# EnnaDelfen/SUHMO

Hardware: AMD Instinct MI355X
Metric: multigrid V-cycles/s (FAS head solve) + GSRB cell-updates/s; achieved HBM GB/s vs peak (higher is better)
Workload: dtype f64; 1 GPU; SHMIP-A head solve, 4096x4096 cells per GPU (square cells of 24.4 m), single AMR level, 64x64 boxes, 6 MG depths, 4+4 GSRB sweeps per depth, 16 bottom (BASELINE north_star: 4096^2 single-level); partition=none

## Files before the change

### suhmo_amd/csrc/suhmo_common.h

```cpp
#pragma once
#include <hip/hip_runtime.h>
#include <cstdio>
#include <cstdlib>
#include <cstring>
#include <utility>
#include <string>
#include <vector>
#include "../../include/suhmo_hip.h"

#define SUHMO_XOFF 16
#define SUHMO_MAXDEPTH 16

struct DV {
    int nx, ny;
    int P;
    int gy;
    int rows;
    int j0, nyg;
    double dx, dy;
    double rdx, rdy;
    double fdx, fdy;
    double alpha, beta;
    int bct[2][2];
    double two_v[2][2];
    double neu[2][2];
    int per[2];
    int ext[2];
    int i0, nxg;
    int cfx[2];
    int rk[2];
};

struct FP { double *f[SUHMO_F_COUNT]; };

__host__ __device__ __forceinline__ int cidx(const DV &v, int i, int j)
{
    return (j + v.gy) * v.P + SUHMO_XOFF + i;
}

__device__ __forceinline__ double phiW(const DV &v, const double *__restrict__ p, int idx, int i, double c, bool homog)
{
    if (i > 0 || v.cfx[0]) return p[idx - 1];
    if (v.per[0]) return p[idx + v.nx - 1];
    if (v.bct[0][0] == 0) return (homog ? 0.0 : v.two_v[0][0]) - c;
    return homog ? c : c + v.neu[0][0];
}
__device__ __forceinline__ double phiE(const DV &v, const double *__restrict__ p, int idx, int i, double c, bool homog)
{
    if (i < v.nx - 1 || v.cfx[1]) return p[idx + 1];
    if (v.per[0]) return p[idx - (v.nx - 1)];
    if (v.bct[0][1] == 0) return (homog ? 0.0 : v.two_v[0][1]) - c;
    return homog ? c : c + v.neu[0][1];
}
__device__ __forceinline__ double phiS(const DV &v, const double *__restrict__ p, int idx, int j, double c, bool homog)
{
    if (j > 0 || v.ext[0]) return p[idx - v.P];
    if (v.per[1]) return p[idx + (v.ny - 1) * v.P];
    if (v.bct[1][0] == 0) return (homog ? 0.0 : v.two_v[1][0]) - c;
    return homog ? c : c + v.neu[1][0];
}
__device__ __forceinline__ double phiN(const DV &v, const double *__restrict__ p, int idx, int j, double c, bool homog)
{
    if (j < v.ny - 1 || v.ext[1]) return p[idx + v.P];
    if (v.per[1]) return p[idx - (v.ny - 1) * v.P];
    if (v.bct[1][1] == 0) return (homog ? 0.0 : v.two_v[1][1]) - c;
    return homog ? c : c + v.neu[1][1];
}

__device__ __forceinline__ void nl_terms(const suhmo_phys_t &ph, double phi, double B, double Pi,
                                         double zb, double mask, double &nl, double &dnl)
{
    if (!ph.use_NL || mask < 0.0) { nl = 0.0; dnl = 0.0; return; }
    double N = Pi - ph.rho_w_g * (phi - zb);
    nl = -ph.A * B * N * N * N;
    dnl = 3.0 * ph.A * B * 1000.0 * ph.grav * N * N;
    if (ph.cutOffbr > B) {
        nl = nl * (1.0 - (ph.cutOffbr - B) / ph.cutOffbr);
        dnl = dnl * B / ph.cutOffbr;
    }
    if (ph.maxOffbr < B) {
        nl = nl * (1.0 - (ph.maxOffbr - B) / ph.maxOffbr);
        dnl = dnl * B / ph.maxOffbr;
    }
}

__device__ __forceinline__ double lofphi_cell(const DV &v, double aterm, double c, double e, double w,
                                              double n, double s, double bxE, double bxW, double byN,
                                              double byS, double nl)
{
    return aterm * c
           - v.beta * (bxE * (e - c) * v.rdx - bxW * (c - w) * v.rdx
                       + byN * (n - c) * v.rdy - byS * (c - s) * v.rdy)
           + nl;
}

__device__ __forceinline__ double lambda_cell(const DV &v, double aterm, double bxE, double bxW,
                                              double byN, double byS)
{
    double lam = aterm;
    lam = lam + v.rdx * v.beta * (bxE + bxW);
    lam = lam + v.rdy * v.beta * (byN + byS);
    return lam;
}

__device__ __forceinline__ void gradcc_from(const DV &v, double c, double w, double e, double s, double n, bool zW, bool zE, bool zS,
                                            bool zN, double &gx, double &gy)
{
    double gW = v.fdx * (c - w), gE = v.fdx * (e - c), gS = v.fdy * (c - s), gN = v.fdy * (n - c);
    if (zW) gW = 0.0;
    if (zE) gE = 0.0;
    if (zS) gS = 0.0;
    if (zN) gN = 0.0;
    gx = 0.5 * (gW + gE);
    gy = 0.5 * (gS + gN);
}
__device__ __forceinline__ double grad_norm(double gx, double gy) { return sqrt(gx * gx + gy * gy); }
__device__ __forceinline__ double re_from(const suhmo_phys_t &ph, double sg, double B)
{
    double discr = 1.0 + 4.0 * ph.omega * (B * B * B * ph.grav * sg) / (12.0 * ph.nu * ph.nu);
    return (-1.0 + sqrt(discr)) / (2.0 * ph.omega);
}
__device__ __forceinline__ double bcoef_face(const suhmo_phys_t &ph, double Rc, double Rm, double Bc, double Bm,
                                             double mc, double mm, bool dom_edge)
{
    double Ref = 0.5 * (Rc + Rm), Bf = 0.5 * (Bc + Bm);
    double mec;
    if (fabs(mc - mm) < 1e-10) mec = (mc > 0.0) ? 1.0 : -1.0; else mec = 0.0;
    if (dom_edge) mec = 0.0;
    double num_q = -(Bf * Bf * Bf * ph.grav);
    double denom_q = 12.0 * ph.nu * (1.0 + ph.omega * Ref);
    if (mec < 0.0 && ph.cutOffB > 0) return 0.0;
    return num_q / denom_q;
}

struct Depth {
    DV v;
    FP fp;
    size_t elems;
    int nbox;
    int prolong_pending;
    int rhs_pending;
    int bcoef_pending;
    double *phi_alt;
    int phi_fresh;
    int zb_state;
    double zb_value;
};

struct VGraph {
    int key[4]; hipGraphExec_t exec;
    double *p0[SUHMO_MAXDEPTH], *a0[SUHMO_MAXDEPTH];
    double *p1[SUHMO_MAXDEPTH], *a1[SUHMO_MAXDEPTH];
    double *rhs;
    int rout_req, rout_done, rout_np; const double *rout_rhs;
    int bcoef_in_relax; long n_bcoef_in_relax;
    int mask_clean; long n_bcoef_unmasked, n_relax_unmasked;
    unsigned zb_uniform, zb_version; long n_relax_zb[SUHMO_MAXDEPTH];
    int has_scan;
};
struct ProfEv { hipEvent_t a, b; long cells; int restricts; };

struct suhmo_level {
    int ndepth;
    int batch_owned;
    int stub;
    Depth d[SUHMO_MAXDEPTH];
    suhmo_level_desc_t desc;
    std::vector<int> boxes;
    suhmo_phys_t ph;
    int device;
    double *scratch;
    double *hscratch;
    double *hscratch_dev;
    unsigned long long hseq;
    int poll_readback;
    size_t scratch_elems;
    suhmo_exchange_fn ex;
    suhmo_allreduce_max_fn ar;
    suhmo_allreduce_fn ar2;
    int (*ard)(void *user, double *dev_values, int n, int op, suhmo_stream_t s);
    void *user;
    int (*ex_begin)(void *user);
    int (*ex_end)(void *user, suhmo_level *L, suhmo_stream_t s);
    long graph_max_cells;
    std::vector<VGraph> vgraphs; int vgraph_seen[4]; hipStream_t gstream;
    long vgraph_replays;
    suhmo_level *gap; double gap_dt;
    void *rccl;
    int faces_deferred;
    void *ipc; int ipc_owner;
    long agg_min_cells;
    int agg_depth, agg_world, agg_rank;
    suhmo_level *agg;
    int agg_static_stale;
    suhmo_allgather_fn ag; void *ag_user;
    double *agg_send, *agg_recv; size_t agg_cap; long agg_gathers;
    int resout_req, resout_armed, resout_done; const double *resout_rhs; long resout_count;
    int resout_np;
    int bcoef_in_relax, bcoef_nd; long bcoef_in_relax_count;
    int avg_overlap, avg_fork, avg_flying; long avg_overlap_count;
    hipStream_t astream; hipEvent_t aev[2];
    long frhs_stream, frhs_tile;
    long strip_tile, strip_tile_rst, strip_tile_shallow, strip_colour, strip_stream, strip_stream_rst, strip_prolong_unfused;
    int prof_on;
    std::vector<ProfEv> prof;
    int gsrb_variant;
    long fused_min_cells;
    int bcoef_fused;
    int bcoef_tile_x;
    int fused_nt;
    int fused_restrict;
    int fused_hc;
    int fas_rhs_fused;
    int strips_rhs_local;
    int skip_mask;
    int mask_reported;
    int coarse_mask_ok;
    unsigned mask_epoch, maskflag_epoch;
    int mask_known, mask_state;
    unsigned mask_version, mask_scan_version;
    int mask_scan_pending, mask_capturing;
    int mask_scan_captured;
    int mask_view;
    int mask_scan_errors;
    unsigned *mask_host; hipEvent_t mask_ev;
    long mask_scans, bcoef_unmasked, relax_unmasked;
    int zb_known, zb_off;
    unsigned zb_version, zb_scan_version;
    int zb_scan_pending, zb_scan_errors;
    unsigned long long *zb_dev, *zb_host;
    hipEvent_t zb_ev;
    long zb_scans, relax_zb_uniform[SUHMO_MAXDEPTH];
    int overlap_halo;
    hipStream_t xstream; hipEvent_t xev[2]; long overlapped;
    int tile_strips;
    int tile_chunks;
    int resid_in_relax;
    int fas_rhs_in_relax;
    long tile_max_cells;
    int tile_restrict;
    int tile_order;
    int bottom_solver; long bottom_one_launch_max_cells;
    unsigned long long *bottom_ctr; long bottom_host_iters, bottom_host_solves;
    int gsrb_tile, tile_t, tile_s;
    struct suhmo_tagmap *tags;
    int faces_made;
    double *bal_buf;
    int track_old_volume, vol_np;
    double *vol_buf, *wb_buf;
};
static inline void suhmo_faces_made(suhmo_level *L) { L->faces_made = 1; }

enum { SUHMO_MASK_UNKNOWN = 0, SUHMO_MASK_CLEAN = 1, SUHMO_MASK_DIRTY = 2 };
static inline void suhmo_mask_written(suhmo_level *L)
{
    L->coarse_mask_ok = 0; L->maskflag_epoch = 0;
    L->mask_version++; L->mask_state = SUHMO_MASK_UNKNOWN;
}
static inline void suhmo_mask_halo_written(suhmo_level *L) { L->mask_version++; L->mask_state = SUHMO_MASK_UNKNOWN; }
enum { SUHMO_ZB_UNKNOWN = 0, SUHMO_ZB_UNIFORM = 1, SUHMO_ZB_VARYING = 2 };
static inline void suhmo_zb_written(suhmo_level *L)
{
    L->zb_version++;
    for (int d = 0; d < SUHMO_MAXDEPTH; d++) L->d[d].zb_state = SUHMO_ZB_UNKNOWN;
}
static inline bool suhmo_zb_uniform(const suhmo_level *L, int depth)
{
    return L->zb_known && !L->zb_off && L->d[depth].zb_state == SUHMO_ZB_UNIFORM && !L->ex && L->desc.nx_global == 0;
}
void suhmo_zb_poll(suhmo_level *L);
int suhmo_zb_scan_if_due(suhmo_level *L, hipStream_t st);
bool suhmo_gsrb_streams(const suhmo_level *L, int depth);
bool suhmo_mask_would_scan(const suhmo_level *L);
#define SUHMO_HSCRATCH_DOUBLES 64
#define SUHMO_HSCRATCH_MASK 60
#define SUHMO_HSCRATCH_ZB 16
static inline unsigned *suhmo_mask_report_word(const suhmo_level *L) { return (unsigned *)(L->scratch + L->scratch_elems - 1); }
static inline unsigned *suhmo_mask_scan_word(const suhmo_level *L) { return suhmo_mask_report_word(L) + 1; }
int suhmo_mask_scan_begin(suhmo_level *L, hipStream_t st);
int suhmo_mask_scan_end(suhmo_level *L, hipStream_t st);
void suhmo_mask_poll(suhmo_level *L);
static inline bool suhmo_mask_clean(const suhmo_level *L, int depth)
{
    return L->mask_known && !L->mask_view && L->mask_state == SUHMO_MASK_CLEAN && (depth == 0 || L->coarse_mask_ok) && L->desc.nx_global == 0;
}
void suhmo_set_error(const char *fmt, ...);
void suhmo_tagmap_release(struct suhmo_tagmap *m);
struct SuhmoTimer { const char *name; double t0; int mode; explicit SuhmoTimer(const char *n); ~SuhmoTimer(); };
#define SUHMO_TIME(label) SuhmoTimer suhmo_tm_(label)
#define HIPCHK(x) do { hipError_t e_ = (x); if (e_ != hipSuccess) { \
    suhmo_set_error("%s:%d %s -> %s", __FILE__, __LINE__, #x, hipGetErrorString(e_)); return -2; } } while (0)
#define ARG(cond) do { if (!(cond)) { suhmo_set_error("%s:%d bad argument: %s", __FILE__, __LINE__, #cond); return -1; } } while (0)

double *suhmo_field(suhmo_level *L, int depth, int field);
int suhmo_level_create_(suhmo_level_t **out, const suhmo_level_desc_t *desc, bool stub);
void suhmo_level_share_transport(suhmo_level *dst, const suhmo_level *src);
int suhmo_level_materialize_(suhmo_level *L);
void suhmo_fp_changed();
unsigned long suhmo_fp_epoch();
struct SwapGuard {
    double **a, **b; bool armed;
    SwapGuard() : a(nullptr), b(nullptr), armed(false) {}
    void arm(double **a_, double **b_) { a = a_; b = b_; std::swap(*a, *b); armed = true; suhmo_fp_changed(); }
    void back() { if (armed) { std::swap(*a, *b); armed = false; suhmo_fp_changed(); } }
    ~SwapGuard() { back(); }
};
int suhmo_average_operator_all(suhmo_level *L, int nd, hipStream_t st);
int suhmo_restrict_both(suhmo_level *L, int depth, hipStream_t st);
bool suhmo_gsrb_can_fuse_prolong(suhmo_level *L, int depth, int sweeps);
int suhmo_level_residual_and_norm(suhmo_level *L, double *out, hipStream_t st);
int suhmo_level_norm_from_partials(suhmo_level *L, int np, double *out, hipStream_t st);
bool suhmo_gsrb_can_fuse_rhs(suhmo_level *L, int depth, int sweeps, bool rhs_local = false);
bool suhmo_gsrb_can_fuse_bcoef(suhmo_level *L, int sweeps);
bool suhmo_gsrb_can_overlap_avg(const suhmo_level *L);
int suhmo_avg_join(suhmo_level *L, hipStream_t st);
void suhmo_avg_release(suhmo_level *L);
int suhmo_launch_gsrb(suhmo_level *L, int depth, int sweeps, int tail, hipStream_t st, int *restricted = nullptr);
void suhmo_level_drop_graphs(suhmo_level *L);
int suhmo_ensure_phi_halo(suhmo_level *L, int depth, int need, hipStream_t st);
int suhmo_fas_coarse_rhs(suhmo_level *L, int depth, hipStream_t st, int hcomp = 0);
struct HostSlot { double *val; unsigned long long *flag; unsigned long long seq; };
HostSlot suhmo_host_slot(suhmo_level *L);
int suhmo_readback(suhmo_level *L, hipStream_t st, double *out, double *out2 = nullptr);
HostSlot suhmo_reduce_slot(suhmo_level *L);
int suhmo_reduce_finish(suhmo_level *L, hipStream_t st, int n, int op, double *out, double *out2 = nullptr);
__device__ __forceinline__ void suhmo_publish(const HostSlot &h, double v)
{
    if (!h.val) return;
    h.val[0] = v;
    __hip_atomic_store(h.flag, h.seq, __ATOMIC_RELEASE, __HIP_MEMORY_SCOPE_SYSTEM);
}
int suhmo_build_mg_coefficients(suhmo_level *L, bool with_faces, hipStream_t st);
void suhmo_ipc_release(suhmo_level *L);
int suhmo_ipc_batch(suhmo_level *L, int open, hipStream_t st);
int suhmo_agg_setup(suhmo_level *L);
void suhmo_agg_release(suhmo_level *L);
int suhmo_agg_gather_static(suhmo_level *L, bool with_faces, hipStream_t st);
int suhmo_agg_gather_faces(suhmo_level *L, int nd, hipStream_t st);
int suhmo_agg_gather_state(suhmo_level *L, hipStream_t st);
int suhmo_agg_scatter(suhmo_level *L, hipStream_t st);
int suhmo_exchange_list(suhmo_level *L, int depth, const int *fields, int n, hipStream_t st);
bool suhmo_bottom_one_launch(const suhmo_level *L, int dep);
int suhmo_bottom_configure(suhmo_level *L, int solver, long one_launch_max_cells);
long suhmo_bottom_counter(const suhmo_level *L, int which);
int suhmo_bottom_solve(suhmo_level *L, int dep, int tail, hipStream_t st);
static inline int suhmo_halo_rows(const DV &v) { return v.gy < v.ny ? v.gy : v.ny; }
struct SolveNoInit {
    double rnorm, initial_rnorm, norm_last;
    int iter;
    void start(double r) { rnorm = r; initial_rnorm = r; norm_last = 2.0 * r; iter = 0; }
    bool go(const suhmo_solver_params_t *sp) const
    {
        const bool goNorm = rnorm > sp->norm_thresh, goRedu = rnorm > sp->eps * initial_rnorm, goIter = iter < sp->max_iter;
        const bool goHang = iter < sp->imin || rnorm < (1.0 - sp->hang) * norm_last, goMin = iter < sp->iter_min;
        return goMin || (goIter && goRedu && goHang && goNorm);
    }
    void cycled(double r) { norm_last = rnorm; rnorm = r; iter++; }
};
template <class Residual, class Cycle>
int suhmo_solve_no_init(const suhmo_solver_params_t *sp, int *iters, double *hist, Residual residual, Cycle cycle)
{
    int rc;
    double rnorm = 0.0;
    if ((rc = residual(&rnorm))) return rc;
    SolveNoInit s;
    s.start(rnorm);
    if (hist) hist[0] = rnorm;
    while (s.go(sp)) {
        if ((rc = cycle()) || (rc = residual(&rnorm))) return rc;
        s.cycled(rnorm);
        if (hist) hist[s.iter] = rnorm;
    }
    if (iters) *iters = s.iter;
    return 0;
}
```

### suhmo_amd/csrc/suhmo_fas.hip

```cpp
#include "suhmo_common.h"
#include <cstdlib>

static int eff_depths(const suhmo_level *L, const suhmo_solver_params_t *sp)
{
    int nd = L->ndepth;
    if (sp->max_depth >= 0 && sp->max_depth + 1 < nd) nd = sp->max_depth + 1;
    return nd;
}

static int relax(suhmo_level *L, int dep, int sweeps, int tail, suhmo_stream_t s, bool observable = false, int *restricted = nullptr)
{
    L->resout_armed = observable && dep == 0 && L->resout_req && L->resid_in_relax;
    int rc = suhmo_launch_gsrb(L, dep, sweeps, tail, (hipStream_t)s, restricted);
    L->resout_armed = 0;
    if (rc) return rc;
    if (sweeps > 0 && observable) return suhmo_level_fill_ghosts(L, dep, SUHMO_F_PHI, 1, s);
    return 0;
}

static int rows_after_prolong(int dep, int num_smooth)
{
    int tail_post = 2;
    for (int d = 1; d <= dep; d++) tail_post = (2 * num_smooth + tail_post + 1) / 2;
    return 2 * num_smooth + tail_post;
}
int suhmo_prolong_with_halo(suhmo_level *L, int depth, hipStream_t st);

static int fas_cycle(suhmo_level *L, int dep, const suhmo_solver_params_t *sp, int nd, suhmo_stream_t s)
{
    int rc;
    const int S = sp->num_smooth;
    const int tail_post = dep == 0 ? 2 : (rows_after_prolong(dep - 1, S) + 1) / 2;
    if (dep == nd - 1) {
        if (!L->bottom_solver) return relax(L, dep, sp->num_bottom, tail_post, s, dep == 0);
        if ((rc = relax(L, dep, sp->num_bottom, tail_post, s))) return rc;
        if ((rc = suhmo_bottom_solve(L, dep, tail_post, (hipStream_t)s))) return rc;
        return dep == 0 ? suhmo_level_fill_ghosts(L, dep, SUHMO_F_PHI, 0, s) : 0;
    }
    Depth &C = L->d[dep + 1];
    int restricted = 0;
    if ((rc = relax(L, dep, S, rows_after_prolong(dep, S), s, false, &restricted))) return rc;
    if (!restricted && (rc = suhmo_restrict_both(L, dep, (hipStream_t)s))) return rc;
    if ((rc = suhmo_avg_join(L, (hipStream_t)s))) return rc;
    if (L->agg && dep + 1 == L->agg_depth) {
        suhmo_level *A = L->agg;
        const int ndA = nd - L->agg_depth;
        if (L->agg_static_stale && (rc = suhmo_agg_gather_static(L, true, (hipStream_t)s))) return rc;
        if ((rc = suhmo_agg_gather_state(L, (hipStream_t)s))) return rc;
        const int next_sweeps = ndA == 1 ? sp->num_bottom : S;
        if (suhmo_gsrb_can_fuse_rhs(A, 0, next_sweeps)) A->d[0].rhs_pending = 1;
        else if ((rc = suhmo_fas_coarse_rhs(A, 0, (hipStream_t)s))) return rc;
        if ((rc = fas_cycle(A, 0, sp, ndA, s))) return rc;
        if ((rc = suhmo_agg_scatter(L, (hipStream_t)s))) return rc;
        if (suhmo_gsrb_can_fuse_prolong(L, dep, S)) L->d[dep].prolong_pending = 1;
        else if ((rc = suhmo_prolong_with_halo(L, dep, (hipStream_t)s))) return rc;
        return relax(L, dep, S, tail_post, s, dep == 0);
    }
    const bool one_pass_rhs = L->fas_rhs_fused != 0;
    const bool rhs_local = L->ex && (C.v.rk[0] || C.v.rk[1]) && one_pass_rhs && L->desc.nx_global == 0 && L->strips_rhs_local
                           && suhmo_halo_rows(C.v) >= 2;
    if (rhs_local) {
        static const int both[2] = {SUHMO_F_PHI, SUHMO_F_RES};
        if ((rc = suhmo_exchange_list(L, dep + 1, both, 2, (hipStream_t)s))) return rc;
    } else if ((rc = suhmo_ensure_phi_halo(L, dep + 1, suhmo_halo_rows(C.v), (hipStream_t)s))) return rc;
    if (one_pass_rhs && (L->desc.nx_global == 0)) {
        const int next_sweeps = (dep + 1 == nd - 1) ? sp->num_bottom : S;
        if (suhmo_gsrb_can_fuse_rhs(L, dep + 1, next_sweeps, rhs_local)) C.rhs_pending = 1;
        else if ((rc = suhmo_fas_coarse_rhs(L, dep + 1, (hipStream_t)s, rhs_local ? suhmo_halo_rows(C.v) - 1 : 0))) return rc;
    } else {
        HIPCHK(hipMemcpyAsync(C.fp.f[SUHMO_F_PHIOLD], C.fp.f[SUHMO_F_PHI], C.elems * sizeof(double), hipMemcpyDeviceToDevice, (hipStream_t)s));
        if ((rc = suhmo_level_apply_op(L, dep + 1, 0, s))) return rc;
        if ((rc = suhmo_level_axby(L, dep + 1, SUHMO_F_RHS, SUHMO_F_RES, SUHMO_F_LPHI, 1.0, 1.0, s))) return rc;
    }
    if (!rhs_local && (rc = suhmo_level_exchange(L, dep + 1, SUHMO_F_RHS, s))) return rc;
    if ((rc = fas_cycle(L, dep + 1, sp, nd, s))) return rc;
    if (suhmo_gsrb_can_fuse_prolong(L, dep, S)) {
        L->d[dep].prolong_pending = 1;
    } else {
        if ((rc = suhmo_prolong_with_halo(L, dep, (hipStream_t)s))) return rc;
    }
    return relax(L, dep, S, tail_post, s, dep == 0);
}

static int vcycle_body(suhmo_level *L, const suhmo_solver_params_t *sp, int nd, suhmo_stream_t s, bool eager)
{
    int rc;
    L->avg_fork = 0;
    if (sp->bcoeff_otf && nd > 1 && suhmo_gsrb_can_fuse_bcoef(L, sp->num_smooth)) {
        L->d[0].bcoef_pending = 1; L->bcoef_nd = nd;
        L->maskflag_epoch = 0; L->mask_reported = 0;
        L->avg_fork = eager && suhmo_gsrb_can_overlap_avg(L);
    } else if (sp->bcoeff_otf) {
        if ((rc = suhmo_avg_join(L, (hipStream_t)s))) return rc;
        L->faces_deferred = 1;
        rc = suhmo_level_update_operator(L, 0, s);
        if (rc) { L->faces_deferred = 0; return rc; }
        if (L->mask_reported) L->maskflag_epoch = L->mask_epoch;
        if ((rc = suhmo_average_operator_all(L, nd, (hipStream_t)s))) return rc;
    } else L->maskflag_epoch = 0;
    rc = fas_cycle(L, 0, sp, nd, s);
    L->avg_fork = 0;
    { int rj = suhmo_avg_join(L, (hipStream_t)s); if (!rc) rc = rj; }
    if (L->d[0].bcoef_pending) {
        L->d[0].bcoef_pending = 0;
        if (!rc) { suhmo_set_error("internal: no relaxation launch formed the face coefficients"); rc = -4; }
    }
    L->maskflag_epoch = 0;
    return rc;
}

void suhmo_level_drop_graphs(suhmo_level *L)
{
    if (getenv("SUHMO_GRAPH_DEBUG")) { int ok = 0; for (VGraph &g : L->vgraphs) ok += g.exec != nullptr; fprintf(stderr,
        "[suhmo] level %dx%d: %zu V-cycle graphs, %d executable\n", L->d[0].v.nx, L->d[0].v.ny, L->vgraphs.size(), ok); }
    for (VGraph &g : L->vgraphs) if (g.exec) (void)hipGraphExecDestroy(g.exec);
    L->vgraphs.clear();
    if (L->gstream) { (void)hipStreamDestroy(L->gstream); L->gstream = nullptr; }
    suhmo_avg_release(L);
}
static int vcycle_graph(suhmo_level *L, const suhmo_solver_params_t *sp, int nd, suhmo_stream_t s, bool &done)
{
    done = false;
    const int key[4] = {sp->num_smooth, sp->num_bottom, sp->bcoeff_otf, nd};
    const int mask_clean = (suhmo_mask_clean(L, 0) ? 1 : 0) | (L->ndepth > 1 && suhmo_mask_clean(L, 1) ? 2 : 0);
    const bool scanning = sp->bcoeff_otf && suhmo_mask_would_scan(L);
    const int bcoef_in_relax = L->bcoef_in_relax != 0;
    unsigned zb_uniform = 0;
    for (int d = 0; d < L->ndepth; d++) if (suhmo_zb_uniform(L, d)) zb_uniform |= 1u << d;
    for (size_t k = L->vgraphs.size(); k-- > 0;) {
        VGraph &g = L->vgraphs[k];
        if (!g.zb_uniform || g.zb_version == L->zb_version) continue;
        if (g.exec) (void)hipGraphExecDestroy(g.exec);
        L->vgraphs.erase(L->vgraphs.begin() + k);
    }
    auto launch = [&](const VGraph &g) {
        int rc = 0;
        if (scanning && (rc = suhmo_mask_scan_begin(L, (hipStream_t)s))) return rc;
        HIPCHK(hipGraphLaunch(g.exec, (hipStream_t)s)); L->vgraph_replays++;
        if (scanning && (rc = suhmo_mask_scan_end(L, (hipStream_t)s))) return rc;
        return 0;
    };
    auto replayed = [&](const VGraph &g) {
        L->bcoef_unmasked += g.n_bcoef_unmasked; L->relax_unmasked += g.n_relax_unmasked; L->bcoef_in_relax_count += g.n_bcoef_in_relax;
        for (int d = 0; d < L->ndepth; d++) L->relax_zb_uniform[d] += g.n_relax_zb[d];
        if (g.rout_done) { L->resout_done = 1; L->resout_count++; L->resout_np = g.rout_np; }
    };
    auto at_start = [&](const VGraph &g) {
        if (memcmp(g.key, key, sizeof(key)) || g.mask_clean != mask_clean || g.bcoef_in_relax != bcoef_in_relax || g.zb_uniform != zb_uniform) return false;
        for (int d = 0; d < L->ndepth; d++) if (L->d[d].fp.f[SUHMO_F_PHI] != g.p0[d] || L->d[d].phi_alt != g.a0[d]) return false;
        if (g.rout_req != (L->resid_in_relax ? L->resout_req : 0) || g.rout_rhs != L->resout_rhs) return false;
        return L->d[0].fp.f[SUHMO_F_RHS] == g.rhs;
    };
    for (const VGraph &g : L->vgraphs)
        if (at_start(g)) {
            if (!g.exec || (scanning && !g.has_scan)) return 0;
            { int rc = launch(g); if (rc) return rc; }
            for (int d = 0; d < L->ndepth; d++) { L->d[d].fp.f[SUHMO_F_PHI] = g.p1[d]; L->d[d].phi_alt = g.a1[d]; } suhmo_fp_changed();
            replayed(g);
            done = true;
            return 0;
        }
    for (int k = 0; k < 4; k++) if (L->vgraph_seen[k] != key[k]) { memcpy(L->vgraph_seen, key, sizeof(key)); return 0; }
    if (L->vgraphs.size() >= 16) return 0;
    if (!L->gstream) HIPCHK(hipStreamCreateWithFlags(&L->gstream, hipStreamNonBlocking));
    VGraph g; memcpy(g.key, key, sizeof(key)); g.exec = nullptr; g.mask_clean = mask_clean; g.has_scan = 0; g.bcoef_in_relax = bcoef_in_relax;
    g.zb_uniform = zb_uniform; g.zb_version = L->zb_version;
    long relax_zb[SUHMO_MAXDEPTH]; memcpy(relax_zb, L->relax_zb_uniform, sizeof(relax_zb));
    for (int d = 0; d < SUHMO_MAXDEPTH; d++) { g.p0[d] = g.a0[d] = g.p1[d] = g.a1[d] = nullptr; }
    for (int d = 0; d < L->ndepth; d++) { g.p0[d] = L->d[d].fp.f[SUHMO_F_PHI]; g.a0[d] = L->d[d].phi_alt; }
    g.rhs = L->d[0].fp.f[SUHMO_F_RHS];
    g.rout_req = L->resid_in_relax ? L->resout_req : 0; g.rout_rhs = L->resout_rhs; g.rout_done = 0;
    const int rout_before = L->resout_done; const long rout_count = L->resout_count;
    const long bcoef_unmasked = L->bcoef_unmasked, relax_unmasked = L->relax_unmasked, bcoef_in_relax_count = L->bcoef_in_relax_count;
    HIPCHK(hipStreamSynchronize((hipStream_t)s));
    hipGraph_t graph = nullptr;
    hipError_t e = hipStreamBeginCapture(L->gstream, hipStreamCaptureModeThreadLocal);
    int rc = 0;
    if (e == hipSuccess) {
        L->mask_capturing = 1; L->mask_scan_captured = 0;
        rc = vcycle_body(L, sp, nd, (suhmo_stream_t)L->gstream, false);
        L->mask_capturing = 0; g.has_scan = L->mask_scan_captured;
        e = hipStreamEndCapture(L->gstream, &graph);
    }
    g.n_bcoef_unmasked = L->bcoef_unmasked - bcoef_unmasked; g.n_relax_unmasked = L->relax_unmasked - relax_unmasked;
    g.n_bcoef_in_relax = L->bcoef_in_relax_count - bcoef_in_relax_count; L->bcoef_in_relax_count = bcoef_in_relax_count;
    L->bcoef_unmasked = bcoef_unmasked; L->relax_unmasked = relax_unmasked;
    for (int d = 0; d < SUHMO_MAXDEPTH; d++) { g.n_relax_zb[d] = L->relax_zb_uniform[d] - relax_zb[d]; L->relax_zb_uniform[d] = relax_zb[d]; }
    g.rout_done = L->resout_count != rout_count;
    g.rout_np = L->resout_np;
    L->resout_done = rout_before; L->resout_count = rout_count;
    bool clean = true;
    for (int d = 0; d < L->ndepth; d++) {
        clean = clean && !L->d[d].prolong_pending && !L->d[d].rhs_pending && !L->d[d].bcoef_pending;
        g.p1[d] = L->d[d].fp.f[SUHMO_F_PHI]; g.a1[d] = L->d[d].phi_alt;
        L->d[d].prolong_pending = 0; L->d[d].rhs_pending = 0; L->d[d].bcoef_pending = 0;
        L->d[d].fp.f[SUHMO_F_PHI] = g.p0[d]; L->d[d].phi_alt = g.a0[d];
    }
    if (e == hipSuccess && rc == 0 && clean && graph && hipGraphInstantiate(&g.exec, graph, nullptr, nullptr, 0) != hipSuccess) g.exec = nullptr;
    if (!(e == hipSuccess && rc == 0 && clean)) g.exec = nullptr;
    if (graph) (void)hipGraphDestroy(graph);
    (void)hipGetLastError();
    L->vgraphs.push_back(g);
    if (!g.exec || (scanning && !g.has_scan)) return 0;
    if ((rc = launch(g))) return rc;
    for (int d = 0; d < L->ndepth; d++) { L->d[d].fp.f[SUHMO_F_PHI] = g.p1[d]; L->d[d].phi_alt = g.a1[d]; } suhmo_fp_changed();
    replayed(g);
    done = true;
    return 0;
}

extern "C" int suhmo_level_vcycle(suhmo_level_t *L, const suhmo_solver_params_t *sp, suhmo_stream_t s)
{
    SUHMO_TIME("AMRFASMultiGrid::VCycle");
    ARG(L && sp);
    HIPCHK(hipSetDevice(L->device));
    int nd = eff_depths(L, sp);
    const Depth &D = L->d[0];
    const bool ext = D.v.ext[0] || D.v.ext[1];
    const bool host_bottom = L->bottom_solver && !suhmo_bottom_one_launch(L, nd - 1);
    suhmo_mask_poll(L);
    suhmo_zb_poll(L);
    { int rc = suhmo_zb_scan_if_due(L, (hipStream_t)s); if (rc) return rc; }
    const bool graphs = L->graph_max_cells > 0 && !L->ex && !ext && !L->prof_on && !host_bottom && (long)D.v.nx * D.v.ny <= L->graph_max_cells;
    if (graphs) {
        bool done = false;
        int rc = vcycle_graph(L, sp, nd, s, done);
        if (rc || done) return rc;
    }
    return vcycle_body(L, sp, nd, s, !graphs);
}

extern "C" int suhmo_level_solve(suhmo_level_t *L, const suhmo_solver_params_t *sp, int *iters, double *hist, suhmo_stream_t s)
{
    SUHMO_TIME("AMRFASMultiGrid::solve");
    ARG(L && sp);
    HIPCHK(hipSetDevice(L->device));
    bool have_res = false;
    int np = 0;
    auto residual = [&](double *rnorm) {
        if (!have_res) return suhmo_level_residual_and_norm(L, rnorm, (hipStream_t)s);
        if (np > 0) return suhmo_level_norm_from_partials(L, np, rnorm, (hipStream_t)s);
        return suhmo_level_norm(L, 0, SUHMO_F_RES, 0, rnorm, s);
    };
    auto cycle = [&] {
        L->resout_req = 1 | 4; L->resout_rhs = nullptr; L->resout_done = 0; L->resout_np = 0;
        int rc = suhmo_level_vcycle(L, sp, s);
        have_res = L->resout_done != 0;
        np = have_res ? L->resout_np : 0;
        L->resout_req = 0; L->resout_done = 0; L->resout_np = 0;
        return rc;
    };
    int rc = suhmo_solve_no_init(sp, iters, hist, residual, cycle);
    if (rc) return rc;
    return suhmo_level_fill_ghosts(L, 0, SUHMO_F_PHI, 0, s);
}
```

### suhmo_amd/csrc/suhmo_gsrb.hip

```cpp
#include "suhmo_hier.h"
#include "suhmo_batch.h"
#include "suhmo_relax_plan.h"
#include <type_traits>

template <bool HAS_ALPHA>
__device__ __forceinline__ void d_gsrb_pass_simple(const DV &v, const FP &fp, suhmo_phys_t ph, int pass, int jlo, int jhi,
                                                   const FP *__restrict__ ft = nullptr, const int2 *__restrict__ push = nullptr)
{
    int j = jlo + (int)(blockIdx.y * blockDim.y + threadIdx.y);
    int t = blockIdx.x * blockDim.x + threadIdx.x;
    if (j > jhi) return;
    int i = 2 * t + ((j + v.j0 + pass) & 1);
    if (i >= v.nx) return;
    double *__restrict__ phi = fp.f[SUHMO_F_PHI];
    int idx = cidx(v, i, j);
    double c = phi[idx];
    double e = phiE(v, phi, idx, i, c, false), w = phiW(v, phi, idx, i, c, false);
    double n = phiN(v, phi, idx, j, c, false), s = phiS(v, phi, idx, j, c, false);
    double bxW = fp.f[SUHMO_F_BX][idx], bxE = fp.f[SUHMO_F_BX][idx + 1];
    double byS = fp.f[SUHMO_F_BY][idx], byN = fp.f[SUHMO_F_BY][idx + v.P];
    double nl, dnl;
    nl_terms(ph, c, fp.f[SUHMO_F_B][idx], fp.f[SUHMO_F_PI][idx], fp.f[SUHMO_F_ZB][idx],
             fp.f[SUHMO_F_MASK][idx], nl, dnl);
    double aterm = HAS_ALPHA ? v.alpha * fp.f[SUHMO_F_ACOEF][idx] : v.alpha;
    double lofphi = lofphi_cell(v, aterm, c, e, w, n, s, bxE, bxW, byN, byS, nl);
    double lam = lambda_cell(v, aterm, bxE, bxW, byN, byS);
    double denom = 1.0e-16 + lam + dnl;
    const double pnew = c + (fp.f[SUHMO_F_RHS][idx] - lofphi) / denom;
    phi[idx] = pnew;
    if (push) {
        if (i == 0) { int2 q = push[j]; if (q.x >= 0) ft[q.x].f[SUHMO_F_PHI][q.y] = pnew; }
        if (i == v.nx - 1) { int2 q = push[v.ny + j]; if (q.x >= 0) ft[q.x].f[SUHMO_F_PHI][q.y] = pnew; }
        if (j == 0) { int2 q = push[2 * v.ny + i]; if (q.x >= 0) ft[q.x].f[SUHMO_F_PHI][q.y] = pnew; }
        if (j == v.ny - 1) { int2 q = push[2 * v.ny + v.nx + i]; if (q.x >= 0) ft[q.x].f[SUHMO_F_PHI][q.y] = pnew; }
    }
}
template <class T, bool HAS_ALPHA>
__global__ __launch_bounds__(256) void k_gsrb_pass_simple(T t, int pass, int lo, int hi, const int2 *__restrict__ push, const int *__restrict__ pbase)
{
    const DV &v = t.view();
    const FP *ft = t.table();
    d_gsrb_pass_simple<HAS_ALPHA>(v, t.fields(), t.phys(), pass, -lo, v.ny - 1 + hi, ft, ft && push ? push + pbase[blockIdx.z] : nullptr);
}
template <class T> int launch_colour_pass(const T &t, bool has_alpha, int pass, int lo, int hi, const void *push, const int *pbase, hipStream_t st)
{
    const dim3 grd = grid2d((t.nx() + 1) / 2, t.ny() + lo + hi);
    if (has_alpha) return launch_grid(k_gsrb_pass_simple<T, true>, t, grd, BLK2D, st, pass, lo, hi, (const int2 *)push, pbase);
    return launch_grid(k_gsrb_pass_simple<T, false>, t, grd, BLK2D, st, pass, lo, hi, (const int2 *)push, pbase);
}
template int launch_colour_pass(const OnBoxes &, bool, int, int, int, const void *, const int *, hipStream_t);
template int launch_colour_pass(const OnMembers &, bool, int, int, int, const void *, const int *, hipStream_t);

static int launch_simple(suhmo_level *L, int depth, int pass, int ext_rows, hipStream_t st)
{
    const DV &v = L->d[depth].v;
    return launch_colour_pass(on_level(L, depth), v.alpha != 0.0, pass, v.rk[0] ? ext_rows : 0, v.rk[1] ? ext_rows : 0, nullptr, nullptr, st);
}

int suhmo_gsrb_colour_pass(suhmo_level *L, int depth, int pass, hipStream_t st)
{
    int rc = launch_simple(L, depth, pass, 0, st); if (rc) return rc;
    L->d[depth].phi_fresh = 0;
    return 0;
}

template <int G, int T, int S> struct BoxGeom { static constexpr int LW = T + 2 * G, NT = (((LW * LW / 2 + S - 1) / S + 63) / 64) * 64; };
template <bool HAS_ALPHA, int G, int T, int S>
__global__ __launch_bounds__((BoxGeom<G, T, S>::NT)) __attribute__((amdgpu_waves_per_eu(1, 3))) void k_gsrb_box_m(const DV *__restrict__ vt,
    const FP *__restrict__ ft, const int2 *__restrict__ halo, const int *__restrict__ hbase,
                                                                     suhmo_phys_t ph, int fsrc, int fdst, int npass, int bcg)
{
    constexpr int BOXG = G, BOXNT = BoxGeom<G, T, S>::NT, HG = SUHMO_BOX_HALO;
    constexpr int LWmax = T + 2 * BOXG;
    __shared__ double pl[LWmax * LWmax];
    __shared__ int own[LWmax * LWmax];
    const int k = blockIdx.y, tid = threadIdx.x;
    const DV &v = vt[k];
    const int tiles_x = (v.nx + T - 1) / T, tiles_y = (v.ny + T - 1) / T;
    if ((int)blockIdx.x >= tiles_x * tiles_y) return;
    const int tj = blockIdx.x / tiles_x, ti = blockIdx.x - tj * tiles_x;
    const int twb = (v.nx + tiles_x - 1) / tiles_x, thb = (v.ny + tiles_y - 1) / tiles_y;
    const int x0 = ti * twb, y0 = tj * thb;
    const int tw = min(twb, v.nx - x0), th = min(thb, v.ny - y0);
    if (tw <= 0 || th <= 0) return;
    const int LW = tw + 2 * BOXG, LH = th + 2 * BOXG, EW = v.nx + 2 * HG, HW = (LW + 1) / 2;
    const int2 *__restrict__ hk = halo + hbase[k];
    const FP &fk = ft[k];
    const int par0 = (v.i0 + x0 - BOXG + v.j0 + y0 - BOXG) & 1;
    int cq[S][2], cb[S][2], co[S][2], cd[S][2];
    double c_rhs[S][2], c_bxW[S][2], c_bxE[S][2], c_byS[S][2], c_byN[S][2], c_B[S][2], c_Pi[S][2], c_zb[S][2], c_mk[S][2], c_at[S][2];
    int2 hq[S][2];
#pragma unroll
    for (int s = 0; s < S; s++)
#pragma unroll
        for (int c = 0; c < 2; c++) {
            cq[s][c] = -1; hq[s][c] = int2{-1, 0};
            const int p = tid + s * BOXNT;
            if (p < LH * HW) {
                const int lj = p / HW, li = 2 * (p - lj * HW) + ((lj + par0 + c) & 1);
                if (li < LW) { cq[s][c] = lj * LW + li; hq[s][c] = hk[(y0 + lj + HG - BOXG) * EW + x0 + li + HG - BOXG]; }
            }
        }
#pragma unroll
    for (int s = 0; s < S; s++)
#pragma unroll
        for (int c = 0; c < 2; c++) {
            const int q = cq[s][c];
            cb[s][c] = -1; co[s][c] = 0; cd[s][c] = 0;
            c_rhs[s][c] = c_bxW[s][c] = c_bxE[s][c] = c_byS[s][c] = c_byN[s][c] = c_B[s][c] = c_Pi[s][c] = c_zb[s][c] = c_mk[s][c] = c_at[s][c] = 0.0;
            if (q < 0) continue;
            const int b = hq[s][c].x, off = hq[s][c].y;
            own[q] = b;
            if (b < 0) { pl[q] = 0.0; continue; }
            const int lj = q / LW, li = q - lj * LW;
            const int dx = li < BOXG ? BOXG - li : (li >= BOXG + tw ? li - (BOXG + tw - 1) : 0), dy = lj < BOXG ? BOXG - lj : (lj >= BOXG + th ? lj - (BOXG + th - 1) : 0);
            const int d = max(dx, dy);
            const FP &fb = b == k ? fk : ft[b];
            if (d >= BOXG) { pl[q] = fb.f[fsrc][off]; continue; }
            const int Pb = b == k ? v.P : vt[b].P;
            cb[s][c] = b; co[s][c] = off; cd[s][c] = d;
            pl[q] = fb.f[fsrc][off];
            c_rhs[s][c] = fb.f[SUHMO_F_RHS][off];
            c_bxW[s][c] = fb.f[SUHMO_F_BX][off]; c_bxE[s][c] = fb.f[SUHMO_F_BX][off + 1];
            c_byS[s][c] = fb.f[SUHMO_F_BY][off]; c_byN[s][c] = fb.f[SUHMO_F_BY][off + Pb];
            c_B[s][c] = fb.f[SUHMO_F_B][off]; c_Pi[s][c] = fb.f[SUHMO_F_PI][off]; c_zb[s][c] = fb.f[SUHMO_F_ZB][off]; c_mk[s][c] = fb.f[SUHMO_F_MASK][off];
            c_at[s][c] = HAS_ALPHA ? v.alpha * fb.f[SUHMO_F_ACOEF][off] : v.alpha;
        }
    __syncthreads();
    int nk[S][2];
    double hW[S][2], hE[S][2], hS[S][2], hN[S][2];
#pragma unroll
    for (int s = 0; s < S; s++)
#pragma unroll
        for (int c = 0; c < 2; c++) {
            nk[s][c] = 0; hW[s][c] = hE[s][c] = hS[s][c] = hN[s][c] = 0.0;
            const int q = cq[s][c], b = cb[s][c];
            if (b < 0) continue;
            const bool oW = own[q - 1] < 0, oE = own[q + 1] < 0, oS = own[q - LW] < 0, oN = own[q + LW] < 0;
            if (!(oW || oE || oS || oN)) continue;
            const DV &vb = b == k ? v : vt[b];
            const double *__restrict__ psrc = (b == k ? fk : ft[b]).f[fsrc];
            const int off = co[s][c];
            if (oW) { if (vb.cfx[0]) { nk[s][c] |= 1; hW[s][c] = psrc[off - 1]; } else if (vb.bct[0][0] == 0) { nk[s][c] |= 2; hW[s][c] = vb.two_v[0][0];
                } else { nk[s][c] |= 3; hW[s][c] = vb.neu[0][0]; } }
            if (oE) { if (vb.cfx[1]) { nk[s][c] |= 1 << 2; hE[s][c] = psrc[off + 1]; } else if (vb.bct[0][1] == 0) { nk[s][c] |= 2 << 2; hE[s][c] = vb.two_v[0][1];
                } else { nk[s][c] |= 3 << 2; hE[s][c] = vb.neu[0][1]; } }
            if (oS) { if (vb.ext[0]) { nk[s][c] |= 1 << 4; hS[s][c] = psrc[off - vb.P]; } else if (vb.bct[1][0] == 0) { nk[s][c] |= 2 << 4;
                hS[s][c] = vb.two_v[1][0]; } else { nk[s][c] |= 3 << 4; hS[s][c] = vb.neu[1][0]; } }
            if (oN) { if (vb.ext[1]) { nk[s][c] |= 1 << 6; hN[s][c] = psrc[off + vb.P]; } else if (vb.bct[1][1] == 0) { nk[s][c] |= 2 << 6;
                hN[s][c] = vb.two_v[1][1]; } else { nk[s][c] |= 3 << 6; hN[s][c] = vb.neu[1][1]; } }
        }
    auto outside = [](int kind, double g, double c) { return kind == 1 ? g : (kind == 2 ? g - c : c + g); };
    auto update = [&](int q, int kinds, double g_w, double g_e, double g_s, double g_n, double rhs, double bxW, double bxE, double byS, double byN, double B,
        double Pi, double zb, double mk, double at) {
        const double c = pl[q];
        double w, e, sv, n;
        if (kinds == 0) { w = pl[q - 1]; e = pl[q + 1]; sv = pl[q - LW]; n = pl[q + LW]; }
        else {
            w = (kinds & 3) ? outside(kinds & 3, g_w, c) : pl[q - 1];
            e = ((kinds >> 2) & 3) ? outside((kinds >> 2) & 3, g_e, c) : pl[q + 1];
            sv = ((kinds >> 4) & 3) ? outside((kinds >> 4) & 3, g_s, c) : pl[q - LW];
            n = ((kinds >> 6) & 3) ? outside((kinds >> 6) & 3, g_n, c) : pl[q + LW];
        }
        double nl, dnl;
        nl_terms(ph, c, B, Pi, zb, mk, nl, dnl);
        const double lofphi = lofphi_cell(v, at, c, e, w, n, sv, bxE, bxW, byN, byS, nl);
        const double lam = lambda_cell(v, at, bxE, bxW, byN, byS);
        const double denom = 1.0e-16 + lam + dnl;
        pl[q] = c + (rhs - lofphi) / denom;
    };
    for (int m = 0; m < npass; m++) {
        const int reach = npass - 1 - m;
        if ((m & 1) == 0) {
#pragma unroll
            for (int s = 0; s < S; s++)
                if (cb[s][0] >= 0 && cd[s][0] <= reach)
                    update(cq[s][0], nk[s][0], hW[s][0], hE[s][0], hS[s][0], hN[s][0], c_rhs[s][0], c_bxW[s][0], c_bxE[s][0], c_byS[s][0], c_byN[s][0], c_B[s][0],
                        c_Pi[s][0], c_zb[s][0], c_mk[s][0], c_at[s][0]);
        } else {
#pragma unroll
            for (int s = 0; s < S; s++)
                if (cb[s][1] >= 0 && cd[s][1] <= reach)
                    update(cq[s][1], nk[s][1], hW[s][1], hE[s][1], hS[s][1], hN[s][1], c_rhs[s][1], c_bxW[s][1], c_bxE[s][1], c_byS[s][1], c_byN[s][1], c_B[s][1],
                        c_Pi[s][1], c_zb[s][1], c_mk[s][1], c_at[s][1]);
        }
        __syncthreads();
    }
    const double *__restrict__ psrc = fk.f[fsrc];
    double *__restrict__ pdst = fk.f[fdst];
    const bool gW = bcg && !v.cfx[0] && !v.per[0], gE = bcg && !v.cfx[1] && !v.per[0], gS = bcg && !v.ext[0] && !v.per[1], gN = bcg && !v.ext[1] && !v.per[1];
    for (int q = tid; q < tw * th; q += BOXNT) {
        const int jj = q / tw, ii = q - jj * tw, gi = x0 + ii, gj = y0 + jj, idx = cidx(v, gi, gj);
        const double c = pl[(BOXG + jj) * LW + BOXG + ii];
        pdst[idx] = c;
        if (gW && gi == 0) pdst[idx - 1] = phiW(v, pdst, idx, gi, c, true);
        if (gE && gi == v.nx - 1) pdst[idx + 1] = phiE(v, pdst, idx, gi, c, true);
        if (gS && gj == 0) pdst[idx - v.P] = phiS(v, pdst, idx, gj, c, true);
        if (gN && gj == v.ny - 1) pdst[idx + v.P] = phiN(v, pdst, idx, gj, c, true);
    }
    if (blockIdx.x == 0)
        for (int q = tid; q < 2 * (v.nx + 2) + 2 * v.ny; q += BOXNT) {
            int ii, jj;
            bool filled;
            if (q < v.nx + 2) { ii = q - 1; jj = -1; filled = gS && ii >= 0 && ii < v.nx; }
            else if (q < 2 * (v.nx + 2)) { ii = q - (v.nx + 2) - 1; jj = v.ny; filled = gN && ii >= 0 && ii < v.nx; }
            else if (q < 2 * (v.nx + 2) + v.ny) { ii = -1; jj = q - 2 * (v.nx + 2); filled = gW; }
            else { ii = v.nx; jj = q - 2 * (v.nx + 2) - v.ny; filled = gE; }
            if (filled) continue;
            const int idx = cidx(v, ii, jj);
            pdst[idx] = psrc[idx];
        }
}
template <int G, int T, int S>
static void launch_box(const suhmo_multi &m, const suhmo_phys_t &ph, bool has_alpha, const void *halo, const int *hbase, int fsrc, int fdst, int npass, int bc_ghosts, hipStream_t st)
{
    const dim3 grd(((m.maxnx + T - 1) / T) * ((m.maxny + T - 1) / T), m.nbox);
    if (has_alpha) hipLaunchKernelGGL((k_gsrb_box_m<true, G, T, S>), grd, dim3(BoxGeom<G, T, S>::NT), 0, st, m.dv, m.fp, (const int2 *)halo, hbase, ph, fsrc, fdst, npass, bc_ghosts);
    else hipLaunchKernelGGL((k_gsrb_box_m<false, G, T, S>), grd, dim3(BoxGeom<G, T, S>::NT), 0, st, m.dv, m.fp, (const int2 *)halo, hbase, ph, fsrc, fdst, npass, bc_ghosts);
}
int suhmo_multi_gsrb_box(const suhmo_multi &m, const suhmo_phys_t &ph, bool has_alpha, const void *halo, const int *hbase, int fsrc, int fdst, int npass, int bc_ghosts, hipStream_t st)
{
    if (m.nbox <= 0) return 0;
    if (npass < 1 || npass > 2 * SUHMO_BOX_HALO) { suhmo_set_error("internal: %d colour passes in one box launch", npass); return -4; }
    if (npass > 4) launch_box<8, 16, 1>(m, ph, has_alpha, halo, hbase, fsrc, fdst, npass, bc_ghosts, st);
    else launch_box<4, 16, 1>(m, ph, has_alpha, halo, hbase, fsrc, fdst, npass, bc_ghosts, st);
    HIPCHK(hipGetLastError());
    return 0;
}

struct FusedGeom {
    int W;
    int Hc;
    int nstrips, nchunks, ntiles;
    int ylo, yhi;
    int jbeg, jend;
    int wrap_y;
    const unsigned *negflag; unsigned mask_epoch;
    int nchl, chunk0, chunk1, edges;
    const double *pc, *pco; int Pc, gyc;
    double *rres, *rphi; int rP, rgy;
    const double *fres; double *frhs, *flphi, *fphiold;
    const double *ortrue; double *ores, *olphi;
    double *onorm;
    double zb_uniform;
};

struct FusedArgs { DV v; FP fp; const double *pin; double *pout; suhmo_phys_t ph; FusedGeom g; };
typedef const __attribute__((address_space(4))) FusedArgs *ColdArgs;
__device__ __forceinline__ ColdArgs cold_args()
{
    ColdArgs k = (ColdArgs)__builtin_amdgcn_kernarg_segment_ptr();
    asm volatile("" : "+s"(k));
    return k;
}
struct SideBC { int t; double two_v, neu; };
template <bool COLD> __device__ __forceinline__ SideBC side_bc(const DV &v, const int d, const int s)
{
    SideBC b;
    if constexpr (COLD) { const ColdArgs k = cold_args(); b.t = k->v.bct[d][s]; b.two_v = k->v.two_v[d][s]; b.neu = k->v.neu[d][s]; }
    else { b.t = v.bct[d][s]; b.two_v = v.two_v[d][s]; b.neu = v.neu[d][s]; }
    return b;
}
__device__ __forceinline__ double bc_ghost(const SideBC &b, double c) { return (b.t == 0) ? b.two_v - c : c + b.neu; }

template <bool MASKED> struct RowMask { double mask[2]; };
template <> struct RowMask<false> {};
template <bool ZBU> struct RowZb { double zb[2]; };
template <> struct RowZb<true> {};
template <bool MASKED, bool ZBU = false>
struct RowCoef : RowMask<MASKED>, RowZb<ZBU> {
    double rhs[2], B[2], Pi[2], a[2], byS[2], byN[2];
    double bx0, bx1, bx2;
};
template <bool MASKED, bool ZBU> __device__ __forceinline__ double row_mask(const RowCoef<MASKED, ZBU> &q, int a)
{
    if constexpr (MASKED) return q.mask[a]; else return 1.0;
}
template <bool MASKED, bool ZBU> __device__ __forceinline__ double row_zb(const RowCoef<MASKED, ZBU> &q, int a, const FusedGeom &g)
{
    if constexpr (ZBU) return g.zb_uniform; else return q.zb[a];
}
#define CP2(d, s, f) d.f[0] = s.f[0]; d.f[1] = s.f[1]
template <bool HAS_ALPHA, bool MASKED, bool ZBU>
__device__ __forceinline__ void copy_coef(RowCoef<MASKED, ZBU> &d, const RowCoef<MASKED, ZBU> &s)
{
    CP2(d, s, rhs); CP2(d, s, B); CP2(d, s, Pi);
    if constexpr (!ZBU) { CP2(d, s, zb); }
    if constexpr (MASKED) { CP2(d, s, mask); }
    if (HAS_ALPHA) { CP2(d, s, a); }
    CP2(d, s, byS); CP2(d, s, byN);
    d.bx0 = s.bx0; d.bx1 = s.bx1; d.bx2 = s.bx2;
}

template <int K, bool HAS_ALPHA, int NT, int RM = 0, bool FRHS = false, bool MASKED = true, bool BCF = false, bool ZBU = false>
__global__ __launch_bounds__(NT) void k_gsrb_fused(DV v, FP fp, const double *__restrict__ pin,
                                                   double *__restrict__ pout, suhmo_phys_t ph, FusedGeom g)
{
    constexpr bool ROUT = RM == 2, RR = RM != 0;
    static_assert(!(FRHS && (RR || HAS_ALPHA)), "the right-hand side is formed in the plain launch of an alpha = 0 operator");
    static_assert(!BCF || (K == 2 && NT == 64 && RM == 0 && !FRHS && !HAS_ALPHA && !MASKED), "the faces are formed in the plain two-sweep launch of a clean-mask alpha = 0 operator");
    static_assert(!ZBU || (K == 2 && NT == 64 && !HAS_ALPHA && !MASKED), "the bed as a scalar: the two-sweep launches of a clean-mask alpha = 0 operator");
    constexpr bool WIDE = RR || BCF;
    constexpr int DL = BCF ? 1 : 0;
    constexpr int LW = 2 * NT, R = 2 * K + 3 + (WIDE ? 1 : 0);
    constexpr int HX = 2 * K + (WIDE ? 2 : 0), EY = RR ? 1 : 0;
    __shared__ double lds[R * LW];
    __shared__ double rre[BCF ? LW : 1], rsg[BCF ? LW : 1];
    __shared__ double2 gpv[BCF ? 2 * NT : 1];

    int b = blockIdx.x, q = g.ntiles / 8, rem = g.ntiles % 8, xcd = b % 8;
    int tile = xcd * q + (xcd < rem ? xcd : rem) + b / 8;
    int strip = tile / g.nchl, chunk = tile % g.nchl;
    chunk = g.edges ? (chunk < g.chunk0 ? chunk : g.chunk1 + (chunk - g.chunk0)) : g.chunk0 + chunk;

    const int t = threadIdx.x;
    const int c0 = strip * g.W;
    const int xl = 2 * t;
    const int i0 = c0 - HX + xl;
    const bool in_row = xl < g.W + 2 * HX;
    int im = i0;
    if (v.per[0]) { if (im < 0) im += v.nx; else if (im >= v.nx) im -= v.nx; }
    const bool cval = in_row && im >= 0 && im < v.nx;
    const int cend = (c0 + g.W < v.nx) ? c0 + g.W : v.nx;
    const bool own = cval && i0 >= c0 && i0 < cend;

    const int jA = g.jbeg + chunk * g.Hc;
    const int jB = (jA + g.Hc < g.jend) ? jA + g.Hc : g.jend;
    const int jmin = (jA - EY - 2 * K > g.ylo) ? jA - EY - 2 * K : g.ylo;
    const int jmax = (jB - 1 + EY + 2 * K < g.yhi) ? jB - 1 + EY + 2 * K : g.yhi;

    const double *__restrict__ f_rhs = fp.f[SUHMO_F_RHS], *__restrict__ f_B = fp.f[SUHMO_F_B];
    const double *__restrict__ f_Pi = fp.f[SUHMO_F_PI], *__restrict__ f_zb = fp.f[SUHMO_F_ZB];
    const double *__restrict__ f_mask = fp.f[SUHMO_F_MASK], *__restrict__ f_a = fp.f[SUHMO_F_ACOEF];
    const double *__restrict__ f_bx = fp.f[SUHMO_F_BX], *__restrict__ f_by = fp.f[SUHMO_F_BY];
    const int jminP = BCF ? ((g.wrap_y || jmin > 0) ? jmin - 1 : jmin) : jmin;
    const int jmaxP = BCF ? ((g.wrap_y || jmax < v.ny - 1) ? jmax + 1 : jmax) : jmax;

    auto wrapj = [&](int j) { if (g.wrap_y) { if (j < 0) j += v.ny; else if (j >= v.ny) j -= v.ny; } return j; };
    auto ld2 = [&](const double *__restrict__ p, int idx) { return *reinterpret_cast<const double2 *>(p + idx); };

    RowCoef<MASKED, ZBU> cf0, cf1, cf2, cf3, cf4, cf5;
    double racc = 0.0, raccp = 0.0;
    double nmax = 0.0;
    const bool xbc = !v.per[0] && (c0 - HX <= 0 || c0 + g.W + HX >= v.nx);
    const bool ybc = !v.per[1] && (jmin <= 0 || jmax >= v.ny - 1);
    double2 pnext = make_double2(0.0, 0.0);
    double2 pprev = make_double2(0.0, 0.0);
    double bw0 = 0.0, be0 = 0.0, bw1 = 0.0, be1 = 0.0, rn0 = 0.0, rn1 = 0.0, rep0 = 0.0, rep1 = 0.0, sgG = 0.0;
    const bool xedge = c0 - HX <= 0 || c0 + g.W + HX >= v.nx;
    bool usemask = false;
    if constexpr (MASKED) usemask = !g.negflag || *g.negflag == g.mask_epoch;

    int sr = 0;
    auto ring = [](int x) { return x < 0 ? x + R : x; };
    for (int r = jminP - 1; r <= jB - 1 + 2 * K + EY + DL; r++) {
        bool lphi = cval && (r + 1 >= jminP) && (r + 1 <= jmaxP);
        if (lphi) {
            const int jr = wrapj(r + 1);
            pnext = ld2(pin, cidx(v, im, jr));
            if (!BCF && g.pc) {
                const int ic = ((jr >> 1) + g.gyc) * g.Pc + SUHMO_XOFF + (im >> 1);
                const double corr = 1.0 * g.pc[ic] + (-1.0) * g.pco[ic];
                pnext.x = pnext.x + corr; pnext.y = pnext.y + corr;
            }
        }
        bool lcf = cval && (r >= jmin) && (r <= jmax);
        if (lcf) {
            int idx = cidx(v, im, wrapj(r));
#define LD2(dst, p, ix) { double2 t_ = ld2(p, ix); dst[0] = t_.x; dst[1] = t_.y; }
            if constexpr (!BCF) { LD2(cf0.rhs, (FRHS ? g.fres : f_rhs), idx); LD2(cf0.Pi, f_Pi, idx); if constexpr (!ZBU) { LD2(cf0.zb, f_zb, idx); } }
            LD2(cf0.B, f_B, idx);
            if constexpr (MASKED) { if (usemask) { LD2(cf0.mask, f_mask, idx); } else { cf0.mask[0] = 1.0; cf0.mask[1] = 1.0; } }
            if (HAS_ALPHA) LD2(cf0.a, f_a, idx);
            if constexpr (BCF) { bw0 = f_B[idx - 1]; be0 = f_B[idx + 2]; }
            else {
                LD2(cf0.byS, f_by, idx); LD2(cf0.byN, f_by, idx + v.P);
                double2 bxp = ld2(f_bx, idx);
                cf0.bx0 = bxp.x; cf0.bx1 = bxp.y; cf0.bx2 = f_bx[idx + 2];
            }
        }
        if constexpr (BCF) {
            if (cval && (r - 1 >= jmin) && (r - 1 <= jmax)) {
                const int idx = cidx(v, im, wrapj(r - 1));
                LD2(cf1.rhs, f_rhs, idx); LD2(cf1.Pi, f_Pi, idx); if constexpr (!ZBU) { LD2(cf1.zb, f_zb, idx); }
            }
        }
        __syncthreads();

        if constexpr (FRHS) {
            const int jf = r - 1;
            if (cval && jf >= jmin && jf <= jmax) {
                const int s0 = ring(sr - 1), sN = sr;
                const double *row = lds + s0 * LW;
                double lo[2], cc[2];
#pragma unroll
                for (int a = 0; a < 2; a++) {
                    const int x = xl + a, i = im + a;
                    double c = row[x];
                    double w = row[(a == 0 && xl == 0) ? 0 : x - 1], e = row[(a == 1 && xl == LW - 2) ? LW - 1 : x + 1];
                    double n = lds[sN * LW + x], s = a ? pprev.y : pprev.x;
                    if (xbc) {
                        if (i == 0) w = (v.bct[0][0] == 0) ? v.two_v[0][0] - c : c + v.neu[0][0];
                        if (i == v.nx - 1) e = (v.bct[0][1] == 0) ? v.two_v[0][1] - c : c + v.neu[0][1];
                    }
                    if (ybc) {
                        if (jf == 0 && !v.ext[0]) s = (v.bct[1][0] == 0) ? v.two_v[1][0] - c : c + v.neu[1][0];
                        if (jf == v.ny - 1 && !v.ext[1]) n = (v.bct[1][1] == 0) ? v.two_v[1][1] - c : c + v.neu[1][1];
                    }
                    double nl, dnl;
                    nl_terms(ph, c, cf1.B[a], cf1.Pi[a], row_zb(cf1, a, g), row_mask(cf1, a), nl, dnl);
                    const double bxW = a ? cf1.bx1 : cf1.bx0, bxE = a ? cf1.bx2 : cf1.bx1;
                    lo[a] = lofphi_cell(v, v.alpha, c, e, w, n, s, bxE, bxW, cf1.byN[a], cf1.byS[a], nl);
                    cc[a] = c;
                }
                cf1.rhs[0] = 1.0 * cf1.rhs[0] + 1.0 * lo[0]; cf1.rhs[1] = 1.0 * cf1.rhs[1] + 1.0 * lo[1];
                const bool lo_end = v.ext[0] && chunk == 0, hi_end = v.ext[1] && chunk == g.nchunks - 1;
                const int jP0 = lo_end ? jmin : jA, jP1 = hi_end ? jmax + 1 : jB;
                const int jR0 = lo_end ? jmin + 1 : jA, jR1 = hi_end ? jmax : jB;
                if (own && jf >= jP0 && jf < jP1) {
                    const int idx = cidx(v, i0, jf);
                    if (jf >= jR0 && jf < jR1) {
                        *reinterpret_cast<double2 *>(g.flphi + idx) = make_double2(lo[0], lo[1]);
                        *reinterpret_cast<double2 *>(g.frhs + idx) = make_double2(cf1.rhs[0], cf1.rhs[1]);
                    }
                    *reinterpret_cast<double2 *>(g.fphiold + idx) = make_double2(cc[0], cc[1]);
                }
                pprev = make_double2(cc[0], cc[1]);
            }
            __syncthreads();
        }

        auto advance_a = [&](const int m, const RowCoef<MASKED, ZBU> &q, auto a_tag) {
            constexpr int a = decltype(a_tag)::value;
            const int j = r - m - DL;
            const int x = xl + a, i = im + a;
            const int s0 = ring(sr - m - DL), sN = ring(sr - m - DL + 1), sS = ring(sr - m - DL - 1);
            const double *row = lds + s0 * LW;
            double c = row[x];
            double w = row[(a == 0 && xl == 0) ? 0 : x - 1], e = row[(a == 1 && xl == LW - 2) ? LW - 1 : x + 1];
            double n = lds[sN * LW + x], s = lds[sS * LW + x];
            if (xbc) {
                const SideBC bW = side_bc<BCF>(v, 0, 0), bE = side_bc<BCF>(v, 0, 1);
                if (i == 0) w = bc_ghost(bW, c);
                if (i == v.nx - 1) e = bc_ghost(bE, c);
            }
            if (ybc) {
                if (j == 0 && (BCF || !v.ext[0])) s = bc_ghost(side_bc<BCF>(v, 1, 0), c);
                if (j == v.ny - 1 && (BCF || !v.ext[1])) n = bc_ghost(side_bc<BCF>(v, 1, 1), c);
            }
            double nl, dnl;
            nl_terms(ph, c, q.B[a], q.Pi[a], row_zb(q, a, g), row_mask(q, a), nl, dnl);
            const double bxW = a ? q.bx1 : q.bx0, bxE = a ? q.bx2 : q.bx1;
            double aterm = HAS_ALPHA ? v.alpha * q.a[a] : v.alpha;
            double lofphi = lofphi_cell(v, aterm, c, e, w, n, s, bxE, bxW, q.byN[a], q.byS[a], nl);
            double lam = lambda_cell(v, aterm, bxE, bxW, q.byN[a], q.byS[a]);
            double denom = 1.0e-16 + lam + dnl;
            lds[s0 * LW + x] = c + (q.rhs[a] - lofphi) / denom;
        };
        auto advance = [&](const int m, const RowCoef<MASKED, ZBU> &q) {
            const int j = r - m - DL;
            if (j >= jmin && j <= jmax) {
                const int a = (j + v.j0 + ((m - 1) & 1)) & 1;
                if (a) { if (cval) advance_a(m, q, std::integral_constant<int, 1>()); }
                else   { if (cval) advance_a(m, q, std::integral_constant<int, 0>()); }
            }
        };
        if constexpr (BCF) {
            const int j1 = r - 1;
            const bool faces = j1 >= jmin && j1 <= jmax;
            double *__restrict__ o_bx = fp.f[SUHMO_F_BX], *__restrict__ o_by = fp.f[SUHMO_F_BY];
            if (faces && cval) {
                const double *row = lds + ring(sr - 1) * LW, *rowN = lds + sr * LW, *rowS = lds + ring(sr - 2) * LW;
                const double ca = row[xl], cb = row[xl + 1];
                double w = row[xl == 0 ? 0 : xl - 1], e = row[xl == LW - 2 ? LW - 1 : xl + 2];
                double na = rowN[xl], nb = rowN[xl + 1], sa = rowS[xl], sb = rowS[xl + 1];
                if (xbc) {
                    const SideBC bW = side_bc<true>(v, 0, 0), bE = side_bc<true>(v, 0, 1);
                    if (im == 0) w = bc_ghost(bW, ca);
                    if (im + 1 == v.nx - 1) e = bc_ghost(bE, cb);
                }
                if (ybc) {
                    if (j1 == 0) { const SideBC bS = side_bc<true>(v, 1, 0); sa = bc_ghost(bS, ca); sb = bc_ghost(bS, cb); }
                    if (j1 == v.ny - 1) { const SideBC bN = side_bc<true>(v, 1, 1); na = bc_ghost(bN, ca); nb = bc_ghost(bN, cb); }
                }
                double gx0, gy0, gx1, gy1;
                gradcc_from(v, ca, w, cb, sa, na, false, false, false, false, gx0, gy0);
                gradcc_from(v, cb, ca, e, sb, nb, false, false, false, false, gx1, gy1);
                const double sg0 = grad_norm(gx0, gy0), sg1 = grad_norm(gx1, gy1);
                rn0 = re_from(ph, sg0, cf1.B[0]); rn1 = re_from(ph, sg1, cf1.B[1]);
                *reinterpret_cast<double2 *>(rre + xl) = make_double2(rn0, rn1);
                if (xedge) {
                    if (v.per[0]) *reinterpret_cast<double2 *>(rsg + xl) = make_double2(sg0, sg1);
                    else if (im == 0) sgG = grad_norm(2.0 * gx0 - gx1, 2.0 * gy0 - gy1);
                    else if (im == v.nx - 2) sgG = grad_norm(2.0 * gx1 - gx0, 2.0 * gy1 - gy0);
                }
                cf1.byN[0] = 0.0; cf1.byN[1] = 0.0;
                if (j1 > jmin) {
                    cf1.byS[0] = bcoef_face(ph, rn0, rep0, cf1.B[0], cf2.B[0], 1.0, 1.0, false);
                    cf1.byS[1] = bcoef_face(ph, rn1, rep1, cf1.B[1], cf2.B[1], 1.0, 1.0, false);
                    cf2.byN[0] = cf1.byS[0]; cf2.byN[1] = cf1.byS[1];
                    double gxp0 = 0.0, gxp1 = 0.0, gyp0 = 0.0, gyp1 = 0.0;
                    if ((g.wrap_y && (j1 == 0 || j1 == v.ny)) || (ybc && (j1 == 1 || j1 == v.ny - 1))) {
                        const double2 px = gpv[t], py = gpv[NT + t];
                        gxp0 = px.x; gxp1 = px.y; gyp0 = py.x; gyp1 = py.y;
                    }
                    if (g.wrap_y && (j1 == 0 || j1 == v.ny)) {
                        const double2 bS = ld2(f_B, cidx(v, im, -1)), bN = ld2(f_B, cidx(v, im, v.ny));
                        const double sp0 = grad_norm(gxp0, gyp0), sp1 = grad_norm(gxp1, gyp1);
                        cf1.byS[0] = bcoef_face(ph, rn0, re_from(ph, sp0, bS.x), cf1.B[0], bS.x, 1.0, 1.0, false);
                        cf1.byS[1] = bcoef_face(ph, rn1, re_from(ph, sp1, bS.y), cf1.B[1], bS.y, 1.0, 1.0, false);
                        cf2.byN[0] = bcoef_face(ph, re_from(ph, sg0, bN.x), rep0, bN.x, cf2.B[0], 1.0, 1.0, false);
                        cf2.byN[1] = bcoef_face(ph, re_from(ph, sg1, bN.y), rep1, bN.y, cf2.B[1], 1.0, 1.0, false);
                        if (own && j1 == v.ny && jB == cold_args()->g.jend) *reinterpret_cast<double2 *>(o_by + cidx(v, i0, v.ny)) = make_double2(cf2.byN[0], cf2.byN[1]);
                    }
                    if (ybc && j1 == 1) {
                        const double2 bS = ld2(f_B, cidx(v, im, -1));
                        const double rg0 = re_from(ph, grad_norm(2.0 * gxp0 - gx0, 2.0 * gyp0 - gy0), bS.x);
                        const double rg1 = re_from(ph, grad_norm(2.0 * gxp1 - gx1, 2.0 * gyp1 - gy1), bS.y);
                        cf2.byS[0] = bcoef_face(ph, rep0, rg0, cf2.B[0], bS.x, 1.0, 1.0, false);
                        cf2.byS[1] = bcoef_face(ph, rep1, rg1, cf2.B[1], bS.y, 1.0, 1.0, false);
                        if (own && jA <= 0) *reinterpret_cast<double2 *>(o_by + cidx(v, i0, 0)) = make_double2(cf2.byS[0], cf2.byS[1]);
                    }
                    if (ybc && j1 == v.ny - 1) {
                        const double2 bN = ld2(f_B, cidx(v, im, v.ny));
                        const double rg0 = re_from(ph, grad_norm(2.0 * gx0 - gxp0, 2.0 * gy0 - gyp0), bN.x);
                        const double rg1 = re_from(ph, grad_norm(2.0 * gx1 - gxp1, 2.0 * gy1 - gyp1), bN.y);
                        cf1.byN[0] = bcoef_face(ph, rg0, rn0, bN.x, cf1.B[0], 1.0, 1.0, false);
                        cf1.byN[1] = bcoef_face(ph, rg1, rn1, bN.y, cf1.B[1], 1.0, 1.0, false);
                        if (own && jB == cold_args()->g.jend) *reinterpret_cast<double2 *>(o_by + cidx(v, i0, v.ny)) = make_double2(cf1.byN[0], cf1.byN[1]);
                    }
                    if (own && j1 >= jA && j1 < jB) *reinterpret_cast<double2 *>(o_by + cidx(v, i0, j1)) = make_double2(cf1.byS[0], cf1.byS[1]);
                } else { cf1.byS[0] = 0.0; cf1.byS[1] = 0.0; }
                gpv[t] = make_double2(gx0, gx1); gpv[NT + t] = make_double2(gy0, gy1);
            }
            advance(1, cf2);
            __syncthreads();
            if (faces && cval) {
                double reW = rre[xl == 0 ? 0 : xl - 1], reE = rre[xl == LW - 2 ? LW - 1 : xl + 2];
                if (xedge) {
                    if (im == 0) reW = re_from(ph, v.per[0] ? rsg[xl == 0 ? 0 : xl - 1] : sgG, bw1);
                    if (im == v.nx - 2) reE = re_from(ph, v.per[0] ? rsg[xl == LW - 2 ? LW - 1 : xl + 2] : sgG, be1);
                }
                cf1.bx0 = bcoef_face(ph, rn0, reW, cf1.B[0], bw1, 1.0, 1.0, false);
                cf1.bx1 = bcoef_face(ph, rn1, rn0, cf1.B[1], cf1.B[0], 1.0, 1.0, false);
                cf1.bx2 = bcoef_face(ph, reE, rn1, be1, cf1.B[1], 1.0, 1.0, false);
                if (own && j1 >= jA && j1 < jB) {
                    const int idx = cidx(v, i0, j1);
                    *reinterpret_cast<double2 *>(o_bx + idx) = make_double2(cf1.bx0, cf1.bx1);
                    if (i0 == v.nx - 2) o_bx[idx + 2] = cf1.bx2;
                }
                rep0 = rn0; rep1 = rn1;
            }
            advance(2, cf3);
            __syncthreads();
            advance(3, cf4);
            __syncthreads();
            advance(4, cf5);
        } else {
        advance(1, cf1);
        __syncthreads();
        advance(2, cf2);
        if constexpr (K >= 2) {
            __syncthreads();
            advance(3, cf3);
            __syncthreads();
            advance(4, cf4);
        }
        }

        if constexpr (RR) {
            const int jr = r - 2 * K - 1;
            if (own && jr >= jA && jr < jB && jr >= 0 && jr < v.ny) {
                const RowCoef<MASKED, ZBU> &q = (K >= 2) ? cf5 : cf3;
                const int s0 = ring(sr - (2 * K + 1)), sN = ring(sr - 2 * K), sS = ring(sr - (2 * K + 2));
                const double *row = lds + s0 * LW;
                double acc = (jr & 1) ? racc : 0.0, accp = (jr & 1) ? raccp : 0.0;
                double lo2[2] = {0.0, 0.0};
#pragma unroll
                for (int a = 0; a < 2; a++) {
                    const int x = xl + a, i = im + a;
                    double c = row[x], w = row[x - 1], e = row[x + 1];
                    double n = lds[sN * LW + x], s = lds[sS * LW + x];
                    if (xbc) {
                        if (i == 0) w = (v.bct[0][0] == 0) ? v.two_v[0][0] - c : c + v.neu[0][0];
                        if (i == v.nx - 1) e = (v.bct[0][1] == 0) ? v.two_v[0][1] - c : c + v.neu[0][1];
                    }
                    if (ybc) {
                        if (jr == 0 && !v.ext[0]) s = (v.bct[1][0] == 0) ? v.two_v[1][0] - c : c + v.neu[1][0];
                        if (jr == v.ny - 1 && !v.ext[1]) n = (v.bct[1][1] == 0) ? v.two_v[1][1] - c : c + v.neu[1][1];
                    }
                    double nl, dnl;
                    nl_terms(ph, c, q.B[a], q.Pi[a], row_zb(q, a, g), row_mask(q, a), nl, dnl);
                    const double bxW = a ? q.bx1 : q.bx0, bxE = a ? q.bx2 : q.bx1;
                    double aterm = HAS_ALPHA ? v.alpha * q.a[a] : v.alpha;
                    double lofphi = lofphi_cell(v, aterm, c, e, w, n, s, bxE, bxW, q.byN[a], q.byS[a], nl);
                    if constexpr (ROUT) lo2[a] = lofphi;
                    else {
                        acc = acc + (q.rhs[a] - lofphi) / 4.0;
                        accp = accp + c / 4.0;
                    }
                }
                if constexpr (ROUT) {
                    const int idx = cidx(v, i0, jr);
                    const double2 rt = *reinterpret_cast<const double2 *>(g.ortrue + idx);
                    const double r0 = -1.0 * lo2[0] + 1.0 * rt.x, r1 = -1.0 * lo2[1] + 1.0 * rt.y;
                    *reinterpret_cast<double2 *>(g.ores + idx) = make_double2(r0, r1);
                    if (g.olphi) *reinterpret_cast<double2 *>(g.olphi + idx) = make_double2(lo2[0], lo2[1]);
                    nmax = fmax(nmax, fmax(fabs(r0), fabs(r1)));
                } else if (jr & 1) {
                    const int ic = ((jr >> 1) + g.rgy) * g.rP + SUHMO_XOFF + (i0 >> 1);
                    g.rres[ic] = acc; g.rphi[ic] = accp;
                } else { racc = acc; raccp = accp; }
            }
        }
        {
            const int jo = r - 2 * K - DL;
            if (own && jo >= jA && jo < jB) {
                const int so = ring(sr - 2 * K - DL);
                double2 o = make_double2(lds[so * LW + xl], lds[so * LW + xl + 1]);
                *reinterpret_cast<double2 *>(pout + cidx(v, i0, jo)) = o;
            }
        }
        sr = sr + 1 == R ? 0 : sr + 1;
        if (in_row) { lds[sr * LW + xl] = pnext.x; lds[sr * LW + xl + 1] = pnext.y; }
        if constexpr (WIDE && K >= 2) copy_coef<HAS_ALPHA, MASKED, ZBU>(cf5, cf4);
        if constexpr (K >= 2) { copy_coef<HAS_ALPHA, MASKED, ZBU>(cf4, cf3); copy_coef<HAS_ALPHA, MASKED, ZBU>(cf3, cf2); }
        else if constexpr (RR) copy_coef<HAS_ALPHA, MASKED, ZBU>(cf3, cf2);
        copy_coef<HAS_ALPHA, MASKED, ZBU>(cf2, cf1);
        if constexpr (BCF) { CP2(cf1, cf0, B); bw1 = bw0; be1 = be0; }
        else copy_coef<HAS_ALPHA, MASKED, ZBU>(cf1, cf0);
    }
    if constexpr (ROUT) {
        if (g.onorm) {
            static_assert(!ROUT || NT == 64, "one wave per workgroup");
#pragma unroll
            for (int o = 32; o > 0; o >>= 1) nmax = fmax(nmax, __shfl_xor(nmax, o));
            if (t == 0) g.onorm[strip * g.nchunks + chunk] = nmax;
        }
    }
}

static bool fused_ok(const suhmo_level *L, const Depth &D, int K)
{
    const DV &v = D.v;
    if (v.nx % 2 || v.nx < 64 || v.ny < 4 * K + 4) return false;
    if (v.cfx[0] || v.cfx[1] || L->desc.nx_global > 0) return false;
    if ((v.ext[0] || v.ext[1]) && (v.gy < 2 * K || v.ny < 2 * K)) return false;
    if (v.per[1] && !(v.ext[0] || v.ext[1]) && v.ny < 4 * K) return false;
    return true;
}

enum { STEP_COLOUR = 0, STEP_TILE, STEP_STREAM };
enum { ABSORB_PROLONG = 1, ABSORB_RHS = 2, ABSORB_BCOEF = 4 };
struct RelaxStep {
    int path;
    int done;
    int S, T, chunks;
    int K, NT;
    bool masked;
    bool zbu;
    bool rst, rout, frhs, bcf, prolong;
    int need, adv;
    bool shallow;
    int absorbs() const { return (prolong ? ABSORB_PROLONG : 0) | (frhs ? ABSORB_RHS : 0) | (bcf ? ABSORB_BCOEF : 0); }
    int RM() const { return rout ? 2 : rst ? 1 : 0; }
};

typedef void (*FusedFn)(DV, FP, const double *, double *, suhmo_phys_t, FusedGeom);
struct FusedKernel { int key; FusedFn fn; int slots; };
constexpr int fused_key(int K, bool alpha, int NT, int RM, bool frhs, bool masked, bool bcf, bool zbu = false)
{
    return K | RM << 4 | alpha << 8 | frhs << 9 | masked << 10 | bcf << 11 | NT << 12 | zbu << 24;
}
#define FK(K, A, NT, RM, F, M, B) {fused_key(K, A, NT, RM, F, M, B), k_gsrb_fused<K, A, NT, RM, F, M, B>, 0}
#define FK_ZBU(RM, F, B) {fused_key(2, false, 64, RM, F, false, B, true), k_gsrb_fused<2, false, 64, RM, F, false, B, true>, 0}
#define FK_PLAIN(K, NT, RM) FK(K, false, NT, RM, false, true, false), FK(K, false, NT, RM, false, false, false)
static FusedKernel fused_kernels[] = {
    FK_PLAIN(2, 64, 0), FK_PLAIN(2, 64, 1), FK_PLAIN(2, 64, 2), FK_PLAIN(1, 64, 0), FK_PLAIN(2, 256, 0), FK_PLAIN(1, 256, 0),
    FK(1, true, 64, 0, false, true, false), FK(2, true, 64, 0, false, true, false), FK(1, true, 256, 0, false, true, false), FK(2, true, 256, 0, false, true, false),
    FK(2, false, 64, 0, true, true, false), FK(2, false, 64, 0, true, false, false), FK(2, false, 64, 0, false, false, true),
    FK_ZBU(0, false, false), FK_ZBU(1, false, false), FK_ZBU(2, false, false), FK_ZBU(0, true, false), FK_ZBU(0, false, true),
};
#undef FK_ZBU
#undef FK_PLAIN
#undef FK
static FusedKernel *fused_kernel(int K, bool alpha, int NT, int RM, bool frhs, bool masked, bool bcf, bool zbu)
{
    const int key = fused_key(K, alpha, NT, RM, frhs, masked, bcf, zbu);
    for (FusedKernel &k : fused_kernels) if (k.key == key) return &k;
    return nullptr;
}

static int launch_fused(suhmo_level *L, int depth, const RelaxStep &s, hipStream_t st, int part = 0)
{
    const int K = s.K, NT = s.NT, RM = s.RM(), ext_rows = s.adv;
    const bool RST = RM == 1, RR = RM != 0, unmasked = !s.masked;
    Depth &D = L->d[depth];
    const DV &v = D.v;
    FusedKernel *k = fused_kernel(K, v.alpha != 0.0, NT, RM, s.frhs, s.masked, s.bcf, s.zbu);
    FusedKernel *plain = (v.alpha != 0.0 || s.frhs || s.bcf) ? fused_kernel(K, false, NT, RM, false, s.masked, false, s.zbu) : k;
    if (!k || !plain || (part && (s.frhs || s.bcf)) || (s.bcf && s.prolong)) { suhmo_set_error("internal: a streaming relaxation step without a kernel"); return -4; }
    if (!D.phi_alt) {
        HIPCHK(hipMalloc(&D.phi_alt, D.elems * sizeof(double)));
        HIPCHK(hipMemsetAsync(D.phi_alt, 0, D.elems * sizeof(double), st));
    }
    FusedGeom g;
    const int HX = 2 * K + ((RR || s.bcf) ? 2 : 0);
    const int EY = RR ? 1 : 0;
    const int maxW = 2 * NT - 2 * HX;
    g.nstrips = (v.nx + maxW - 1) / maxW;
    g.W = 2 * ((v.nx + 2 * g.nstrips - 1) / (2 * g.nstrips));
    g.nstrips = (v.nx + g.W - 1) / g.W;
    {
        if (!plain->slots) {
            int nb = 0, ncu = 0, dev = 0;
            HIPCHK(hipGetDevice(&dev));
            HIPCHK(hipDeviceGetAttribute(&ncu, hipDeviceAttributeMultiprocessorCount, dev));
            HIPCHK(hipOccupancyMaxActiveBlocksPerMultiprocessor(&nb, plain->fn, NT, 0));
            plain->slots = (nb > 0 ? nb : 1) * (ncu > 0 ? ncu : 256);
        }
        g.jbeg = v.ext[0] ? -ext_rows : 0;
        g.jend = v.ny + (v.ext[1] ? ext_rows : 0);
        const int nrows = g.jend - g.jbeg;
        int nch = plain->slots / g.nstrips;
        if (nch < 1) nch = 1;
        g.Hc = (nrows + nch - 1) / nch;
        if (g.Hc < 8 * K) g.Hc = 8 * K;
        if ((long)v.nx * v.ny < 2000000L) g.Hc = 6;
        if (L->fused_hc > 0) g.Hc = L->fused_hc;
        if (RST) g.Hc += g.Hc & 1;
        if (g.Hc > nrows) g.Hc = nrows;
        g.nchunks = (nrows + g.Hc - 1) / g.Hc;
    }
    g.nchl = g.nchunks; g.chunk0 = 0; g.chunk1 = g.nchunks; g.edges = 0;
    if (part) {
        int c0 = 0, c1 = g.nchunks;
        if (v.ext[0]) while (c0 < g.nchunks && g.jbeg + c0 * g.Hc - 2 * K - EY < 0) c0++;
        if (v.ext[1]) while (c1 > c0 && std::min(g.jbeg + c1 * g.Hc, g.jend) - 1 + 2 * K + EY > v.ny - 1) c1--;
        const bool ok = c1 > c0 && c1 - c0 < g.nchunks;
        if (!ok) { if (part == 1) return 1; }
        else if (part == 1) { g.chunk0 = c0; g.chunk1 = c1; g.nchl = c1 - c0; }
        else { g.edges = 1; g.chunk0 = c0; g.chunk1 = c1; g.nchl = g.nchunks - (c1 - c0); }
    }
    g.ntiles = g.nstrips * g.nchl;
    bool selfper = v.per[1] && !(v.ext[0] || v.ext[1]);
    g.wrap_y = selfper;
    g.ylo = v.ext[0] ? g.jbeg - 2 * K - EY : (selfper ? -2 * K - EY : 0);
    g.yhi = v.ext[1] ? g.jend - 1 + 2 * K + EY : (selfper ? v.ny - 1 + 2 * K + EY : v.ny - 1);
    const double *pin = D.fp.f[SUHMO_F_PHI];
    g.pc = g.pco = nullptr; g.Pc = g.gyc = 0;
    if (s.prolong) {
        Depth &C = L->d[depth + 1];
        g.pc = C.fp.f[SUHMO_F_PHI]; g.pco = C.fp.f[SUHMO_F_PHIOLD]; g.Pc = C.v.P; g.gyc = C.v.gy;
        if (part != 1) D.prolong_pending = 0;
    }
    g.negflag = nullptr; g.mask_epoch = 0;
    if (!unmasked && L->skip_mask && L->maskflag_epoch && L->maskflag_epoch == L->mask_epoch && (depth == 0 || L->coarse_mask_ok)
        && (L->desc.nx_global == 0)) {
        g.negflag = suhmo_mask_report_word(L); g.mask_epoch = L->mask_epoch;
    }
    g.rres = g.rphi = nullptr; g.rP = g.rgy = 0;
    if (RST) {
        Depth &C = L->d[depth + 1];
        g.rres = C.fp.f[SUHMO_F_RES]; g.rphi = C.fp.f[SUHMO_F_PHI]; g.rP = C.v.P; g.rgy = C.v.gy;
        C.phi_fresh = 0;
    }
    g.zb_uniform = s.zbu ? D.zb_value : 0.0;
    g.fres = nullptr; g.frhs = g.flphi = g.fphiold = nullptr;
    g.ortrue = nullptr; g.ores = g.olphi = nullptr; g.onorm = nullptr;
    if (RM == 2) {
        g.ortrue = L->resout_rhs ? L->resout_rhs : D.fp.f[SUHMO_F_RHS];
        g.ores = D.fp.f[SUHMO_F_RES];
        if (L->resout_req & 2) { g.olphi = suhmo_field(L, depth, SUHMO_F_LPHI); if (!g.olphi) return -2; }
        if ((L->resout_req & 4) && (size_t)g.nstrips * g.nchunks + 4 < L->scratch_elems) { g.onorm = L->scratch + 2; L->resout_np = g.nstrips * g.nchunks; }
        else L->resout_np = 0;
    }
    if (s.frhs) {
        g.fres = D.fp.f[SUHMO_F_RES]; g.frhs = D.fp.f[SUHMO_F_RHS]; g.flphi = suhmo_field(L, depth, SUHMO_F_LPHI); g.fphiold = suhmo_field(L, depth, SUHMO_F_PHIOLD);
        if (!g.flphi || !g.fphiold) return -2;
        D.rhs_pending = 0; L->frhs_stream++;
    }
    if (s.bcf) { D.bcoef_pending = 0; L->bcoef_in_relax_count++; suhmo_faces_made(L); L->bcoef_unmasked++; }
    hipLaunchKernelGGL(k->fn, dim3(g.ntiles), dim3(NT), 0, st, v, D.fp, pin, D.phi_alt, L->ph, g);
    if (unmasked) L->relax_unmasked++;
    if (s.zbu) L->relax_zb_uniform[depth]++;
    if (part != 1) { std::swap(D.fp.f[SUHMO_F_PHI], D.phi_alt); suhmo_fp_changed(); }
    return 0;
}

struct TileGeom {
    int ntx, nty;
    const double *pc, *pco; int Pc, gyc;
    double *rres, *rphi; int rP, rgy;
    int frhs;
    int jbeg, jend;
    int chunks;
    int order;
};
struct PairCoef { double rhs0, rhs1, B0, B1, Pi0, Pi1, zb0, zb1, a0, a1, byS0, byS1, byN0, byN1, bx0, bx1, bx2; int mneg; };

template <int T, bool RST> struct TileShape { static constexpr int TX = T, TY = (RST && T == 32) ? 28 : T; };
template <int S, int T, bool RST> struct TileThreads { static constexpr int NT = 256; };
template <int S, int T, bool HAS_ALPHA, bool RST = false, bool CHUNKED = false>
__device__ __forceinline__ void d_gsrb_tile(const DV &v, const FP &fp, const double *__restrict__ pin, double *__restrict__ pout,
                                            const suhmo_phys_t &ph, const TileGeom &g)
{
    constexpr int TX = TileShape<T, RST>::TX, TY = TileShape<T, RST>::TY;
    constexpr int HX = 2 * S + (RST ? 2 : 0), HY = 2 * S + (RST ? 1 : 0);
    constexpr int LX = TX + 2 * HX, LY = TY + 2 * HY, NP = LX / 2, NPAIR = NP * LY;
    constexpr int NT = TileThreads<S, T, RST>::NT, NK = (NPAIR + NT - 1) / NT;
    constexpr int PAD = LX + 2;
    __shared__ double lds_raw[LY * LX + 2 * PAD];
    double *const lds = lds_raw + PAD;
    __shared__ double lq[RST ? TY * TX : 1];
    int tl = blockIdx.x;
    if (g.order) {
        const int nt = g.ntx * g.nty, q8 = nt / 8, rem = nt % 8, xcd = tl % 8;
        tl = xcd * q8 + (xcd < rem ? xcd : rem) + tl / 8;
    }
    int tx = tl % g.ntx, ty = tl / g.ntx;
    if (g.order == 2) {
        const int pan = tl / (8 * g.ntx), r = tl - pan * 8 * g.ntx, hp = (g.nty - 8 * pan < 8) ? g.nty - 8 * pan : 8;
        tx = r / hp; ty = 8 * pan + r % hp;
    }
    const int tj0 = g.jbeg + ty * TY;
    const int gx0 = tx * TX - HX, gy0 = tj0 - HY;
    const int t = threadIdx.x;
    const int par = __builtin_amdgcn_readfirstlane((int)(threadIdx.x >> 6)) & 1;
    const int u0 = ((t >> 7) << 6) | (t & 63);
    auto pair_pos = [&](const int k, int &ly, int &lx) -> bool {
        const int u = u0 + (NT / 2) * k, r = u / NP;
        ly = 2 * r + par; lx = 2 * (u - r * NP);
        return ly < LY;
    };
    static_assert(LY % 2 == 0, "rows of the region come in pairs of parities");
    const bool perx = v.per[0] && !v.cfx[0] && !v.cfx[1], pery = v.per[1] && !v.ext[0] && !v.ext[1];
    const bool openW = !perx && gx0 <= (v.cfx[0] ? -1 : 0), openE = !perx && gx0 + LX - 1 >= v.nx - 1 + (v.cfx[1] ? 1 : 0);
    const bool openS = !pery && !v.rk[0] && gy0 <= (v.ext[0] ? -1 : 0), openN = !pery && !v.rk[1] && gy0 + LY - 1 >= v.ny - 1 + (v.ext[1] ? 1 : 0);
    auto wrap = [](int i, int n) { i %= n; return i < 0 ? i + n : i; };
    auto ld2 = [&](const double *__restrict__ p, int idx) { return *reinterpret_cast<const double2 *>(p + idx); };

    PairCoef cf0, cf1, cf2, cf3, cf4;
    bool lv0, lv1, lv2, lv3, lv4;
    static_assert(NK <= 5 && TX * TY / 4 <= NT, "tile too large for the workgroup");
#define TILE_EACH(F) { F(0, cf0, lv0); if constexpr (NK > 1) F(1, cf1, lv1); if constexpr (NK > 2) F(2, cf2, lv2); \
                       if constexpr (NK > 3) F(3, cf3, lv3); if constexpr (NK > 4) F(4, cf4, lv4); }
    bool special = false;
    const bool inner = gx0 >= 0 && gx0 + LX <= v.nx && gy0 >= 0 && gy0 + LY <= v.ny;
    auto ldcoef = [&](PairCoef &c, double2 &p2, const int idx, const int i, const int j) {
        if (g.pc) {
            const int ic = ((j >> 1) + g.gyc) * g.Pc + SUHMO_XOFF + (i >> 1);
            const double corr = 1.0 * g.pc[ic] + (-1.0) * g.pco[ic];
            p2.x = p2.x + corr; p2.y = p2.y + corr;
        }
        double2 d;
        d = ld2(g.frhs ? fp.f[SUHMO_F_RES] : fp.f[SUHMO_F_RHS], idx); c.rhs0 = d.x; c.rhs1 = d.y;
        d = ld2(fp.f[SUHMO_F_B], idx); c.B0 = d.x; c.B1 = d.y;
        d = ld2(fp.f[SUHMO_F_PI], idx); c.Pi0 = d.x; c.Pi1 = d.y;
        d = ld2(fp.f[SUHMO_F_ZB], idx); c.zb0 = d.x; c.zb1 = d.y;
        d = ld2(fp.f[SUHMO_F_MASK], idx); c.mneg = (d.x < 0.0 ? 1 : 0) | (d.y < 0.0 ? 2 : 0);
        if (HAS_ALPHA) { d = ld2(fp.f[SUHMO_F_ACOEF], idx); c.a0 = d.x; c.a1 = d.y; }
        d = ld2(fp.f[SUHMO_F_BY], idx); c.byS0 = d.x; c.byS1 = d.y;
        d = ld2(fp.f[SUHMO_F_BY], idx + v.P); c.byN0 = d.x; c.byN1 = d.y;
        d = ld2(fp.f[SUHMO_F_BX], idx); c.bx0 = d.x; c.bx1 = d.y; c.bx2 = fp.f[SUHMO_F_BX][idx + 2];
        special = special || c.mneg != 0 || ph.cutOffbr > c.B0 || ph.cutOffbr > c.B1 || ph.maxOffbr < c.B0 || ph.maxOffbr < c.B1;
    };
    auto load = [&](const int k, PairCoef &c, bool &live) {
        live = false;
        int ly, lx;
        if (pair_pos(k, ly, lx)) {
            int i = gx0 + lx, j = gy0 + ly;
            if (inner) {
                live = true;
                const int idx = cidx(v, i, j);
                double2 p2 = ld2(pin, idx);
                ldcoef(c, p2, idx, i, j);
                lds[ly * LX + lx] = p2.x; lds[ly * LX + lx + 1] = p2.y;
                return;
            }
            const bool inx = perx || (i >= 0 && i < v.nx), iny = pery || (j >= 0 && j < v.ny) || (j < 0 && v.rk[0] && j >= g.jbeg - HY) || (j >= v.ny && v.rk[1]
                && j < g.jend + HY);
            const bool exi = inx || (i == -2 && v.cfx[0]) || (i == v.nx && v.cfx[1]);
            const bool exj = iny || (j == -1 && v.ext[0] && !v.rk[0]) || (j == v.ny && v.ext[1] && !v.rk[1]);
            double2 p2 = make_double2(0.0, 0.0);
            if (exi && exj) {
                live = inx && iny;
                if (perx) i = wrap(i, v.nx);
                if (pery) j = wrap(j, v.ny);
                const int idx = cidx(v, i, j);
                p2 = ld2(pin, idx);
            }
            if (live) ldcoef(c, p2, cidx(v, i, j), i, j);
            lds[ly * LX + lx] = p2.x; lds[ly * LX + lx + 1] = p2.y;
        }
    };
    TILE_EACH(load);
    constexpr bool PLAIN_OK = !HAS_ALPHA && !RST && !CHUNKED;
    const bool plain = PLAIN_OK && !__syncthreads_or(special ? 1 : 0) && ph.use_NL && !openW && !openE && !openS && !openN
                       && !v.cfx[0] && !v.cfx[1] && !(v.ext[0] && !v.rk[0]) && !(v.ext[1] && !v.rk[1]);
    if constexpr (!PLAIN_OK) __syncthreads();

    if (g.frhs) {
        const int ylo = openS ? 0 : 1, yhi = openN ? LY - 1 : LY - 2;
        auto mkrhs = [&](const int k, PairCoef &q_, const bool live) {
            int ly, lx;
            if (pair_pos(k, ly, lx) && live) {
                const int i = gx0 + lx, j = gy0 + ly;
                if (ly >= ylo && ly <= yhi) {
                    const double *row = lds + ly * LX;
                    double lo[2], cc[2];
#pragma unroll
                    for (int a = 0; a < 2; a++) {
                        const int x = lx + a, ii = i + a;
                        double c = row[x];
                        double w = row[x > 0 ? x - 1 : 0], e = row[x < LX - 1 ? x + 1 : LX - 1];
                        double s_ = lds[(ly > 0 ? ly - 1 : 0) * LX + x], n = lds[(ly < LY - 1 ? ly + 1 : LY - 1) * LX + x];
                        if (!perx) {
                            if (ii == 0 && !v.cfx[0]) w = (v.bct[0][0] == 0) ? v.two_v[0][0] - c : c + v.neu[0][0];
                            if (ii == v.nx - 1 && !v.cfx[1]) e = (v.bct[0][1] == 0) ? v.two_v[0][1] - c : c + v.neu[0][1];
                        }
                        if (!pery) {
                            if (j == 0 && !v.ext[0]) s_ = (v.bct[1][0] == 0) ? v.two_v[1][0] - c : c + v.neu[1][0];
                            if (j == v.ny - 1 && !v.ext[1]) n = (v.bct[1][1] == 0) ? v.two_v[1][1] - c : c + v.neu[1][1];
                        }
                        double nl, dnl;
                        nl_terms(ph, c, a ? q_.B1 : q_.B0, a ? q_.Pi1 : q_.Pi0, a ? q_.zb1 : q_.zb0, (q_.mneg >> a) & 1 ? -1.0 : 1.0, nl, dnl);
                        const double bxW = a ? q_.bx1 : q_.bx0, bxE = a ? q_.bx2 : q_.bx1;
                        double aterm = HAS_ALPHA ? v.alpha * (a ? q_.a1 : q_.a0) : v.alpha;
                        lo[a] = lofphi_cell(v, aterm, c, e, w, n, s_, bxE, bxW, a ? q_.byN1 : q_.byN0, a ? q_.byS1 : q_.byS0, nl);
                        cc[a] = c;
                    }
                    q_.rhs0 = 1.0 * q_.rhs0 + 1.0 * lo[0]; q_.rhs1 = 1.0 * q_.rhs1 + 1.0 * lo[1];
                    if (lx >= HX && lx < HX + TX && ly >= HY && ly < HY + TY && i < v.nx && j < g.jend) {
                        const int idx = cidx(v, i, j);
                        *reinterpret_cast<double2 *>(fp.f[SUHMO_F_LPHI] + idx) = make_double2(lo[0], lo[1]);
                        *reinterpret_cast<double2 *>(fp.f[SUHMO_F_RHS] + idx) = make_double2(q_.rhs0, q_.rhs1);
                        *reinterpret_cast<double2 *>(fp.f[SUHMO_F_PHIOLD] + idx) = make_double2(cc[0], cc[1]);
                    }
                }
            }
        };
        TILE_EACH(mkrhs);
        __syncthreads();
    }

#pragma unroll 1
    for (int chunk = 0; chunk < (CHUNKED ? g.chunks : 1); chunk++) {
    if (CHUNKED && chunk > 0 && (perx || pery)) {
        auto refresh = [&](const int k, const PairCoef &, const bool live) {
            int ly, lx;
            if (pair_pos(k, ly, lx) && live) {
                const int i = gx0 + lx, j = gy0 + ly;
                if (i < 0 || i >= v.nx || j < 0 || j >= v.ny) {
                    const int src = ((pery ? wrap(j, v.ny) : j) - gy0) * LX + ((perx ? wrap(i, v.nx) : i) - gx0);
                    const double a0 = lds[src], a1 = lds[src + 1];
                    lds[ly * LX + lx] = a0; lds[ly * LX + lx + 1] = a1;
                }
            }
        };
        TILE_EACH(refresh);
        __syncthreads();
    }
    if constexpr (PLAIN_OK) { if (plain) {
#pragma unroll 1
        for (int p = 0; p < 2 * S; p++) {
            const int lo = p + 1, xhi = LX - 2 - p, yhi = LY - 2 - p;
            const int a_pass = (gy0 + par + v.j0 + p) & 1;
#define TOUCH(c) asm volatile("" : "+v"(c.rhs0), "+v"(c.rhs1), "+v"(c.B0), "+v"(c.B1), "+v"(c.Pi0), "+v"(c.Pi1), "+v"(c.zb0), "+v"(c.zb1), \
                              "+v"(c.byS0), "+v"(c.byS1), "+v"(c.byN0), "+v"(c.byN1), "+v"(c.bx0), "+v"(c.bx1), "+v"(c.bx2))
            TOUCH(cf0); if constexpr (NK > 1) TOUCH(cf1); if constexpr (NK > 2) TOUCH(cf2); if constexpr (NK > 3) TOUCH(cf3); if constexpr (NK > 4) TOUCH(cf4);
#undef TOUCH
            double nv0 = 0.0, nv1 = 0.0, nv2 = 0.0, nv3 = 0.0, nv4 = 0.0;
            int ad0 = -1, ad1 = -1, ad2 = -1, ad3 = -1, ad4 = -1;
            auto upd = [&](const int k, const PairCoef &q_, auto a_tag, double &nv, int &ad) {
                constexpr int A = decltype(a_tag)::value;
                int ly, lx;
                const bool ok = pair_pos(k, ly, lx);
                if (!ok) { ly = par; lx = 0; }
                const int x = lx + A;
                const double *row = lds + ly * LX;
                double2 pr; double wl, er, s, n;
                pr = *reinterpret_cast<const double2 *>(row + lx); wl = row[lx - 1]; er = row[lx + 2]; s = row[x - LX]; n = row[x + LX];
                const double c = A ? pr.y : pr.x;
                const double w = A ? pr.x : wl, e = A ? er : pr.y;
                const double B = A ? q_.B1 : q_.B0;
                const double N = (A ? q_.Pi1 : q_.Pi0) - ph.rho_w_g * (c - (A ? q_.zb1 : q_.zb0));
                const double nl = -ph.A * B * N * N * N;
                const double dnl = 3.0 * ph.A * B * 1000.0 * ph.grav * N * N;
                const double bxW = A ? q_.bx1 : q_.bx0, bxE = A ? q_.bx2 : q_.bx1;
                const double byN = A ? q_.byN1 : q_.byN0, byS = A ? q_.byS1 : q_.byS0;
                const double aterm = HAS_ALPHA ? v.alpha * (A ? q_.a1 : q_.a0) : v.alpha;
                const double lofphi = lofphi_cell(v, aterm, c, e, w, n, s, bxE, bxW, byN, byS, nl);
                const double lam = lambda_cell(v, aterm, bxE, bxW, byN, byS);
                const double denom = 1.0e-16 + lam + dnl;
                const double cnew = c + ((A ? q_.rhs1 : q_.rhs0) - lofphi) / denom;
                const bool in = ok && x >= lo && x <= xhi && ly >= lo && ly <= yhi;
                nv = cnew;
                ad = in ? ly * LX + x : -1;
            };
            if (a_pass) {
                using A1 = std::integral_constant<int, 1>;
                upd(0, cf0, A1(), nv0, ad0); if constexpr (NK > 1) upd(1, cf1, A1(), nv1, ad1); if constexpr (NK > 2) upd(2, cf2, A1(), nv2, ad2);
                if constexpr (NK > 3) upd(3, cf3, A1(), nv3, ad3); if constexpr (NK > 4) upd(4, cf4, A1(), nv4, ad4);
            } else {
                using A0 = std::integral_constant<int, 0>;
                upd(0, cf0, A0(), nv0, ad0); if constexpr (NK > 1) upd(1, cf1, A0(), nv1, ad1); if constexpr (NK > 2) upd(2, cf2, A0(), nv2, ad2);
                if constexpr (NK > 3) upd(3, cf3, A0(), nv3, ad3); if constexpr (NK > 4) upd(4, cf4, A0(), nv4, ad4);
            }
            lds[ad0] = nv0; if constexpr (NK > 1) lds[ad1] = nv1; if constexpr (NK > 2) lds[ad2] = nv2;
            if constexpr (NK > 3) lds[ad3] = nv3; if constexpr (NK > 4) lds[ad4] = nv4;
            __syncthreads();
        }
    } }
    if (!(PLAIN_OK && plain))
#pragma unroll 1
    for (int p = 0; p < 2 * S; p++) {
        const int xlo = openW ? 0 : p + 1, xhi = openE ? LX - 1 : LX - 2 - p;
        const int ylo = openS ? 0 : p + 1, yhi = openN ? LY - 1 : LY - 2 - p;
        auto relax = [&](const int k, const PairCoef &q_, const bool live) {
            int ly, lx;
            if (pair_pos(k, ly, lx) && live) {
                const int j = gy0 + ly;
                const int a = (j + v.j0 + p) & 1;
                const int x = lx + a, i = gx0 + x;
                if (x >= xlo && x <= xhi && ly >= ylo && ly <= yhi) {
                    const double *row = lds + ly * LX;
                    double c = row[x];
                    double w = row[x > 0 ? x - 1 : 0], e = row[x < LX - 1 ? x + 1 : LX - 1];
                    double s = lds[(ly > 0 ? ly - 1 : 0) * LX + x], n = lds[(ly < LY - 1 ? ly + 1 : LY - 1) * LX + x];
                    if (!perx) {
                        if (i == 0 && !v.cfx[0]) w = (v.bct[0][0] == 0) ? v.two_v[0][0] - c : c + v.neu[0][0];
                        if (i == v.nx - 1 && !v.cfx[1]) e = (v.bct[0][1] == 0) ? v.two_v[0][1] - c : c + v.neu[0][1];
                    }
                    if (!pery) {
                        if (j == 0 && !v.ext[0]) s = (v.bct[1][0] == 0) ? v.two_v[1][0] - c : c + v.neu[1][0];
                        if (j == v.ny - 1 && !v.ext[1]) n = (v.bct[1][1] == 0) ? v.two_v[1][1] - c : c + v.neu[1][1];
                    }
                    double nl, dnl;
                    nl_terms(ph, c, a ? q_.B1 : q_.B0, a ? q_.Pi1 : q_.Pi0, a ? q_.zb1 : q_.zb0, (q_.mneg >> a) & 1 ? -1.0 : 1.0, nl, dnl);
                    const double bxW = a ? q_.bx1 : q_.bx0, bxE = a ? q_.bx2 : q_.bx1;
                    const double byN = a ? q_.byN1 : q_.byN0, byS = a ? q_.byS1 : q_.byS0;
                    double aterm = HAS_ALPHA ? v.alpha * (a ? q_.a1 : q_.a0) : v.alpha;
                    double lofphi = lofphi_cell(v, aterm, c, e, w, n, s, bxE, bxW, byN, byS, nl);
                    double lam = lambda_cell(v, aterm, bxE, bxW, byN, byS);
                    double denom = 1.0e-16 + lam + dnl;
                    lds[ly * LX + x] = c + ((a ? q_.rhs1 : q_.rhs0) - lofphi) / denom;
                }
            }
        };
        TILE_EACH(relax);
        __syncthreads();
    }
    }

    const int oi1 = (tx * TX + TX < v.nx) ? tx * TX + TX : v.nx, oj1 = (tj0 + TY < g.jend) ? tj0 + TY : g.jend;
    const int wi0 = tx * TX - ((tx == 0 && v.cfx[0]) ? 1 : 0), wi1 = oi1 + ((oi1 == v.nx && v.cfx[1]) ? 1 : 0);
    const int wj0 = tj0 - ((ty == 0 && v.ext[0] && !v.rk[0]) ? 1 : 0), wj1 = oj1 + ((oj1 == v.ny && v.ext[1] && !v.rk[1]) ? 1 : 0);
    auto store = [&](const int k, const PairCoef &q_, const bool) {
        int ly, lx;
        if (pair_pos(k, ly, lx)) {
            const int i = gx0 + lx, j = gy0 + ly;
            if (inner && !RST) {
                if (lx >= HX && lx < HX + TX && ly >= HY && ly < HY + TY)
                    *reinterpret_cast<double2 *>(pout + cidx(v, i, j)) = make_double2(lds[ly * LX + lx], lds[ly * LX + lx + 1]);
                return;
            }
            if (j >= wj0 && j < wj1) {
                const bool m0 = i >= wi0 && i < wi1, m1 = i + 1 >= wi0 && i + 1 < wi1;
                if (m0 && m1) *reinterpret_cast<double2 *>(pout + cidx(v, i, j)) = make_double2(lds[ly * LX + lx], lds[ly * LX + lx + 1]);
                else if (m0) pout[cidx(v, i, j)] = lds[ly * LX + lx];
                else if (m1) pout[cidx(v, i + 1, j)] = lds[ly * LX + lx + 1];
            }
            if (lx >= HX && lx < HX + TX && ly >= HY && ly < HY + TY && i < v.nx && j >= 0 && j < v.ny) {
                if constexpr (RST) {
                    const double *row = lds + ly * LX;
#pragma unroll
                    for (int a = 0; a < 2; a++) {
                        const int x = lx + a, ii = i + a;
                        double c = row[x], w = row[x - 1], e = row[x + 1];
                        double s_ = lds[(ly - 1) * LX + x], n = lds[(ly + 1) * LX + x];
                        if (!perx) {
                            if (ii == 0 && !v.cfx[0]) w = (v.bct[0][0] == 0) ? v.two_v[0][0] - c : c + v.neu[0][0];
                            if (ii == v.nx - 1 && !v.cfx[1]) e = (v.bct[0][1] == 0) ? v.two_v[0][1] - c : c + v.neu[0][1];
                        }
                        if (!pery) {
                            if (j == 0 && !v.ext[0]) s_ = (v.bct[1][0] == 0) ? v.two_v[1][0] - c : c + v.neu[1][0];
                            if (j == v.ny - 1 && !v.ext[1]) n = (v.bct[1][1] == 0) ? v.two_v[1][1] - c : c + v.neu[1][1];
                        }
                        double nl, dnl;
                        nl_terms(ph, c, a ? q_.B1 : q_.B0, a ? q_.Pi1 : q_.Pi0, a ? q_.zb1 : q_.zb0, (q_.mneg >> a) & 1 ? -1.0 : 1.0, nl, dnl);
                        const double bxW = a ? q_.bx1 : q_.bx0, bxE = a ? q_.bx2 : q_.bx1;
                        double aterm = HAS_ALPHA ? v.alpha * (a ? q_.a1 : q_.a0) : v.alpha;
                        double lofphi = lofphi_cell(v, aterm, c, e, w, n, s_, bxE, bxW, a ? q_.byN1 : q_.byN0, a ? q_.byS1 : q_.byS0, nl);
                        lq[(ly - HY) * TX + (lx - HX) + a] = ((a ? q_.rhs1 : q_.rhs0) - lofphi) / 4.0;
                    }
                }
            }
        }
    };
    TILE_EACH(store);
#undef TILE_EACH
    if constexpr (RST) {
        __syncthreads();
        if (t < TX * TY / 4) {
            const int cx = t % (TX / 2), cy = t / (TX / 2);
            const int i = tx * TX + 2 * cx, j = tj0 + 2 * cy;
            if (i < v.nx && j >= 0 && j < v.ny) {
                const double *q0 = lq + (2 * cy) * TX + 2 * cx, *p0 = lds + (HY + 2 * cy) * LX + HX + 2 * cx;
                double acc = 0.0, accp = 0.0;
                acc = acc + q0[0]; accp = accp + p0[0] / 4.0;
                acc = acc + q0[1]; accp = accp + p0[1] / 4.0;
                acc = acc + q0[TX]; accp = accp + p0[LX] / 4.0;
                acc = acc + q0[TX + 1]; accp = accp + p0[LX + 1] / 4.0;
                const int ic = ((j >> 1) + g.rgy) * g.rP + SUHMO_XOFF + (i >> 1);
                g.rres[ic] = acc; g.rphi[ic] = accp;
            }
        }
    }
}
#define TILE_KERNEL_ATTRS(S, T, RST) __launch_bounds__((TileThreads<S, T, RST>::NT)) __attribute__((amdgpu_waves_per_eu((TileThreads<S, T, RST>::NT == 384 ? 3 : 2))))
template <int S, int T, bool HAS_ALPHA, bool RST = false, bool CHUNKED = false>
__global__ TILE_KERNEL_ATTRS(S, T, RST) void k_gsrb_tile(DV v, FP fp, const double *__restrict__ pin, double *__restrict__ pout, suhmo_phys_t ph, TileGeom g)
{
    d_gsrb_tile<S, T, HAS_ALPHA, RST, CHUNKED>(v, fp, pin, pout, ph, g);
}
template <int S, int T, bool HAS_ALPHA, bool CHUNKED>
__global__ TILE_KERNEL_ATTRS(S, T, false) void k_gsrb_tile_b(BatchTab t, BatchTab c, BatchSel sel, TileGeom g, int prolong)
{
    const int k = batch_member(sel);
    const DV v = t.dv[k];
    const FP fp = batch_fp(t, k);
    const suhmo_phys_t ph = t.ph[k];
    if (prolong) { const FP fc = batch_fp(c, k); g.pc = fc.f[SUHMO_F_PHI]; g.pco = fc.f[SUHMO_F_PHIOLD]; }
    d_gsrb_tile<S, T, HAS_ALPHA, false, CHUNKED>(v, fp, fp.f[SUHMO_F_PHI], fp.f[SUHMO_F_PHI2], ph, g);
}
static bool tile_ok(const suhmo_level *L, const Depth &D)
{
    const DV &v = D.v;
    if (!L->gsrb_tile || !suhmo_batch_tile_ok(v)) return false;
    if ((v.rk[0] || v.rk[1]) && (!L->ex || !L->tile_strips || L->desc.nx_global > 0 || v.gy < 10 || v.ny < 10)) return false;
    return true;
}
bool suhmo_batch_tile_ok(const DV &v)
{
    if (v.nx & 1) return false;
    if (v.per[1] && (v.ny & 1)) return false;
    if ((v.per[0] && v.cfx[0] != v.cfx[1]) || (v.per[1] && v.ext[0] != v.ext[1])) return false;
    return true;
}

typedef void (*TileFn)(DV, FP, const double *, double *, suhmo_phys_t, TileGeom);
struct TileKernel { int key; TileFn fn; int NT, TX, TY; };
constexpr int tile_key(int S, int T, bool alpha, bool rst, bool chunked) { return S | alpha << 4 | rst << 5 | chunked << 6 | T << 8; }
#define TK(S, T, A, R, C) {tile_key(S, T, A, R, C), k_gsrb_tile<S, T, A, R, C>, TileThreads<S, T, R>::NT, TileShape<T, R>::TX, TileShape<T, R>::TY}
#define TK_ST(S, T, C) TK(S, T, false, false, C), TK(S, T, true, false, C), TK(S, T, false, true, C), TK(S, T, true, true, C)
static const TileKernel tile_kernels[] = {
    TK_ST(4, 16, false), TK_ST(4, 32, false), TK_ST(2, 16, false), TK_ST(2, 32, false), TK_ST(1, 16, false), TK_ST(1, 32, false),
    TK_ST(4, 16, true), TK_ST(4, 32, true),
};
#undef TK_ST
#undef TK
static const TileKernel *tile_kernel(int S, int T, bool alpha, bool rst, bool chunked)
{
    const int key = tile_key(S, T, alpha, rst, chunked);
    for (const TileKernel &k : tile_kernels) if (k.key == key) return &k;
    return nullptr;
}
static int launch_tile(suhmo_level *L, int depth, const RelaxStep &s, hipStream_t st)
{
    Depth &D = L->d[depth];
    const DV &v = D.v;
    const TileKernel *k = tile_kernel(s.S, s.T, v.alpha != 0.0, s.rst, s.chunks > 1);
    if (!k) { suhmo_set_error("internal: a tile relaxation step without a kernel"); return -4; }
    if (!D.phi_alt) {
        HIPCHK(hipMalloc(&D.phi_alt, D.elems * sizeof(double)));
        HIPCHK(hipMemsetAsync(D.phi_alt, 0, D.elems * sizeof(double), st));
    }
    TileGeom g;
    g.jbeg = v.rk[0] ? -s.adv : 0; g.jend = v.ny + (v.rk[1] ? s.adv : 0);
    g.ntx = (v.nx + k->TX - 1) / k->TX; g.nty = (g.jend - g.jbeg + k->TY - 1) / k->TY;
    g.pc = g.pco = nullptr; g.Pc = g.gyc = 0;
    g.rres = g.rphi = nullptr; g.rP = g.rgy = 0;
    if (s.rst) {
        Depth &C = L->d[depth + 1];
        g.rres = C.fp.f[SUHMO_F_RES]; g.rphi = C.fp.f[SUHMO_F_PHI]; g.rP = C.v.P; g.rgy = C.v.gy;
        C.phi_fresh = 0;
    }
    if (s.prolong) {
        Depth &C = L->d[depth + 1];
        g.pc = C.fp.f[SUHMO_F_PHI]; g.pco = C.fp.f[SUHMO_F_PHIOLD]; g.Pc = C.v.P; g.gyc = C.v.gy;
        D.prolong_pending = 0;
    }
    g.chunks = s.chunks;
    g.order = L->tile_order;
    g.frhs = 0;
    if (s.frhs) {
        if (!suhmo_field(L, depth, SUHMO_F_LPHI) || !suhmo_field(L, depth, SUHMO_F_PHIOLD)) return -2;
        g.frhs = 1; D.rhs_pending = 0; L->frhs_tile++;
    }
    hipLaunchKernelGGL(k->fn, dim3(g.ntx * g.nty), dim3(k->NT), 0, st, v, D.fp, (const double *)D.fp.f[SUHMO_F_PHI], D.phi_alt, L->ph, g);
    { std::swap(D.fp.f[SUHMO_F_PHI], D.phi_alt); suhmo_fp_changed(); }
    return 0;
}

static int pick_K(const suhmo_level *L, const Depth &D, bool tile, int remaining)
{
    int variant = L->gsrb_variant;
    if (variant < 0) {
        const long cells = (long)D.v.nx * D.v.ny;
        variant = (cells >= (long)L->fused_min_cells) ? 2 : 0;
        if (tile && cells < L->tile_max_cells) variant = 0;
    }
    if (variant >= 2 && remaining >= 2 && fused_ok(L, D, 2)) return 2;
    if (variant >= 1 && fused_ok(L, D, 1)) return 1;
    return 0;
}
static int prolong_halo_rows(const suhmo_level *L, int depth)
{
    const Depth &D = L->d[depth], &C = L->d[depth + 1];
    int R = D.phi_fresh < 2 * C.phi_fresh ? D.phi_fresh : 2 * C.phi_fresh;
    return R & ~1;
}
static int pending(const Depth &D)
{
    return (D.prolong_pending ? ABSORB_PROLONG : 0) | (D.rhs_pending ? ABSORB_RHS : 0) | (D.bcoef_pending ? ABSORB_BCOEF : 0);
}
static bool has_halo(const suhmo_level *L, const DV &v) { return L->ex && (v.ext[0] || v.ext[1]); }

static RelaxStep relax_step(const suhmo_level *L, int depth, int left, int tail, bool restricts, int F, bool settled, int absorb)
{
    const Depth &D = L->d[depth];
    const DV &v = D.v;
    const bool ext = has_halo(L, v), stored = v.ext[0] || v.ext[1];
    const long cells = (long)v.nx * v.ny;
    const bool can_restrict = restricts && L->fused_restrict && depth + 1 < L->ndepth && !(v.ny & 1) && !(v.j0 & 1);
    const bool tile = tile_ok(L, D);
    const int K = pick_K(L, D, tile, left);
    RelaxStep s{};
    if (K == 0 && tile) {
        const TileStep t = plan_tile_step(left, L->tile_s, L->tile_chunks && !ext ? plan_single_tile(L->tile_t, v.nx, v.ny) : 0, plan_tile_edge(L->tile_t, cells));
        s.rst = can_restrict && (L->tile_restrict == 1 || (L->tile_restrict == 2 && ext)) && t.S * t.chunks == left;
        s.need = ext ? 2 * t.S + (s.rst ? 1 : 0) : 0;
        if (!(settled && F < s.need)) {
            s.path = STEP_TILE; s.S = t.S; s.chunks = t.chunks; s.T = t.T; s.done = t.S * t.chunks;
            s.frhs = absorb & ABSORB_RHS; s.prolong = absorb & ABSORB_PROLONG;
            s.adv = ext ? plan_halo_advance(F, s.need, 2 * (left - t.S) + tail, v.gy - s.need, true) : 0;
            return s;
        }
        s = RelaxStep{}; s.shallow = true;
    }
    if (K == 0) { s.path = STEP_COLOUR; s.done = 1; s.need = ext ? 1 : 0; return s; }
    s.path = STEP_STREAM; s.K = s.done = K; s.NT = plan_stream_threads(L->fused_nt, cells);
    s.masked = !(suhmo_mask_clean(L, depth) && v.alpha == 0.0);
    s.prolong = absorb & ABSORB_PROLONG;
    const bool variants = K == 2 && s.NT == 64 && v.alpha == 0.0, last = K == left;
    s.zbu = variants && !s.masked && !stored && suhmo_zb_uniform(L, depth);
    s.rst = can_restrict && variants && last && (!stored || (ext && L->desc.nx_global == 0 && v.gy >= 5));
    s.rout = L->resout_armed && depth == 0 && !restricts && variants && last && (!stored || ext) && L->desc.nx_global == 0 && !(absorb & ABSORB_RHS);
    if (ext && settled && F < 2 * K + 1) s.rst = s.rout = false;
    s.need = ext ? 2 * K + (s.rst || s.rout ? 1 : 0) : 0;
    const bool plain = variants && !s.rst && !s.rout;
    s.frhs = (absorb & ABSORB_RHS) && plain;
    s.bcf = absorb == ABSORB_BCOEF && plain && depth == 0 && !stored && !s.masked;
    s.adv = ext ? plan_halo_advance(F, s.need, (absorb & ABSORB_RHS) ? F : 2 * (left - K) + tail, v.gy - s.need, s.rst) : 0;
    return s;
}

bool suhmo_gsrb_streams(const suhmo_level *L, int depth) { return relax_step(L, depth, 2, 0, false, 0, false, 0).path == STEP_STREAM; }

bool suhmo_gsrb_can_fuse_rhs(suhmo_level *L, int depth, int sweeps, bool rhs_local)
{
    const Depth &D = L->d[depth];
    if (sweeps < 1 || !L->fas_rhs_in_relax) return false;
    const RelaxStep s = relax_step(L, depth, sweeps, 0, false, 0, false, ABSORB_RHS);
    if (!s.frhs) return false;
    const bool strip = D.v.rk[0] || D.v.rk[1];
    if (s.path == STEP_TILE) return !strip && (L->fas_rhs_in_relax & 1);
    if (!(L->fas_rhs_in_relax & 2) || sweeps < 4) return false;
    if (!(D.v.ext[0] || D.v.ext[1])) return true;
    return strip && L->ex && rhs_local && L->desc.nx_global == 0 && D.phi_fresh >= D.v.gy && D.v.gy >= 2 * s.K + 1 && D.v.ny >= D.v.gy;
}
bool suhmo_gsrb_can_fuse_bcoef(suhmo_level *L, int sweeps)
{
    if (!L->bcoef_in_relax || L->ex) return false;
    const RelaxStep s = relax_step(L, 0, sweeps, 0, false, 0, false, ABSORB_BCOEF | pending(L->d[0]));
    return s.bcf && sweeps >= 3;
}
bool suhmo_gsrb_can_overlap_avg(const suhmo_level *L)
{
    return L->avg_overlap && !L->mask_capturing && !L->prof_on && !L->ex && !L->agg && !L->ex_begin && !L->ex_end && !L->ipc;
}
static int avg_fork(suhmo_level *L, hipStream_t st)
{
    if (!L->astream) {
        HIPCHK(hipStreamCreateWithFlags(&L->astream, hipStreamNonBlocking));
        HIPCHK(hipEventCreateWithFlags(&L->aev[0], hipEventDisableTiming)); HIPCHK(hipEventCreateWithFlags(&L->aev[1], hipEventDisableTiming));
    }
    HIPCHK(hipEventRecord(L->aev[0], st));
    HIPCHK(hipStreamWaitEvent(L->astream, L->aev[0], 0));
    int rc = suhmo_average_operator_all(L, L->bcoef_nd, L->astream); if (rc) return rc;
    HIPCHK(hipEventRecord(L->aev[1], L->astream));
    L->avg_flying = 1; L->avg_overlap_count++;
    return 0;
}
int suhmo_avg_join(suhmo_level *L, hipStream_t st)
{
    if (!L->avg_flying) return 0;
    L->avg_flying = 0;
    HIPCHK(hipStreamWaitEvent(st, L->aev[1], 0));
    return 0;
}
void suhmo_avg_release(suhmo_level *L)
{
    if (!L->astream) return;
    (void)hipStreamDestroy(L->astream); (void)hipEventDestroy(L->aev[0]); (void)hipEventDestroy(L->aev[1]);
    L->astream = nullptr; L->aev[0] = L->aev[1] = nullptr; L->avg_flying = 0;
}
bool suhmo_gsrb_can_fuse_prolong(suhmo_level *L, int depth, int sweeps)
{
    const Depth &D = L->d[depth];
    if (sweeps < 1 || depth + 1 >= L->ndepth) return false;
    const RelaxStep s = relax_step(L, depth, sweeps, 0, false, 0, false, ABSORB_PROLONG);
    if (!s.prolong) return false;
    const bool stored = D.v.ext[0] || D.v.ext[1];
    if (s.path == STEP_STREAM && stored && !L->ex) return false;
    const bool halo = s.path == STEP_TILE ? (D.v.rk[0] || D.v.rk[1]) : stored;
    return !halo || prolong_halo_rows(L, depth) >= s.need;
}

int suhmo_launch_gsrb(suhmo_level *L, int depth, int sweeps, int tail, hipStream_t st, int *restricted)
{
    Depth &D = L->d[depth];
    const bool ext = has_halo(L, D.v);
    if (restricted) *restricted = 0;
    int F = !ext ? 0 : D.prolong_pending ? prolong_halo_rows(L, depth) : D.phi_fresh;
    if (depth > 0) { int rc = suhmo_avg_join(L, st); if (rc) return rc; }
    for (int it = 0; it < sweeps;) {
        const int left = sweeps - it, absorb = pending(D);
        const bool settled = !ext || D.prolong_pending;
        RelaxStep s = relax_step(L, depth, left, tail, restricted != nullptr, F, settled, absorb);
        bool flying = false;
        if (!settled && s.path != STEP_COLOUR && F < s.need) {
            flying = s.path == STEP_STREAM && (L->overlap_halo == 2 || (L->overlap_halo && (L->rccl || L->ipc))) && D.v.ny >= 6 * s.need;
            if (flying) {
                if (!L->xstream) {
                    HIPCHK(hipStreamCreateWithFlags(&L->xstream, hipStreamNonBlocking));
                    HIPCHK(hipEventCreateWithFlags(&L->xev[0], hipEventDisableTiming)); HIPCHK(hipEventCreateWithFlags(&L->xev[1], hipEventDisableTiming));
                }
                HIPCHK(hipEventRecord(L->xev[0], st));
                HIPCHK(hipStreamWaitEvent(L->xstream, L->xev[0], 0));
            }
            int rc = suhmo_ensure_phi_halo(L, depth, s.need, flying ? L->xstream : st); if (rc) return rc;
            if (flying) HIPCHK(hipEventRecord(L->xev[1], L->xstream));
            F = D.phi_fresh;
            s = relax_step(L, depth, left, tail, restricted != nullptr, F, true, absorb);
        }
        if (s.absorbs() != absorb || (ext && s.path != STEP_COLOUR && F < s.need)) {
            suhmo_set_error("internal: a relaxation launch that takes %d of what is pending (%d) or reads %d halo rows of %d", s.absorbs(), absorb, s.need, F);
            return -4;
        }
        if (s.shallow) L->strip_tile_shallow++;
        ProfEv pe{};
        const bool prof = L->prof_on && depth == 0;
        if (prof) {
            HIPCHK(hipEventCreate(&pe.a)); HIPCHK(hipEventCreate(&pe.b));
            HIPCHK(hipEventRecord(pe.a, st));
        }
        int rc = 0;
        if (s.path == STEP_TILE) {
            rc = launch_tile(L, depth, s, st);
            if (!rc && ext) { L->strip_tile++; if (s.rst) L->strip_tile_rst++; }
        } else if (s.path == STEP_COLOUR) {
            for (int pass = 0; pass < 2; pass++) {
                if (ext && F < 1) {
                    if ((rc = suhmo_ensure_phi_halo(L, depth, 1, st))) return rc;
                    F = D.phi_fresh;
                }
                const int E = ext ? plan_halo_advance(F, 1, 2 * left - (pass + 1) + tail, L->desc.nx_global > 0 ? 0 : D.v.gy - 1, false) : 0;
                if ((rc = launch_simple(L, depth, pass, E, st))) return rc;
                if (ext) { F = E; D.phi_fresh = F; L->strip_colour++; }
            }
        } else {
            if (flying) {
                rc = launch_fused(L, depth, s, st, 1);
                if (rc < 0) return rc;
                HIPCHK(hipStreamWaitEvent(st, L->xev[1], 0));
                if (rc == 1) rc = launch_fused(L, depth, s, st, 0); else { rc = launch_fused(L, depth, s, st, 2); L->overlapped++; }
            } else rc = launch_fused(L, depth, s, st);
            if (!rc && ext) { L->strip_stream++; if (s.rst) L->strip_stream_rst++; }
        }
        if (rc) return rc;
        if (s.rst) *restricted = 1;
        if (s.rout) { L->resout_done = 1; L->resout_count++; }
        if (ext && s.path != STEP_COLOUR) { F = s.adv; D.phi_fresh = F; }
        if (prof) {
            HIPCHK(hipEventRecord(pe.b, st));
            pe.cells = (long)D.v.nx * D.v.ny * s.done;
            pe.restricts = s.bcf ? 2 : s.rst ? 1 : 0;
            L->prof.push_back(pe);
        }
        if (s.bcf) { rc = L->avg_fork ? avg_fork(L, st) : suhmo_average_operator_all(L, L->bcoef_nd, st); if (rc) return rc; }
        it += s.done;
    }
    HIPCHK(hipGetLastError());
    return 0;
}

typedef void (*TileBFn)(BatchTab, BatchTab, BatchSel, TileGeom, int);
struct TileBKernel { int key; TileBFn fn; int NT; };
#define TB(S, T, A, C) {tile_key(S, T, A, false, C), k_gsrb_tile_b<S, T, A, C>, TileThreads<S, T, false>::NT}
#define TB_ST(S, T, C) TB(S, T, false, C), TB(S, T, true, C)
static const TileBKernel tile_b_kernels[] = {
    TB_ST(4, 16, false), TB_ST(4, 32, false), TB_ST(2, 16, false), TB_ST(2, 32, false), TB_ST(1, 16, false), TB_ST(1, 32, false),
    TB_ST(4, 16, true), TB_ST(4, 32, true),
};
#undef TB_ST
#undef TB
static const TileBKernel *tile_b_kernel(int S, int T, bool alpha, bool chunked)
{
    const int key = tile_key(S, T, alpha, false, chunked);
    for (const TileBKernel &k : tile_b_kernels) if (k.key == key) return &k;
    return nullptr;
}
int suhmo_batch_gsrb_tile(const BatchTab &t, const BatchTab *coarse, const DV *vc, const BatchSel &sel, const DV &v, int S, int T, int chunks, bool frhs, bool prolong,
                          bool has_alpha, int order, hipStream_t st)
{
    if (sel.n <= 0) return 0;
    TileGeom g;
    g.jbeg = 0; g.jend = v.ny;
    g.ntx = (v.nx + T - 1) / T; g.nty = (v.ny + T - 1) / T;
    g.pc = g.pco = nullptr; g.Pc = g.gyc = 0;
    g.rres = g.rphi = nullptr; g.rP = g.rgy = 0;
    const TileBKernel *k = tile_b_kernel(S, T, has_alpha, chunks > 1);
    if (!k || (chunks > 1 && g.ntx * g.nty != 1)) { suhmo_set_error("internal: a tile relaxation step of a batch without a kernel"); return -4; }
    if (prolong) {
        if (!coarse || !vc) { suhmo_set_error("internal: fused prolongation without the coarse tables"); return -4; }
        g.Pc = vc->P; g.gyc = vc->gy;
    }
    g.chunks = chunks; g.order = order; g.frhs = frhs ? 1 : 0;
    hipLaunchKernelGGL(k->fn, dim3(g.ntx * g.nty, 1, sel.n), dim3(k->NT), 0, st, t, coarse ? *coarse : t, sel, g, (int)prolong);
    HIPCHK(hipGetLastError());
    return 0;
}
```

### suhmo_amd/csrc/suhmo_level.hip

```cpp
#include "suhmo_hier.h"
#include "suhmo_level_int.h"
#include "suhmo_reduce.h"
#include <algorithm>
#include <cstdarg>
#include <cmath>
#include <initializer_list>

static thread_local char g_err[512] = "";
void suhmo_set_error(const char *fmt, ...)
{
    va_list ap; va_start(ap, fmt); vsnprintf(g_err, sizeof(g_err), fmt, ap); va_end(ap);
}
extern "C" const char *suhmo_last_error(void) { return g_err; }
#include <atomic>
#include <chrono>
#include <map>
#include <mutex>
namespace {
std::atomic<int> g_timer_mode{-1};
std::mutex g_timer_mu;
struct TimerRec { long count = 0; double total = 0.0; };
std::map<std::string, TimerRec> g_timers;
inline double now_s() { return std::chrono::duration<double>(std::chrono::steady_clock::now().time_since_epoch()).count(); }
inline int timer_mode()
{
    int m = g_timer_mode.load(std::memory_order_relaxed);
    if (m < 0) { const char *e = getenv("SUHMO_TIMERS"); m = e ? atoi(e) : 0; g_timer_mode.store(m); }
    return m;
}
}
SuhmoTimer::SuhmoTimer(const char *n) : name(n), t0(0.0), mode(timer_mode())
{
    if (!mode) return;
    if (mode >= 2) (void)hipDeviceSynchronize();
    t0 = now_s();
}
SuhmoTimer::~SuhmoTimer()
{
    if (!mode) return;
    if (mode >= 2) (void)hipDeviceSynchronize();
    double dt = now_s() - t0;
    std::lock_guard<std::mutex> lk(g_timer_mu);
    TimerRec &r = g_timers[name];
    r.count++; r.total += dt;
}
extern "C" int suhmo_timers_enable(int mode) { g_timer_mode.store(mode < 0 ? 0 : mode); return 0; }
extern "C" int suhmo_timers_reset(void) { std::lock_guard<std::mutex> lk(g_timer_mu); g_timers.clear(); return 0; }
extern "C" long suhmo_timers_report(char *buf, long size)
{
    std::vector<std::pair<std::string, TimerRec>> v;
    { std::lock_guard<std::mutex> lk(g_timer_mu); v.assign(g_timers.begin(), g_timers.end()); }
    std::sort(v.begin(), v.end(), [](const auto &a, const auto &b) { return a.second.total > b.second.total; });
    std::string out;
    char line[256];
    for (auto &e : v) {
        snprintf(line, sizeof(line), "%-56s %10ld %14.6f %12.2f\n", e.first.c_str(), e.second.count, e.second.total, 1e6 * e.second.total / std::max(1L, e.second.count));
        out += line;
    }
    if (buf && size > 0) { long n = std::min<long>(size - 1, (long)out.size()); memcpy(buf, out.data(), n); buf[n] = 0; }
    return (long)out.size() + 1;
}

extern "C" int suhmo_device_count(void)
{
    int n = 0;
    if (hipGetDeviceCount(&n) != hipSuccess) return 0;
    return n;
}

static bool boxes_coarsenable(const std::vector<int> &b, int r)
{
    for (size_t k = 0; k < b.size(); k += 4)
        if (b[k] % r || b[k + 1] % r || (b[k + 2] + 1) % r || (b[k + 3] + 1) % r) return false;
    return true;
}

static void make_dv(DV &v, const suhmo_level_desc_t &d, int depth)
{
    int c = 1 << depth;
    memset(&v, 0, sizeof(v));
    v.nx = d.nx / c; v.ny = d.ny / c;
    v.gy = d.halo_rows < 1 ? 1 : d.halo_rows;
    v.rows = v.ny + 2 * v.gy;
    v.P = ((v.nx + 2 * SUHMO_XOFF + 15) / 16) * 16;
    v.j0 = d.j0 / c; v.nyg = d.ny_global / c;
    v.i0 = d.i0 / c; v.nxg = (d.nx_global > 0 ? d.nx_global : d.nx) / c;
    v.dx = d.dx * c; v.dy = d.dy * c;
    v.rdx = 1.0 / (v.dx * v.dx); v.rdy = 1.0 / (v.dy * v.dy);
    v.fdx = 1.0 / v.dx; v.fdy = 1.0 / v.dy;
    v.alpha = d.alpha; v.beta = d.beta;
    for (int dir = 0; dir < 2; dir++) {
        v.per[dir] = d.bc.periodic[dir];
        for (int s = 0; s < 2; s++) {
            v.bct[dir][s] = d.bc.type[dir][s];
            v.two_v[dir][s] = 2.0 * d.bc.value[dir][s];
            double isign = s == 0 ? -1.0 : 1.0;
            v.neu[dir][s] = isign * (dir == 0 ? v.dx : v.dy) * d.bc.value[dir][s];
        }
    }
    bool whole = (d.j0 == 0 && d.ny == d.ny_global);
    v.ext[0] = (!whole) && (d.j0 > 0 || d.bc.periodic[1]);
    v.ext[1] = (!whole) && (d.j0 + d.ny < d.ny_global || d.bc.periodic[1]);
    v.cfx[0] = v.i0 > 0 || (v.per[0] && v.nx < v.nxg);
    v.cfx[1] = v.i0 + v.nx < v.nxg || (v.per[0] && v.nx < v.nxg);
    if (d.nx_global > 0) {
        const int pj0 = d.patch_ny > 0 ? d.patch_j0 : d.j0, pj1 = d.patch_ny > 0 ? d.patch_j0 + d.patch_ny : d.j0 + d.ny;
        v.rk[0] = d.j0 > pj0; v.rk[1] = d.j0 + d.ny < pj1;
    } else { v.rk[0] = v.ext[0]; v.rk[1] = v.ext[1]; }
}

static std::atomic<unsigned long> g_fp_epoch{1};
void suhmo_fp_changed() { g_fp_epoch.fetch_add(1, std::memory_order_relaxed); }
unsigned long suhmo_fp_epoch() { return g_fp_epoch.load(std::memory_order_relaxed); }

double *suhmo_field(suhmo_level *L, int depth, int field)
{
    Depth &D = L->d[depth];
    if (!D.fp.f[field]) {
        double *p = nullptr;
        if (L->stub) return nullptr;
        if (hipMalloc(&p, D.elems * sizeof(double)) != hipSuccess) return nullptr;
        (void)hipMemset(p, 0, D.elems * sizeof(double));
        D.fp.f[field] = p;
        suhmo_fp_changed();
    }
    return D.fp.f[field];
}

static int level_storage(suhmo_level *L);
int suhmo_level_create_(suhmo_level_t **out, const suhmo_level_desc_t *desc, bool stub);
extern "C" int suhmo_level_create(suhmo_level_t **out, const suhmo_level_desc_t *desc) { return suhmo_level_create_(out, desc, false); }
int suhmo_level_materialize_(suhmo_level *L) { return L->stub ? level_storage(L) : 0; }
int suhmo_level_create_(suhmo_level_t **out, const suhmo_level_desc_t *desc, bool stub)
{
    ARG(out && desc);
    ARG(desc->nx >= 2 && desc->ny >= 2 && desc->dx > 0 && desc->dy > 0);
    ARG(desc->ny_global >= desc->ny && desc->j0 >= 0 && desc->j0 + desc->ny <= desc->ny_global);
    ARG(desc->i0 >= 0 && (desc->nx_global == 0 ? desc->i0 == 0 : desc->i0 + desc->nx <= desc->nx_global));
    ARG(desc->i0 % 2 == 0);
    ARG(desc->patch_ny == 0 || (desc->nx_global > 0 && desc->patch_j0 <= desc->j0 && desc->j0 + desc->ny <= desc->patch_j0 + desc->patch_ny));
    ARG((long)(desc->nx + 64) * (long)(desc->ny + 2 * (desc->halo_rows < 1 ? 1 : desc->halo_rows)) < (1L << 31));
    int ndev = 0;
    HIPCHK(hipGetDeviceCount(&ndev));
    if (ndev <= 0) { suhmo_set_error("no HIP device: the product path has no CPU fallback"); return -3; }
    ARG(desc->device >= 0 && desc->device < ndev);
    HIPCHK(hipSetDevice(desc->device));
    suhmo_level *L = new suhmo_level();
    L->desc = *desc; L->ph = desc->phys; L->device = desc->device; L->batch_owned = 0;
    L->ex = nullptr; L->ar = nullptr; L->ar2 = nullptr; L->ard = nullptr; L->user = nullptr; L->ex_begin = nullptr; L->ex_end = nullptr; L->rccl = nullptr;
        L->ipc = nullptr; L->ipc_owner = 0; L->faces_deferred = 0; L->gap = nullptr; L->gap_dt = 0.0; L->prof_on = 0; L->gsrb_variant = -1; L->fused_hc = 0;
    L->bcoef_fused = 1;
    L->bcoef_tile_x = 62;
    L->fused_nt = 64;
    L->fused_restrict = 1;
    L->gsrb_tile = 1; L->tile_t = 0; L->tile_s = 4;
    L->tile_max_cells = 3000000;
    L->fas_rhs_in_relax = 3;
    L->tile_chunks = 1;
    L->tile_order = 2; L->tile_restrict = 0;
    L->tile_strips = 1;
    L->overlap_halo = 1; L->xstream = nullptr; L->xev[0] = L->xev[1] = nullptr; L->overlapped = 0;
    L->strips_rhs_local = 1;
    L->fas_rhs_fused = 1;
    L->agg_min_cells = 100000; L->agg_depth = 0; L->agg_world = 1; L->agg_rank = 0; L->agg = nullptr; L->ag = nullptr; L->ag_user = nullptr;
    L->agg_send = L->agg_recv = nullptr; L->agg_cap = 0; L->agg_gathers = 0; L->agg_static_stale = 0;
    L->frhs_stream = L->frhs_tile = 0;
    L->strip_tile = L->strip_tile_rst = L->strip_tile_shallow = L->strip_colour = L->strip_stream = L->strip_stream_rst = L->strip_prolong_unfused = 0;
    L->bcoef_in_relax = 1; L->bcoef_nd = 0; L->bcoef_in_relax_count = 0;
    L->avg_overlap = 1; L->avg_fork = L->avg_flying = 0; L->avg_overlap_count = 0; L->astream = nullptr; L->aev[0] = L->aev[1] = nullptr;
    L->resout_np = 0;
    L->resout_req = L->resout_armed = L->resout_done = 0; L->resout_rhs = nullptr; L->resout_count = 0; L->resid_in_relax = 1;
    L->graph_max_cells = 1500000; L->gstream = nullptr; L->vgraph_replays = 0; memset(L->vgraph_seen, 0, sizeof(L->vgraph_seen));
    L->fused_min_cells = 1000000;
    L->skip_mask = 1; L->mask_known = 1; L->poll_readback = 1; L->zb_known = 1;
    L->bottom_solver = 0; L->bottom_one_launch_max_cells = 16384;
    L->bottom_ctr = nullptr; L->bottom_host_iters = L->bottom_host_solves = 0;
    {
        struct IntKnob { const char *env; int suhmo_level::*field; };
        struct LongKnob { const char *env; long suhmo_level::*field; };
        static const IntKnob ints[] = {
            {"SUHMO_GSRB_VARIANT", &suhmo_level::gsrb_variant}, {"SUHMO_FUSED_HC", &suhmo_level::fused_hc}, {"SUHMO_BCOEF_FUSED", &suhmo_level::bcoef_fused},
            {"SUHMO_BCOEF_TILE_X", &suhmo_level::bcoef_tile_x}, {"SUHMO_FUSED_NT", &suhmo_level::fused_nt}, {"SUHMO_OVERLAP_HALO", &suhmo_level::overlap_halo},
            {"SUHMO_STRIPS_RHS_LOCAL", &suhmo_level::strips_rhs_local}, {"SUHMO_FAS_RHS_FUSED", &suhmo_level::fas_rhs_fused},
            {"SUHMO_RESID_IN_RELAX", &suhmo_level::resid_in_relax}, {"SUHMO_BCOEF_IN_RELAX", &suhmo_level::bcoef_in_relax}, {"SUHMO_TILE_STRIPS", &suhmo_level::tile_strips}, {"SUHMO_TILE_CHUNKS", &suhmo_level::tile_chunks},
            {"SUHMO_TILE_RESTRICT", &suhmo_level::tile_restrict}, {"SUHMO_TILE_ORDER", &suhmo_level::tile_order}, {"SUHMO_FAS_RHS_IN_RELAX", &suhmo_level::fas_rhs_in_relax},
            {"SUHMO_TILE_S", &suhmo_level::tile_s}, {"SUHMO_GSRB_TILE", &suhmo_level::gsrb_tile}, {"SUHMO_TILE_T", &suhmo_level::tile_t},
            {"SUHMO_FUSED_RESTRICT", &suhmo_level::fused_restrict}, {"SUHMO_SKIP_MASK", &suhmo_level::skip_mask}, {"SUHMO_MASK_KNOWN", &suhmo_level::mask_known}, {"SUHMO_ZB_KNOWN", &suhmo_level::zb_known},
            {"SUHMO_POLL_READBACK", &suhmo_level::poll_readback}, {"SUHMO_AVG_OVERLAP", &suhmo_level::avg_overlap}};
        static const LongKnob longs[] = {
            {"SUHMO_AGG_MIN_CELLS", &suhmo_level::agg_min_cells}, {"SUHMO_TILE_MAX_CELLS", &suhmo_level::tile_max_cells},
            {"SUHMO_GRAPH_MAX_CELLS", &suhmo_level::graph_max_cells}, {"SUHMO_FUSED_MIN_CELLS", &suhmo_level::fused_min_cells},
            {"SUHMO_BOTTOM_ONE_LAUNCH_MAX_CELLS", &suhmo_level::bottom_one_launch_max_cells}};
        for (const IntKnob &k : ints) if (const char *e = getenv(k.env)) L->*(k.field) = atoi(e);
        for (const LongKnob &k : longs) if (const char *e = getenv(k.env)) L->*(k.field) = atol(e);
        L->fas_rhs_fused = L->fas_rhs_fused != 0;
        if (L->tile_order < 0 || L->tile_order > 2) L->tile_order = 0;
        if (L->tile_t != 16 && L->tile_t != 32) L->tile_t = 0;
    }
    if (desc->boxes && desc->nbox > 0) {
        L->boxes.assign(desc->boxes, desc->boxes + 4 * (size_t)desc->nbox);
    } else {
        int mb = desc->max_box > 0 ? desc->max_box : 64;
        for (int bj = 0; bj * mb < desc->ny; bj++)
            for (int bi = 0; bi * mb < desc->nx; bi++) {
                int lo0 = desc->i0 + bi * mb, lo1 = desc->j0 + bj * mb;
                int hi0 = std::min(lo0 + mb, desc->i0 + desc->nx) - 1, hi1 = std::min(lo1 + mb, desc->j0 + desc->ny) - 1;
                int b[4] = {lo0, lo1, hi0, hi1};
                L->boxes.insert(L->boxes.end(), b, b + 4);
            }
    }
    L->desc.boxes = nullptr;
    L->desc.nbox = (int)(L->boxes.size() / 4);
    {
        long cells = 0;
        for (size_t k = 0; k < L->boxes.size(); k += 4) {
            const int *b = &L->boxes[k];
            if (b[0] < desc->i0 || b[2] >= desc->i0 + desc->nx || b[1] < desc->j0 || b[3] >= desc->j0 + desc->ny || b[0] > b[2] || b[1] > b[3]) {
                suhmo_set_error("box %zu outside the strip", k / 4); delete L; return -1;
            }
            cells += (long)(b[2] - b[0] + 1) * (b[3] - b[1] + 1);
        }
        if (cells != (long)desc->nx * desc->ny) { suhmo_set_error("boxes do not tile the level"); delete L; return -1; }
    }
    L->ndepth = 1;
    for (int dep = 1; dep < SUHMO_MAXDEPTH; dep++) {
        if (!boxes_coarsenable(L->boxes, (1 << dep) * 2)) break;
        if ((desc->j0 % (1 << dep)) || (desc->ny_global % (1 << dep))) break;
        if ((desc->i0 % (2 << dep)) || (desc->nx_global % (1 << dep))) break;
        L->ndepth = dep + 1;
    }
    for (int dep = 0; dep < L->ndepth; dep++) {
        Depth &D = L->d[dep];
        make_dv(D.v, L->desc, dep);
        D.elems = (size_t)D.v.P * (size_t)(D.v.rows + 1);
        D.nbox = L->desc.nbox;
        memset(&D.fp, 0, sizeof(D.fp));
        D.phi_alt = nullptr; D.prolong_pending = 0; D.rhs_pending = 0; D.bcoef_pending = 0; D.phi_fresh = 0;
        D.zb_state = SUHMO_ZB_UNKNOWN; D.zb_value = 0.0;
    }
    L->scratch = nullptr; L->scratch_elems = 0; L->hscratch = nullptr; L->hscratch_dev = nullptr; L->hseq = 0;
    L->mask_epoch = 0; L->maskflag_epoch = 0; L->mask_reported = 0; L->coarse_mask_ok = 0;
    L->mask_state = SUHMO_MASK_UNKNOWN; L->mask_version = 1; L->mask_scan_version = 0; L->mask_scan_pending = 0; L->mask_capturing = 0;
    L->mask_scan_captured = 0; L->mask_view = 0; L->mask_scan_errors = 0;
    L->mask_host = nullptr; L->mask_ev = nullptr; L->mask_scans = L->bcoef_unmasked = L->relax_unmasked = 0;
    L->zb_off = 0; L->zb_version = 1; L->zb_scan_version = 0; L->zb_scan_pending = 0; L->zb_scan_errors = 0;
    L->zb_dev = L->zb_host = nullptr; L->zb_ev = nullptr; L->zb_scans = 0; memset(L->relax_zb_uniform, 0, sizeof(L->relax_zb_uniform));
    L->stub = 1;
    if (!stub) { int rc = level_storage(L); if (rc) { suhmo_level_destroy(L); return rc; } }
    *out = L;
    return 0;
}
static int level_storage(suhmo_level *L)
{
    static const int eager[] = {SUHMO_F_PHI, SUHMO_F_RHS, SUHMO_F_ACOEF, SUHMO_F_B, SUHMO_F_PI, SUHMO_F_ZB,
                                SUHMO_F_MASK, SUHMO_F_BX, SUHMO_F_BY, SUHMO_F_RES, SUHMO_F_LPHI};
    HIPCHK(hipSetDevice(L->device));
    L->stub = 0;
    for (int dep = 0; dep < L->ndepth; dep++) {
        for (int f : eager) {
            if (dep == 0 && f == SUHMO_F_LPHI) continue;
            if (!suhmo_field(L, dep, f)) { suhmo_set_error("hipMalloc failed (depth %d field %d)", dep, f); return -2; }
        }
        if (dep > 0) { suhmo_field(L, dep, SUHMO_F_PHIOLD); suhmo_field(L, dep, SUHMO_F_CORR); }
    }
    L->scratch_elems = 16384;
    HIPCHK(hipMalloc(&L->scratch, L->scratch_elems * sizeof(double)));
    HIPCHK(hipMemset(L->scratch, 0, L->scratch_elems * sizeof(double)));
    HIPCHK(hipHostMalloc(&L->hscratch, SUHMO_HSCRATCH_DOUBLES * sizeof(double), hipHostMallocMapped | hipHostMallocCoherent));
    memset(L->hscratch, 0, SUHMO_HSCRATCH_DOUBLES * sizeof(double));
    L->mask_host = (unsigned *)(L->hscratch + SUHMO_HSCRATCH_MASK);
    L->zb_host = (unsigned long long *)(L->hscratch + SUHMO_HSCRATCH_ZB);
    HIPCHK(hipMalloc(&L->zb_dev, 2 * SUHMO_MAXDEPTH * sizeof(unsigned long long)));
    if (L->poll_readback && hipHostGetDevicePointer((void **)&L->hscratch_dev, L->hscratch, 0) != hipSuccess) { L->hscratch_dev = nullptr; L->poll_readback = 0; (void)hipGetLastError(); }
    return 0;
}

extern "C" int suhmo_level_destroy(suhmo_level_t *L)
{
    if (!L) return 0;
    if (L->batch_owned) { suhmo_set_error("this level is a member of a batch: suhmo_batch_destroy frees it"); return -1; }
    (void)hipSetDevice(L->device);
    (void)hipDeviceSynchronize();
    if (L->rccl) (void)suhmo_level_detach_rccl(L);
    if (L->gap) { (void)suhmo_level_destroy(L->gap); L->gap = nullptr; }
    suhmo_ipc_release(L);
    suhmo_agg_release(L);
    suhmo_level_drop_graphs(L);
    for (int dep = 0; dep < L->ndepth; dep++)
        for (int f = 0; f < SUHMO_F_COUNT; f++)
            if (L->d[dep].fp.f[f]) (void)hipFree(L->d[dep].fp.f[f]);
    for (int dep = 0; dep < L->ndepth; dep++)
        if (L->d[dep].phi_alt) (void)hipFree(L->d[dep].phi_alt);
    for (auto &pe : L->prof) { (void)hipEventDestroy(pe.a); (void)hipEventDestroy(pe.b); }
    if (L->xstream) { (void)hipStreamDestroy(L->xstream); (void)hipEventDestroy(L->xev[0]); (void)hipEventDestroy(L->xev[1]); }
    if (L->scratch) (void)hipFree(L->scratch);
    if (L->bal_buf) (void)hipFree(L->bal_buf);
    if (L->vol_buf) (void)hipFree(L->vol_buf);
    if (L->wb_buf) (void)hipFree(L->wb_buf);
    if (L->bottom_ctr) (void)hipFree(L->bottom_ctr);
    suhmo_tagmap_release(L->tags);
    if (L->mask_ev) (void)hipEventDestroy(L->mask_ev);
    if (L->zb_ev) (void)hipEventDestroy(L->zb_ev);
    if (L->zb_dev) (void)hipFree(L->zb_dev);
    if (L->hscratch) (void)hipHostFree(L->hscratch);
    delete L;
    return 0;
}

__global__ __launch_bounds__(256) void k_zb_scan(DV v, const double *__restrict__ zb, unsigned long long *__restrict__ out)
{
    const long long first = __double_as_longlong(zb[cidx(v, 0, 0)]);
    bool differs = false;
    for_valid_cells(v, [&](int i, int j) { differs = differs || __double_as_longlong(zb[cidx(v, i, j)]) != first; });
    if (differs) out[0] = 1ull;
    if (blockIdx.x == 0 && blockIdx.y == 0 && threadIdx.x == 0 && threadIdx.y == 0) out[1] = (unsigned long long)first;
}
void suhmo_zb_poll(suhmo_level *L)
{
    if (!L->zb_scan_pending) return;
    const hipError_t e = hipEventQuery(L->zb_ev);
    if (e == hipErrorNotReady) { (void)hipGetLastError(); return; }
    L->zb_scan_pending = 0;
    if (e != hipSuccess) { (void)hipGetLastError(); L->zb_scan_errors++; return; }
    if (L->zb_scan_version != L->zb_version) return;
    const volatile unsigned long long *h = L->zb_host;
    for (int d = 0; d < L->ndepth; d++) {
        const unsigned long long bits = h[2 * d + 1];
        L->d[d].zb_state = h[2 * d] ? SUHMO_ZB_VARYING : SUHMO_ZB_UNIFORM;
        memcpy(&L->d[d].zb_value, &bits, sizeof(double));
    }
}
int suhmo_zb_scan_if_due(suhmo_level *L, hipStream_t st)
{
    const DV &v0 = L->d[0].v;
    if (!L->zb_known || L->zb_off || L->zb_scan_pending || L->zb_scan_errors >= 3 || !L->zb_host || !L->zb_dev || L->d[0].zb_state != SUHMO_ZB_UNKNOWN) return 0;
    if (L->ex || L->desc.nx_global != 0 || v0.ext[0] || v0.ext[1] || L->batch_owned) return 0;
    bool streams = false;
    for (int d = 0; d < L->ndepth && !streams; d++) streams = suhmo_gsrb_streams(L, d);
    if (!streams) return 0;
    if (!L->zb_ev) HIPCHK(hipEventCreateWithFlags(&L->zb_ev, hipEventDisableTiming));
    const size_t bytes = 2 * (size_t)L->ndepth * sizeof(unsigned long long);
    HIPCHK(hipMemsetAsync(L->zb_dev, 0, bytes, st));
    for (int d = 0; d < L->ndepth; d++) {
        const DV &v = L->d[d].v;
        hipLaunchKernelGGL(k_zb_scan, reduce_grid(v.nx, v.ny, CAP_LEVEL), BLK2D, 0, st, v, (const double *)L->d[d].fp.f[SUHMO_F_ZB], L->zb_dev + 2 * d);
    }
    HIPCHK(hipGetLastError());
    HIPCHK(hipMemcpyAsync(L->zb_host, L->zb_dev, bytes, hipMemcpyDeviceToHost, st));
    HIPCHK(hipEventRecord(L->zb_ev, st));
    L->zb_scan_pending = 1; L->zb_scan_version = L->zb_version; L->zb_scans++;
    return 0;
}

static int remake_views(suhmo_level *L)
{
    for (int dep = 0; dep < L->ndepth; dep++) make_dv(L->d[dep].v, L->desc, dep);
    suhmo_level_drop_graphs(L);
    return 0;
}
extern "C" int suhmo_level_set_alpha_beta(suhmo_level_t *L, double alpha, double beta)
{
    ARG(L);
    L->desc.alpha = alpha; L->desc.beta = beta;
    if (L->agg) { int rc = suhmo_level_set_alpha_beta(L->agg, alpha, beta); if (rc) return rc; }
    return remake_views(L);
}
extern "C" int suhmo_level_set_bc(suhmo_level_t *L, const suhmo_bc_t *bc)
{
    ARG(L && bc);
    for (int d = 0; d < 2; d++)
        if ((bc->periodic[d] != 0) != (L->desc.bc.periodic[d] != 0)) { suhmo_set_error("setBC cannot change the periodicity of the domain"); return -1; }
    for (int d = 0; d < 2; d++) for (int s = 0; s < 2; s++) ARG(bc->type[d][s] == 0 || bc->type[d][s] == 1);
    L->desc.bc = *bc;
    if (L->agg) { int rc = suhmo_level_set_bc(L->agg, bc); if (rc) return rc; }
    return remake_views(L);
}

static long *option_slot_long(suhmo_level *L, const char *key)
{
    if (!strcmp(key, "fused_min_cells")) return &L->fused_min_cells;
    if (!strcmp(key, "tile_max_cells")) return &L->tile_max_cells;
    if (!strcmp(key, "graph_max_cells")) return &L->graph_max_cells;
    if (!strcmp(key, "agg_min_cells")) return &L->agg_min_cells;
    return nullptr;
}
static int *option_slot_int(suhmo_level *L, const char *key)
{
    static const struct { const char *k; int suhmo_level::*m; } tab[] = {
        {"gsrb_variant", &suhmo_level::gsrb_variant}, {"fused_hc", &suhmo_level::fused_hc}, {"bcoef_fused", &suhmo_level::bcoef_fused}, {"bcoef_tile_x", &suhmo_level::bcoef_tile_x},
        {"fused_nt", &suhmo_level::fused_nt}, {"fused_restrict", &suhmo_level::fused_restrict}, {"strips_rhs_local", &suhmo_level::strips_rhs_local},
        {"tile_strips", &suhmo_level::tile_strips}, {"overlap_halo", &suhmo_level::overlap_halo}, {"skip_mask", &suhmo_level::skip_mask}, {"mask_known", &suhmo_level::mask_known}, {"zb_known", &suhmo_level::zb_known}, {"tile_chunks",
            &suhmo_level::tile_chunks}, {"tile_order", &suhmo_level::tile_order}, {"tile_restrict", &suhmo_level::tile_restrict}, {"fas_rhs_in_relax",
            &suhmo_level::fas_rhs_in_relax}, {"resid_in_relax", &suhmo_level::resid_in_relax}, {"bcoef_in_relax", &suhmo_level::bcoef_in_relax}, {"fas_rhs_fused", &suhmo_level::fas_rhs_fused},
        {"avg_overlap", &suhmo_level::avg_overlap}, {"tile_s", &suhmo_level::tile_s}, {"gsrb_tile", &suhmo_level::gsrb_tile}, {"tile_t", &suhmo_level::tile_t}, {"poll_readback", &suhmo_level::poll_readback}};
    for (const auto &e : tab) if (!strcmp(key, e.k)) return &(L->*(e.m));
    return nullptr;
}
extern "C" int suhmo_level_set_option(suhmo_level_t *L, const char *key, long value)
{
    ARG(L && key);
    if (!strcmp(key, "bottom_solver")) {
        if (value != 0 && value != 1) { suhmo_set_error("bottom_solver: 0 (bottom relaxes only) or 1 (RelaxSolver)"); return -1; }
        return suhmo_bottom_configure(L, (int)value, L->bottom_one_launch_max_cells);
    }
    if (!strcmp(key, "bottom_one_launch_max_cells")) {
        if (value < 0) { suhmo_set_error("bottom_one_launch_max_cells: >= 0"); return -1; }
        return suhmo_bottom_configure(L, L->bottom_solver, value);
    }
    if (!strcmp(key, "track_old_volume")) {
        if (value != 0 && value != 1) { suhmo_set_error("track_old_volume: 0 or 1"); return -1; }
        L->track_old_volume = (int)value; return 0;
    }
    if (long *p = option_slot_long(L, key)) {
        *p = value; suhmo_level_drop_graphs(L);
        if (!strcmp(key, "agg_min_cells")) return suhmo_agg_setup(L);
        return 0;
    }
    if (int *p = option_slot_int(L, key)) {
        if (!strcmp(key, "tile_t") && value != 0 && value != 16 && value != 32) { suhmo_set_error("tile_t: 0 (by size), 16 or 32"); return -1; }
        if (!strcmp(key, "fused_nt") && value != 64 && value != 256) { suhmo_set_error("fused_nt: 64 or 256"); return -1; }
        if (!strcmp(key, "poll_readback") && value && !L->hscratch_dev) { suhmo_set_error("poll_readback: no device address of the host slot"); return -1; }
        *p = (int)value; suhmo_level_drop_graphs(L); return 0;
    }
    suhmo_set_error("unknown option '%s'", key);
    return -1;
}
extern "C" int suhmo_level_get_option(const suhmo_level_t *L, const char *key, long *value)
{
    ARG(L && key && value);
    if (long *p = option_slot_long(const_cast<suhmo_level *>(L), key)) { *value = *p; return 0; }
    if (int *p = option_slot_int(const_cast<suhmo_level *>(L), key)) { *value = *p; return 0; }
    if (!strcmp(key, "overlapped_launches")) { *value = L->overlapped; return 0; }
    if (!strcmp(key, "agg_gathers")) { *value = L->agg_gathers; return 0; }
    if (!strcmp(key, "rhs_in_streaming_launches")) { *value = L->frhs_stream; return 0; }
    if (!strcmp(key, "rhs_in_tile_launches")) { *value = L->frhs_tile; return 0; }
    {
        static const struct { const char *k; long suhmo_level::*m; } strip[] = {
            {"strip_tile_launches", &suhmo_level::strip_tile}, {"strip_tile_restricting_launches", &suhmo_level::strip_tile_rst},
            {"strip_tile_shallow_halo_fallbacks", &suhmo_level::strip_tile_shallow}, {"strip_colour_passes", &suhmo_level::strip_colour},
            {"strip_streaming_launches", &suhmo_level::strip_stream}, {"strip_streaming_restricting_launches", &suhmo_level::strip_stream_rst},
            {"strip_unfused_prolongations", &suhmo_level::strip_prolong_unfused}};
        for (const auto &e : strip) if (!strcmp(key, e.k)) { *value = L->*(e.m); return 0; }
    }
    if (!strcmp(key, "residual_in_relax_launches")) { *value = L->resout_count; return 0; }
    if (!strcmp(key, "bcoef_in_relax_launches")) { *value = L->bcoef_in_relax_count; return 0; }
    if (!strcmp(key, "avg_overlap_launches")) { *value = L->avg_overlap_count; return 0; }
    if (!strcmp(key, "mask_scans")) { *value = L->mask_scans; return 0; }
    if (!strcmp(key, "mask_state")) { *value = L->mask_state; return 0; }
    if (!strcmp(key, "bcoef_unmasked_launches")) { *value = L->bcoef_unmasked; return 0; }
    if (!strcmp(key, "relax_unmasked_launches")) { *value = L->relax_unmasked; return 0; }
    {
        if (!strcmp(key, "zb_scans")) { *value = L->zb_scans; return 0; }
        const bool st = !strncmp(key, "zb_state", 8), nl = !strncmp(key, "relax_zb_uniform_launches", 25);
        const char *rest = st ? key + 8 : nl ? key + 25 : nullptr;
        if (rest && !*rest) {
            *value = st ? L->d[0].zb_state : 0;
            for (int d = 0; nl && d < L->ndepth; d++) *value += L->relax_zb_uniform[d];
            return 0;
        }
        if (rest && rest[0] == '_' && rest[1] == 'd' && rest[2] >= '0' && rest[2] <= '9') {
            const int d = atoi(rest + 2);
            if (d >= L->ndepth) { suhmo_set_error("option '%s': the level has %d depths", key, L->ndepth); return -1; }
            *value = st ? L->d[d].zb_state : L->relax_zb_uniform[d];
            return 0;
        }
    }
    if (!strcmp(key, "vcycle_graph_replays")) { *value = L->vgraph_replays; return 0; }
    if (!strcmp(key, "bottom_solver")) { *value = L->bottom_solver; return 0; }
    if (!strcmp(key, "track_old_volume")) { *value = L->track_old_volume; return 0; }
    if (!strcmp(key, "bottom_one_launch_max_cells")) { *value = L->bottom_one_launch_max_cells; return 0; }
    if (!strcmp(key, "bottom_solver_iterations")) { *value = suhmo_bottom_counter(L, 0); return 0; }
    if (!strcmp(key, "bottom_solves_one_launch")) { *value = suhmo_bottom_counter(L, 1); return 0; }
    if (!strcmp(key, "bottom_solves_host_loop")) { *value = suhmo_bottom_counter(L, 2); return 0; }
    suhmo_set_error("unknown option '%s'", key);
    return -1;
}

extern "C" int suhmo_level_num_depths(const suhmo_level_t *L) { return L ? L->ndepth : -1; }
extern "C" int suhmo_level_synchronize(suhmo_level_t *L, suhmo_stream_t s)
{
    ARG(L);
    HIPCHK(hipStreamSynchronize((hipStream_t)s));
    return 0;
}
extern "C" int suhmo_level_set_hooks(suhmo_level_t *L, suhmo_exchange_fn ex, suhmo_allreduce_max_fn ar, void *user)
{
    ARG(L);
    L->ex = ex; L->ar = ar; L->ar2 = nullptr; L->ard = nullptr; L->user = user; L->ex_begin = nullptr; L->ex_end = nullptr;
    return 0;
}
void suhmo_level_share_transport(suhmo_level *dst, const suhmo_level *src)
{
    dst->ex = src->ex; dst->ar = src->ar; dst->ar2 = src->ar2; dst->ard = src->ard; dst->user = src->user;
    dst->ex_begin = src->ex_begin; dst->ex_end = src->ex_end; dst->ipc = src->ipc;
}
extern "C" int suhmo_level_set_allgather(suhmo_level_t *L, suhmo_allgather_fn fn, void *user)
{
    ARG(L);
    HIPCHK(hipSetDevice(L->device));
    L->ag = fn; L->ag_user = user;
    return suhmo_agg_setup(L);
}
extern "C" int suhmo_level_agglomerated_depth(const suhmo_level_t *L) { return L ? L->agg_depth : -1; }
extern "C" int suhmo_level_set_reduce_hook(suhmo_level_t *L, suhmo_allreduce_fn fn)
{
    ARG(L);
    L->ar2 = fn;
    return 0;
}

extern "C" int suhmo_level_exchange(suhmo_level_t *L, int depth, int field, suhmo_stream_t s)
{
    ARG(L); ARG(depth >= 0 && depth < L->ndepth); ARG(field >= 0 && field < SUHMO_F_COUNT);
    const DV &v = L->d[depth].v;
    if (L->ex && (v.ext[0] || v.ext[1])) {
        if (!suhmo_field(L, depth, field)) return -2;
        int rc = L->ex(L->user, L, depth, &field, 1, s);
        if (!rc && field == SUHMO_F_PHI) L->d[depth].phi_fresh = suhmo_halo_rows(v);
        if (field == SUHMO_F_MASK) suhmo_mask_halo_written(L);
        if (field == SUHMO_F_ZB) suhmo_zb_written(L);
        return rc;
    }
    return 0;
}
extern "C" int suhmo_level_halo_info(const suhmo_level_t *L, int depth, int *halo_rows, int *ext_lo, int *ext_hi, int *nx, int *ny)
{
    ARG(L); ARG(depth >= 0 && depth < L->ndepth);
    const DV &v = L->d[depth].v;
    if (halo_rows) *halo_rows = v.gy;
    if (ext_lo) *ext_lo = v.ext[0];
    if (ext_hi) *ext_hi = v.ext[1];
    if (nx) *nx = v.nx;
    if (ny) *ny = v.ny;
    return 0;
}
extern "C" int suhmo_level_phi_halo_fresh(const suhmo_level_t *L, int depth)
{
    if (!L || depth < 0 || depth >= L->ndepth) return -1;
    return L->d[depth].phi_fresh;
}


extern "C" int suhmo_level_field_view(suhmo_level_t *L, int depth, int field, double **base, long *pitch, long *origin)
{
    CHECK_DF(L, depth, field);
    double *p = suhmo_field(L, depth, field);
    if (!p) { suhmo_set_error("field allocation failed"); return -2; }
    if (field == SUHMO_F_MASK) { L->mask_view = 1; suhmo_mask_written(L); suhmo_level_drop_graphs(L); }
    if (field == SUHMO_F_ZB) { L->zb_off = 1; suhmo_zb_written(L); suhmo_level_drop_graphs(L); }
    if (depth == 0 && (field == SUHMO_F_BX || field == SUHMO_F_BY)) suhmo_faces_made(L);
    if (base) *base = p;
    if (pitch) *pitch = L->d[depth].v.P;
    if (origin) *origin = cidx(L->d[depth].v, 0, 0);
    return 0;
}

static int copy2d(suhmo_level *L, int depth, int field, double *host, long hpitch, int i0, int j0, int ni, int nj,
                  bool to_canvas, bool on_device, hipStream_t st)
{
    if (ni <= 0 || nj <= 0) return 0;
    double *p = suhmo_field(L, depth, field);
    if (!p) { suhmo_set_error("field allocation failed"); return -2; }
    const DV &v = L->d[depth].v;
    double *c = p + cidx(v, i0, j0);
    hipMemcpyKind kind = to_canvas ? (on_device ? hipMemcpyDeviceToDevice : hipMemcpyHostToDevice)
                                   : (on_device ? hipMemcpyDeviceToDevice : hipMemcpyDeviceToHost);
    if (to_canvas)
        HIPCHK(hipMemcpy2DAsync(c, (size_t)v.P * 8, host, (size_t)hpitch * 8, (size_t)ni * 8, nj, kind, st));
    else
        HIPCHK(hipMemcpy2DAsync(host, (size_t)hpitch * 8, c, (size_t)v.P * 8, (size_t)ni * 8, nj, kind, st));
    return 0;
}

static int field_io(suhmo_level *L, int depth, int field, double *buf, int ghosted, int on_device, bool set, hipStream_t st)
{
    const DV &v = L->d[depth].v;
    int rc;
    if (is_xface(field)) rc = copy2d(L, depth, field, buf, v.nx + 1, 0, 0, v.nx + 1, v.ny, set, on_device, st);
    else if (is_yface(field)) rc = copy2d(L, depth, field, buf, v.nx, 0, 0, v.nx, v.ny + 1, set, on_device, st);
    else if (ghosted) rc = copy2d(L, depth, field, buf, v.nx + 2, -1, -1, v.nx + 2, v.ny + 2, set, on_device, st);
    else rc = copy2d(L, depth, field, buf, v.nx, 0, 0, v.nx, v.ny, set, on_device, st);
    if (rc) return rc;
    if (!on_device) HIPCHK(hipStreamSynchronize(st));
    return 0;
}

extern "C" int suhmo_level_set_field(suhmo_level_t *L, int depth, int field, const double *src, int ghosted,
                                     int on_device, suhmo_stream_t s)
{
    CHECK_DF(L, depth, field); ARG(src);
    HIPCHK(hipSetDevice(L->device));
    if (field == SUHMO_F_PHI) phi_changed(L, depth);
    if (field == SUHMO_F_MASK) suhmo_mask_written(L);
    if (field == SUHMO_F_ZB) suhmo_zb_written(L);
    if (depth == 0 && (field == SUHMO_F_BX || field == SUHMO_F_BY)) suhmo_faces_made(L);
    return field_io(L, depth, field, (double *)src, ghosted, on_device, true, (hipStream_t)s);
}
extern "C" int suhmo_level_get_field(suhmo_level_t *L, int depth, int field, double *dst, int ghosted,
                                     int on_device, suhmo_stream_t s)
{
    CHECK_DF(L, depth, field); ARG(dst);
    HIPCHK(hipSetDevice(L->device));
    return field_io(L, depth, field, dst, ghosted, on_device, false, (hipStream_t)s);
}

static void box_region(const suhmo_level *L, int depth, int field, int ibox, int r[4])
{
    const int *b = &L->boxes[4 * (size_t)ibox];
    int c = 1 << depth;
    r[0] = b[0] / c - L->d[depth].v.i0; r[1] = b[1] / c - L->d[depth].v.j0;
    r[2] = (b[2] + 1) / c - 1 - L->d[depth].v.i0; r[3] = (b[3] + 1) / c - 1 - L->d[depth].v.j0;
    if (is_xface(field)) r[2] += 1;
    if (is_yface(field)) r[3] += 1;
}

extern "C" int suhmo_level_put_box(suhmo_level_t *L, int depth, int field, int ibox, const double *fab,
                                   int flo0, int flo1, int fhi0, int fhi1, int with_domain_ghosts, suhmo_stream_t s)
{
    CHECK_DF(L, depth, field); ARG(fab); ARG(ibox >= 0 && ibox < L->desc.nbox);
    HIPCHK(hipSetDevice(L->device));
    hipStream_t st = (hipStream_t)s;
    const DV &v = L->d[depth].v;
    if (field == SUHMO_F_PHI) phi_changed(L, depth);
    if (field == SUHMO_F_MASK) suhmo_mask_written(L);
    if (field == SUHMO_F_ZB) suhmo_zb_written(L);
    if (depth == 0 && (field == SUHMO_F_BX || field == SUHMO_F_BY)) suhmo_faces_made(L);
    int r[4]; box_region(L, depth, field, ibox, r);
    int j0 = v.j0;
    flo0 -= v.i0; fhi0 -= v.i0;
    const bool patch = L->desc.nx_global > 0;
    long fp = fhi0 - flo0 + 1;
    ARG(flo0 <= r[0] && fhi0 >= r[2] && flo1 - j0 <= r[1] && fhi1 - j0 >= r[3]);
    double *h = (double *)fab;
    int rc = copy2d(L, depth, field, h + (long)(r[1] + j0 - flo1) * fp + (r[0] - flo0), fp, r[0], r[1],
                    r[2] - r[0] + 1, r[3] - r[1] + 1, true, false, st);
    if (rc) return rc;
    if (with_domain_ghosts && !is_face(field)) {
        if (r[0] == 0 && flo0 <= -1)
            rc |= copy2d(L, depth, field, h + (long)(r[1] + j0 - flo1) * fp + (-1 - flo0), fp, -1, r[1], 1, r[3] - r[1] + 1, true, false, st);
        if (r[2] == v.nx - 1 && fhi0 >= v.nx)
            rc |= copy2d(L, depth, field, h + (long)(r[1] + j0 - flo1) * fp + (v.nx - flo0), fp, v.nx, r[1], 1, r[3] - r[1] + 1, true, false, st);
        if (r[1] + j0 == 0 && flo1 <= -1)
            rc |= copy2d(L, depth, field, h + (long)(-1 - flo1) * fp + (r[0] - flo0), fp, r[0], -1 - j0, r[2] - r[0] + 1, 1, true, false, st);
        else if (patch && r[1] == 0 && flo1 <= j0 - 1)
            rc |= copy2d(L, depth, field, h + (long)(j0 - 1 - flo1) * fp + (r[0] - flo0), fp, r[0], -1, r[2] - r[0] + 1, 1, true, false, st);
        if (r[3] + j0 == v.nyg - 1 && fhi1 >= v.nyg)
            rc |= copy2d(L, depth, field, h + (long)(v.nyg - flo1) * fp + (r[0] - flo0), fp, r[0], v.nyg - j0, r[2] - r[0] + 1, 1, true, false, st);
        else if (patch && r[3] == v.ny - 1 && fhi1 >= j0 + v.ny)
            rc |= copy2d(L, depth, field, h + (long)(j0 + v.ny - flo1) * fp + (r[0] - flo0), fp, r[0], v.ny, r[2] - r[0] + 1, 1, true, false, st);
        if (rc) return rc;
    }
    HIPCHK(hipStreamSynchronize(st));
    return 0;
}

extern "C" int suhmo_level_get_box(suhmo_level_t *L, int depth, int field, int ibox, double *fab,
                                   int flo0, int flo1, int fhi0, int fhi1, suhmo_stream_t s)
{
    CHECK_DF(L, depth, field); ARG(fab); ARG(ibox >= 0 && ibox < L->desc.nbox);
    HIPCHK(hipSetDevice(L->device));
    hipStream_t st = (hipStream_t)s;
    const DV &v = L->d[depth].v;
    int j0 = v.j0;
    flo0 -= v.i0; fhi0 -= v.i0;
    long fp = fhi0 - flo0 + 1;
    int lo0 = std::max(flo0, -1), hi0 = std::min(fhi0, v.nx + (field == SUHMO_F_BX ? 0 : 0));
    int lo1 = std::max(flo1 - j0, -v.gy), hi1 = std::min(fhi1 - j0, v.ny + v.gy - 1);
    int rc = copy2d(L, depth, field, fab + (long)(lo1 + j0 - flo1) * fp + (lo0 - flo0), fp, lo0, lo1,
                    hi0 - lo0 + 1, hi1 - lo1 + 1, false, false, st);
    if (rc) return rc;
    HIPCHK(hipStreamSynchronize(st));
    return 0;
}

__global__ void k_pack_rows(DV v, const double *__restrict__ p, int jstart, int rows, double *__restrict__ buf)
{
    int i = blockIdx.x * blockDim.x + threadIdx.x, r = blockIdx.y * blockDim.y + threadIdx.y;
    if (i > v.nx || r >= rows) return;
    buf[(size_t)r * (v.nx + 1) + i] = p[cidx(v, i, jstart + r)];
}
__global__ void k_unpack_rows(DV v, double *__restrict__ p, int jstart, int rows, const double *__restrict__ buf)
{
    int i = blockIdx.x * blockDim.x + threadIdx.x, r = blockIdx.y * blockDim.y + threadIdx.y;
    if (i > v.nx || r >= rows) return;
    p[cidx(v, i, jstart + r)] = buf[(size_t)r * (v.nx + 1) + i];
}
extern "C" int suhmo_level_pack_rows(suhmo_level_t *L, int depth, int field, int side, int rows, double *dev_buf, suhmo_stream_t s)
{
    CHECK_DF(L, depth, field); ARG(dev_buf); ARG(side == 0 || side == 1);
    const DV &v = L->d[depth].v;
    ARG(rows >= 1 && rows <= v.gy && rows <= v.ny);
    HIPCHK(hipSetDevice(L->device));
    int jstart = side == 0 ? 0 : v.ny - rows;
    if (field == SUHMO_F_BY && side == 0) jstart = 1;
    hipLaunchKernelGGL(k_pack_rows, grid2d(v.nx + 1, rows), BLK2D, 0, (hipStream_t)s, v, suhmo_field(L, depth, field), jstart, rows, dev_buf);
    HIPCHK(hipGetLastError());
    return 0;
}
extern "C" int suhmo_level_unpack_rows(suhmo_level_t *L, int depth, int field, int side, int rows, const double *dev_buf, suhmo_stream_t s)
{
    CHECK_DF(L, depth, field); ARG(dev_buf); ARG(side == 0 || side == 1);
    const DV &v = L->d[depth].v;
    ARG(rows >= 1 && rows <= v.gy);
    HIPCHK(hipSetDevice(L->device));
    if (field == SUHMO_F_MASK) suhmo_mask_halo_written(L);
    if (field == SUHMO_F_ZB) suhmo_zb_written(L);
    int jstart = side == 0 ? -rows : v.ny;
    if (field == SUHMO_F_BY && side == 1) jstart = v.ny + 1;
    hipLaunchKernelGGL(k_unpack_rows, grid2d(v.nx + 1, rows), BLK2D, 0, (hipStream_t)s, v, suhmo_field(L, depth, field), jstart, rows, dev_buf);
    HIPCHK(hipGetLastError());
    return 0;
}

extern "C" int suhmo_level_profile_enable(suhmo_level_t *L, int on) { ARG(L); L->prof_on = on; return 0; }
extern "C" int suhmo_level_profile_reset(suhmo_level_t *L)
{
    ARG(L);
    for (auto &pe : L->prof) { (void)hipEventDestroy(pe.a); (void)hipEventDestroy(pe.b); }
    L->prof.clear();
    return 0;
}
static int profile_read_kind(suhmo_level_t *L, suhmo_stream_t s, int kind, double *ms_total, long *launches, long *cells);
extern "C" int suhmo_level_profile_read(suhmo_level_t *L, suhmo_stream_t s, double *ms_total, long *launches, long *cells)
{ return profile_read_kind(L, s, 0, ms_total, launches, cells); }
extern "C" int suhmo_level_profile_read_restricting(suhmo_level_t *L, suhmo_stream_t s, double *ms_total, long *launches, long *cells)
{ return profile_read_kind(L, s, 1, ms_total, launches, cells); }
static int profile_read_kind(suhmo_level_t *L, suhmo_stream_t s, int kind, double *ms_total, long *launches, long *cells)
{
    ARG(L);
    HIPCHK(hipStreamSynchronize((hipStream_t)s));
    double tot = 0.0; long n = 0, c = 0;
    for (auto &pe : L->prof) {
        if (pe.restricts != kind) continue;
        float ms = 0.f;
        HIPCHK(hipEventElapsedTime(&ms, pe.a, pe.b));
        tot += ms; n++; c += pe.cells;
    }
    if (ms_total) *ms_total = tot;
    if (launches) *launches = n;
    if (cells) *cells = c;
    return 0;
}
```

Measured before the change: 549.9 V-cycles/s.

## Carry y-face coefficients in a register ring instead of reloading byS per row

In the streaming GSRB kernel with a uniform bed, the south y-face coefficient is now taken from the previous row's north face held in registers, so each row no longer loads byS. This cuts one global load stream and shrinks the per-row coefficient registers, which may raise occupancy. The chunk-height heuristic is also retuned for this variant: slots now come from the variant's own occupancy rather than the plain kernel's, are reduced by a sixteenth, and use a lower minimum chunk height. It is on by default through a new knob and is part of the V-cycle graph key.

```diff
diff --git a/suhmo_amd/csrc/suhmo_common.h b/suhmo_amd/csrc/suhmo_common.h
--- a/suhmo_amd/csrc/suhmo_common.h
+++ b/suhmo_amd/csrc/suhmo_common.h
@@ -156,6 +156,7 @@
     int bcoef_in_relax; long n_bcoef_in_relax;
     int mask_clean; long n_bcoef_unmasked, n_relax_unmasked;
     unsigned zb_uniform, zb_version; long n_relax_zb[SUHMO_MAXDEPTH];
+    int yface_ring; long n_relax_yring[SUHMO_MAXDEPTH];
     int has_scan;
 };
 struct ProfEv { hipEvent_t a, b; long cells; int restricts; };
@@ -231,6 +232,8 @@
     unsigned long long *zb_dev, *zb_host;
     hipEvent_t zb_ev;
     long zb_scans, relax_zb_uniform[SUHMO_MAXDEPTH];
+    int yface_ring;
+    long relax_yring[SUHMO_MAXDEPTH];
     int overlap_halo;
     hipStream_t xstream; hipEvent_t xev[2]; long overlapped;
     int tile_strips;
@@ -271,6 +274,7 @@
 void suhmo_zb_poll(suhmo_level *L);
 int suhmo_zb_scan_if_due(suhmo_level *L, hipStream_t st);
 bool suhmo_gsrb_streams(const suhmo_level *L, int depth);
+int suhmo_gsrb_stream_wg_per_cu(const char *which, long *value);
 bool suhmo_mask_would_scan(const suhmo_level *L);
 #define SUHMO_HSCRATCH_DOUBLES 64
 #define SUHMO_HSCRATCH_MASK 60
diff --git a/suhmo_amd/csrc/suhmo_fas.hip b/suhmo_amd/csrc/suhmo_fas.hip
--- a/suhmo_amd/csrc/suhmo_fas.hip
+++ b/suhmo_amd/csrc/suhmo_fas.hip
@@ -125,6 +125,7 @@
     const int mask_clean = (suhmo_mask_clean(L, 0) ? 1 : 0) | (L->ndepth > 1 && suhmo_mask_clean(L, 1) ? 2 : 0);
     const bool scanning = sp->bcoeff_otf && suhmo_mask_would_scan(L);
     const int bcoef_in_relax = L->bcoef_in_relax != 0;
+    const int yface_ring = L->yface_ring != 0;
     unsigned zb_uniform = 0;
     for (int d = 0; d < L->ndepth; d++) if (suhmo_zb_uniform(L, d)) zb_uniform |= 1u << d;
     for (size_t k = L->vgraphs.size(); k-- > 0;) {
@@ -142,11 +143,11 @@
     };
     auto replayed = [&](const VGraph &g) {
         L->bcoef_unmasked += g.n_bcoef_unmasked; L->relax_unmasked += g.n_relax_unmasked; L->bcoef_in_relax_count += g.n_bcoef_in_relax;
-        for (int d = 0; d < L->ndepth; d++) L->relax_zb_uniform[d] += g.n_relax_zb[d];
+        for (int d = 0; d < L->ndepth; d++) { L->relax_zb_uniform[d] += g.n_relax_zb[d]; L->relax_yring[d] += g.n_relax_yring[d]; }
         if (g.rout_done) { L->resout_done = 1; L->resout_count++; L->resout_np = g.rout_np; }
     };
     auto at_start = [&](const VGraph &g) {
-        if (memcmp(g.key, key, sizeof(key)) || g.mask_clean != mask_clean || g.bcoef_in_relax != bcoef_in_relax || g.zb_uniform != zb_uniform) return false;
+        if (memcmp(g.key, key, sizeof(key)) || g.mask_clean != mask_clean || g.bcoef_in_relax != bcoef_in_relax || g.zb_uniform != zb_uniform || g.yface_ring != yface_ring) return false;
         for (int d = 0; d < L->ndepth; d++) if (L->d[d].fp.f[SUHMO_F_PHI] != g.p0[d] || L->d[d].phi_alt != g.a0[d]) return false;
         if (g.rout_req != (L->resid_in_relax ? L->resout_req : 0) || g.rout_rhs != L->resout_rhs) return false;
         return L->d[0].fp.f[SUHMO_F_RHS] == g.rhs;
@@ -164,7 +165,8 @@
     if (L->vgraphs.size() >= 16) return 0;
     if (!L->gstream) HIPCHK(hipStreamCreateWithFlags(&L->gstream, hipStreamNonBlocking));
     VGraph g; memcpy(g.key, key, sizeof(key)); g.exec = nullptr; g.mask_clean = mask_clean; g.has_scan = 0; g.bcoef_in_relax = bcoef_in_relax;
-    g.zb_uniform = zb_uniform; g.zb_version = L->zb_version;
+    g.zb_uniform = zb_uniform; g.zb_version = L->zb_version; g.yface_ring = yface_ring;
+    long relax_yr[SUHMO_MAXDEPTH]; memcpy(relax_yr, L->relax_yring, sizeof(relax_yr));
     long relax_zb[SUHMO_MAXDEPTH]; memcpy(relax_zb, L->relax_zb_uniform, sizeof(relax_zb));
     for (int d = 0; d < SUHMO_MAXDEPTH; d++) { g.p0[d] = g.a0[d] = g.p1[d] = g.a1[d] = nullptr; }
     for (int d = 0; d < L->ndepth; d++) { g.p0[d] = L->d[d].fp.f[SUHMO_F_PHI]; g.a0[d] = L->d[d].phi_alt; }
@@ -186,6 +188,7 @@
     g.n_bcoef_in_relax = L->bcoef_in_relax_count - bcoef_in_relax_count; L->bcoef_in_relax_count = bcoef_in_relax_count;
     L->bcoef_unmasked = bcoef_unmasked; L->relax_unmasked = relax_unmasked;
     for (int d = 0; d < SUHMO_MAXDEPTH; d++) { g.n_relax_zb[d] = L->relax_zb_uniform[d] - relax_zb[d]; L->relax_zb_uniform[d] = relax_zb[d]; }
+    for (int d = 0; d < SUHMO_MAXDEPTH; d++) { g.n_relax_yring[d] = L->relax_yring[d] - relax_yr[d]; L->relax_yring[d] = relax_yr[d]; }
     g.rout_done = L->resout_count != rout_count;
     g.rout_np = L->resout_np;
     L->resout_done = rout_before; L->resout_count = rout_count;
diff --git a/suhmo_amd/csrc/suhmo_gsrb.hip b/suhmo_amd/csrc/suhmo_gsrb.hip
--- a/suhmo_amd/csrc/suhmo_gsrb.hip
+++ b/suhmo_amd/csrc/suhmo_gsrb.hip
@@ -267,32 +267,35 @@
 template <> struct RowMask<false> {};
 template <bool ZBU> struct RowZb { double zb[2]; };
 template <> struct RowZb<true> {};
-template <bool MASKED, bool ZBU = false>
-struct RowCoef : RowMask<MASKED>, RowZb<ZBU> {
-    double rhs[2], B[2], Pi[2], a[2], byS[2], byN[2];
+template <bool YR> struct RowByS { double byS[2]; };
+template <> struct RowByS<true> {};
+template <bool MASKED, bool ZBU = false, bool YR = false>
+struct RowCoef : RowMask<MASKED>, RowZb<ZBU>, RowByS<YR> {
+    double rhs[2], B[2], Pi[2], a[2], byN[2];
     double bx0, bx1, bx2;
 };
-template <bool MASKED, bool ZBU> __device__ __forceinline__ double row_mask(const RowCoef<MASKED, ZBU> &q, int a)
+template <bool MASKED, bool ZBU, bool YR> __device__ __forceinline__ double row_mask(const RowCoef<MASKED, ZBU, YR> &q, int a)
 {
     if constexpr (MASKED) return q.mask[a]; else return 1.0;
 }
-template <bool MASKED, bool ZBU> __device__ __forceinline__ double row_zb(const RowCoef<MASKED, ZBU> &q, int a, const FusedGeom &g)
+template <bool MASKED, bool ZBU, bool YR> __device__ __forceinline__ double row_zb(const RowCoef<MASKED, ZBU, YR> &q, int a, const FusedGeom &g)
 {
     if constexpr (ZBU) return g.zb_uniform; else return q.zb[a];
 }
 #define CP2(d, s, f) d.f[0] = s.f[0]; d.f[1] = s.f[1]
-template <bool HAS_ALPHA, bool MASKED, bool ZBU>
-__device__ __forceinline__ void copy_coef(RowCoef<MASKED, ZBU> &d, const RowCoef<MASKED, ZBU> &s)
+template <bool HAS_ALPHA, bool MASKED, bool ZBU, bool YR>
+__device__ __forceinline__ void copy_coef(RowCoef<MASKED, ZBU, YR> &d, const RowCoef<MASKED, ZBU, YR> &s)
 {
     CP2(d, s, rhs); CP2(d, s, B); CP2(d, s, Pi);
     if constexpr (!ZBU) { CP2(d, s, zb); }
     if constexpr (MASKED) { CP2(d, s, mask); }
     if (HAS_ALPHA) { CP2(d, s, a); }
-    CP2(d, s, byS); CP2(d, s, byN);
+    if constexpr (!YR) { CP2(d, s, byS); }
+    CP2(d, s, byN);
     d.bx0 = s.bx0; d.bx1 = s.bx1; d.bx2 = s.bx2;
 }
 
-template <int K, bool HAS_ALPHA, int NT, int RM = 0, bool FRHS = false, bool MASKED = true, bool BCF = false, bool ZBU = false>
+template <int K, bool HAS_ALPHA, int NT, int RM = 0, bool FRHS = false, bool MASKED = true, bool BCF = false, bool ZBU = false, bool YR = false>
 __global__ __launch_bounds__(NT) void k_gsrb_fused(DV v, FP fp, const double *__restrict__ pin,
                                                    double *__restrict__ pout, suhmo_phys_t ph, FusedGeom g)
 {
@@ -300,6 +303,7 @@
     static_assert(!(FRHS && (RR || HAS_ALPHA)), "the right-hand side is formed in the plain launch of an alpha = 0 operator");
     static_assert(!BCF || (K == 2 && NT == 64 && RM == 0 && !FRHS && !HAS_ALPHA && !MASKED), "the faces are formed in the plain two-sweep launch of a clean-mask alpha = 0 operator");
     static_assert(!ZBU || (K == 2 && NT == 64 && !HAS_ALPHA && !MASKED), "the bed as a scalar: the two-sweep launches of a clean-mask alpha = 0 operator");
+    static_assert(!YR || (ZBU && RM == 0 && !FRHS && !BCF), "one ring of y-faces: the plain two-sweep launch with the bed as a scalar");
     constexpr bool WIDE = RR || BCF;
     constexpr int DL = BCF ? 1 : 0;
     constexpr int LW = 2 * NT, R = 2 * K + 3 + (WIDE ? 1 : 0);
@@ -339,7 +343,8 @@
     auto wrapj = [&](int j) { if (g.wrap_y) { if (j < 0) j += v.ny; else if (j >= v.ny) j -= v.ny; } return j; };
     auto ld2 = [&](const double *__restrict__ p, int idx) { return *reinterpret_cast<const double2 *>(p + idx); };
 
-    RowCoef<MASKED, ZBU> cf0, cf1, cf2, cf3, cf4, cf5;
+    RowCoef<MASKED, ZBU, YR> cf0, cf1, cf2, cf3, cf4, cf5;
+    double ys5[2] = {0.0, 0.0};
     double racc = 0.0, raccp = 0.0;
     double nmax = 0.0;
     const bool xbc = !v.per[0] && (c0 - HX <= 0 || c0 + g.W + HX >= v.nx);
@@ -374,10 +379,14 @@
             if (HAS_ALPHA) LD2(cf0.a, f_a, idx);
             if constexpr (BCF) { bw0 = f_B[idx - 1]; be0 = f_B[idx + 2]; }
             else {
-                LD2(cf0.byS, f_by, idx); LD2(cf0.byN, f_by, idx + v.P);
+                if constexpr (!YR) { LD2(cf0.byS, f_by, idx); }
+                LD2(cf0.byN, f_by, idx + v.P);
                 double2 bxp = ld2(f_bx, idx);
                 cf0.bx0 = bxp.x; cf0.bx1 = bxp.y; cf0.bx2 = f_bx[idx + 2];
             }
+        }
+        if constexpr (YR) {
+            if (cval && r == jmin - 1) { LD2(cf0.byN, f_by, cidx(v, im, r) + v.P); }
         }
         if constexpr (BCF) {
             if (cval && (r - 1 >= jmin) && (r - 1 <= jmax)) {
@@ -430,7 +439,7 @@
             __syncthreads();
         }
 
-        auto advance_a = [&](const int m, const RowCoef<MASKED, ZBU> &q, auto a_tag) {
+        auto advance_a = [&](const int m, const RowCoef<MASKED, ZBU, YR> &q, const double (&byS)[2], auto a_tag) {
             constexpr int a = decltype(a_tag)::value;
             const int j = r - m - DL;
             const int x = xl + a, i = im + a;
@@ -452,18 +461,21 @@
             nl_terms(ph, c, q.B[a], q.Pi[a], row_zb(q, a, g), row_mask(q, a), nl, dnl);
             const double bxW = a ? q.bx1 : q.bx0, bxE = a ? q.bx2 : q.bx1;
             double aterm = HAS_ALPHA ? v.alpha * q.a[a] : v.alpha;
-            double lofphi = lofphi_cell(v, aterm, c, e, w, n, s, bxE, bxW, q.byN[a], q.byS[a], nl);
-            double lam = lambda_cell(v, aterm, bxE, bxW, q.byN[a], q.byS[a]);
+            double lofphi = lofphi_cell(v, aterm, c, e, w, n, s, bxE, bxW, q.byN[a], byS[a], nl);
+            double lam = lambda_cell(v, aterm, bxE, bxW, q.byN[a], byS[a]);
             double denom = 1.0e-16 + lam + dnl;
             lds[s0 * LW + x] = c + (q.rhs[a] - lofphi) / denom;
         };
-        auto advance = [&](const int m, const RowCoef<MASKED, ZBU> &q) {
+        auto advance_s = [&](const int m, const RowCoef<MASKED, ZBU, YR> &q, const double (&byS)[2]) {
             const int j = r - m - DL;
             if (j >= jmin && j <= jmax) {
                 const int a = (j + v.j0 + ((m - 1) & 1)) & 1;
-                if (a) { if (cval) advance_a(m, q, std::integral_constant<int, 1>()); }
-                else   { if (cval) advance_a(m, q, std::integral_constant<int, 0>()); }
-            }
+                if (a) { if (cval) advance_a(m, q, byS, std::integral_constant<int, 1>()); }
+                else   { if (cval) advance_a(m, q, byS, std::integral_constant<int, 0>()); }
+            }
+        };
+        auto advance = [&](const int m, const RowCoef<MASKED, ZBU, YR> &q, const RowCoef<MASKED, ZBU, YR> &below) {
+            if constexpr (YR) advance_s(m, q, below.byN); else advance_s(m, q, q.byS);
         };
         if constexpr (BCF) {
             const int j1 = r - 1;
@@ -533,7 +545,7 @@
                 } else { cf1.byS[0] = 0.0; cf1.byS[1] = 0.0; }
                 gpv[t] = make_double2(gx0, gx1); gpv[NT + t] = make_double2(gy0, gy1);
             }
-            advance(1, cf2);
+            advance(1, cf2, cf3);
             __syncthreads();
             if (faces && cval) {
                 double reW = rre[xl == 0 ? 0 : xl - 1], reE = rre[xl == LW - 2 ? LW - 1 : xl + 2];
@@ -551,27 +563,27 @@
                 }
                 rep0 = rn0; rep1 = rn1;
             }
-            advance(2, cf3);
+            advance(2, cf3, cf4);
             __syncthreads();
-            advance(3, cf4);
+            advance(3, cf4, cf5);
             __syncthreads();
-            advance(4, cf5);
+            advance(4, cf5, cf5);
         } else {
-        advance(1, cf1);
+        advance(1, cf1, cf2);
         __syncthreads();
-        advance(2, cf2);
+        advance(2, cf2, cf3);
         if constexpr (K >= 2) {
             __syncthreads();
-            advance(3, cf3);
+            advance(3, cf3, cf4);
             __syncthreads();
-            advance(4, cf4);
+            if constexpr (YR) advance_s(4, cf4, ys5); else advance(4, cf4, cf4);
         }
         }
 
         if constexpr (RR) {
             const int jr = r - 2 * K - 1;
             if (own && jr >= jA && jr < jB && jr >= 0 && jr < v.ny) {
-                const RowCoef<MASKED, ZBU> &q = (K >= 2) ? cf5 : cf3;
+                const RowCoef<MASKED, ZBU, YR> &q = (K >= 2) ? cf5 : cf3;
                 const int s0 = ring(sr - (2 * K + 1)), sN = ring(sr - 2 * K), sS = ring(sr - (2 * K + 2));
                 const double *row = lds + s0 * LW;
                 double acc = (jr & 1) ? racc : 0.0, accp = (jr & 1) ? raccp : 0.0;
@@ -623,12 +635,13 @@
         }
         sr = sr + 1 == R ? 0 : sr + 1;
         if (in_row) { lds[sr * LW + xl] = pnext.x; lds[sr * LW + xl + 1] = pnext.y; }
-        if constexpr (WIDE && K >= 2) copy_coef<HAS_ALPHA, MASKED, ZBU>(cf5, cf4);
-        if constexpr (K >= 2) { copy_coef<HAS_ALPHA, MASKED, ZBU>(cf4, cf3); copy_coef<HAS_ALPHA, MASKED, ZBU>(cf3, cf2); }
-        else if constexpr (RR) copy_coef<HAS_ALPHA, MASKED, ZBU>(cf3, cf2);
-        copy_coef<HAS_ALPHA, MASKED, ZBU>(cf2, cf1);
+        if constexpr (WIDE && K >= 2) copy_coef<HAS_ALPHA, MASKED, ZBU, YR>(cf5, cf4);
+        if constexpr (YR) { ys5[0] = cf4.byN[0]; ys5[1] = cf4.byN[1]; }
+        if constexpr (K >= 2) { copy_coef<HAS_ALPHA, MASKED, ZBU, YR>(cf4, cf3); copy_coef<HAS_ALPHA, MASKED, ZBU, YR>(cf3, cf2); }
+        else if constexpr (RR) copy_coef<HAS_ALPHA, MASKED, ZBU, YR>(cf3, cf2);
+        copy_coef<HAS_ALPHA, MASKED, ZBU, YR>(cf2, cf1);
         if constexpr (BCF) { CP2(cf1, cf0, B); bw1 = bw0; be1 = be0; }
-        else copy_coef<HAS_ALPHA, MASKED, ZBU>(cf1, cf0);
+        else copy_coef<HAS_ALPHA, MASKED, ZBU, YR>(cf1, cf0);
     }
     if constexpr (ROUT) {
         if (g.onorm) {
@@ -659,6 +672,7 @@
     int K, NT;
     bool masked;
     bool zbu;
+    bool yring;
     bool rst, rout, frhs, bcf, prolong;
     int need, adv;
     bool shallow;
@@ -667,28 +681,55 @@
 };
 
 typedef void (*FusedFn)(DV, FP, const double *, double *, suhmo_phys_t, FusedGeom);
-struct FusedKernel { int key; FusedFn fn; int slots; };
-constexpr int fused_key(int K, bool alpha, int NT, int RM, bool frhs, bool masked, bool bcf, bool zbu = false)
-{
-    return K | RM << 4 | alpha << 8 | frhs << 9 | masked << 10 | bcf << 11 | NT << 12 | zbu << 24;
-}
-#define FK(K, A, NT, RM, F, M, B) {fused_key(K, A, NT, RM, F, M, B), k_gsrb_fused<K, A, NT, RM, F, M, B>, 0}
-#define FK_ZBU(RM, F, B) {fused_key(2, false, 64, RM, F, false, B, true), k_gsrb_fused<2, false, 64, RM, F, false, B, true>, 0}
+struct FusedKernel { int key; FusedFn fn; int slots, wg_per_cu; };
+constexpr int fused_key(int K, bool alpha, int NT, int RM, bool frhs, bool masked, bool bcf, bool zbu = false, bool yring = false)
+{
+    return K | RM << 4 | alpha << 8 | frhs << 9 | masked << 10 | bcf << 11 | NT << 12 | zbu << 24 | yring << 25;
+}
+#define FK(K, A, NT, RM, F, M, B) {fused_key(K, A, NT, RM, F, M, B), k_gsrb_fused<K, A, NT, RM, F, M, B>, 0, 0}
+#define FK_ZBU(RM, F, B, YR) {fused_key(2, false, 64, RM, F, false, B, true, YR), k_gsrb_fused<2, false, 64, RM, F, false, B, true, YR>, 0, 0}
 #define FK_PLAIN(K, NT, RM) FK(K, false, NT, RM, false, true, false), FK(K, false, NT, RM, false, false, false)
 static FusedKernel fused_kernels[] = {
     FK_PLAIN(2, 64, 0), FK_PLAIN(2, 64, 1), FK_PLAIN(2, 64, 2), FK_PLAIN(1, 64, 0), FK_PLAIN(2, 256, 0), FK_PLAIN(1, 256, 0),
     FK(1, true, 64, 0, false, true, false), FK(2, true, 64, 0, false, true, false), FK(1, true, 256, 0, false, true, false), FK(2, true, 256, 0, false, true, false),
     FK(2, false, 64, 0, true, true, false), FK(2, false, 64, 0, true, false, false), FK(2, false, 64, 0, false, false, true),
-    FK_ZBU(0, false, false), FK_ZBU(1, false, false), FK_ZBU(2, false, false), FK_ZBU(0, true, false), FK_ZBU(0, false, true),
+    FK_ZBU(0, false, false, false), FK_ZBU(1, false, false, false), FK_ZBU(2, false, false, false), FK_ZBU(0, true, false, false), FK_ZBU(0, false, true, false),
+    FK_ZBU(0, false, false, true),
 };
 #undef FK_ZBU
 #undef FK_PLAIN
 #undef FK
-static FusedKernel *fused_kernel(int K, bool alpha, int NT, int RM, bool frhs, bool masked, bool bcf, bool zbu)
-{
-    const int key = fused_key(K, alpha, NT, RM, frhs, masked, bcf, zbu);
+static FusedKernel *fused_kernel(int K, bool alpha, int NT, int RM, bool frhs, bool masked, bool bcf, bool zbu, bool yring = false)
+{
+    const int key = fused_key(K, alpha, NT, RM, frhs, masked, bcf, zbu, yring);
     for (FusedKernel &k : fused_kernels) if (k.key == key) return &k;
     return nullptr;
+}
+static int fused_occupancy(FusedKernel *k, int NT)
+{
+    if (k->slots) return 0;
+    int nb = 0, ncu = 0, dev = 0;
+    HIPCHK(hipGetDevice(&dev));
+    HIPCHK(hipDeviceGetAttribute(&ncu, hipDeviceAttributeMultiprocessorCount, dev));
+    HIPCHK(hipOccupancyMaxActiveBlocksPerMultiprocessor(&nb, k->fn, NT, 0));
+    k->wg_per_cu = nb > 0 ? nb : 1;
+    k->slots = k->wg_per_cu * (ncu > 0 ? ncu : 256);
+    return 0;
+}
+int suhmo_gsrb_stream_wg_per_cu(const char *which, long *value)
+{
+    static const struct { const char *name; int RM; bool frhs, bcf, yring; } tab[] = {
+        {"plain", 0, false, false, false}, {"yring", 0, false, false, true}, {"rst", 1, false, false, false}, {"rout", 2, false, false, false},
+        {"frhs", 0, true, false, false}, {"bcf", 0, false, true, false}};
+    for (const auto &e : tab) {
+        if (strcmp(which, e.name)) continue;
+        FusedKernel *k = fused_kernel(2, false, 64, e.RM, e.frhs, false, e.bcf, true, e.yring);
+        if (!k) { suhmo_set_error("internal: no streaming kernel '%s'", which); return -4; }
+        int rc = fused_occupancy(k, 64); if (rc) return rc;
+        *value = k->wg_per_cu;
+        return 0;
+    }
+    return 1;
 }
 
 static int launch_fused(suhmo_level *L, int depth, const RelaxStep &s, hipStream_t st, int part = 0)
@@ -697,9 +738,8 @@
     const bool RST = RM == 1, RR = RM != 0, unmasked = !s.masked;
     Depth &D = L->d[depth];
     const DV &v = D.v;
-    FusedKernel *k = fused_kernel(K, v.alpha != 0.0, NT, RM, s.frhs, s.masked, s.bcf, s.zbu);
-    FusedKernel *plain = (v.alpha != 0.0 || s.frhs || s.bcf) ? fused_kernel(K, false, NT, RM, false, s.masked, false, s.zbu) : k;
-    if (!k || !plain || (part && (s.frhs || s.bcf)) || (s.bcf && s.prolong)) { suhmo_set_error("internal: a streaming relaxation step without a kernel"); return -4; }
+    FusedKernel *k = fused_kernel(K, v.alpha != 0.0, NT, RM, s.frhs, s.masked, s.bcf, s.zbu, s.yring);
+    if (!k || (part && (s.frhs || s.bcf)) || (s.bcf && s.prolong)) { suhmo_set_error("internal: a streaming relaxation step without a kernel"); return -4; }
     if (!D.phi_alt) {
         HIPCHK(hipMalloc(&D.phi_alt, D.elems * sizeof(double)));
         HIPCHK(hipMemsetAsync(D.phi_alt, 0, D.elems * sizeof(double), st));
@@ -712,20 +752,15 @@
     g.W = 2 * ((v.nx + 2 * g.nstrips - 1) / (2 * g.nstrips));
     g.nstrips = (v.nx + g.W - 1) / g.W;
     {
-        if (!plain->slots) {
-            int nb = 0, ncu = 0, dev = 0;
-            HIPCHK(hipGetDevice(&dev));
-            HIPCHK(hipDeviceGetAttribute(&ncu, hipDeviceAttributeMultiprocessorCount, dev));
-            HIPCHK(hipOccupancyMaxActiveBlocksPerMultiprocessor(&nb, plain->fn, NT, 0));
-            plain->slots = (nb > 0 ? nb : 1) * (ncu > 0 ? ncu : 256);
-        }
+        { int rc = fused_occupancy(k, NT); if (rc) return rc; }
         g.jbeg = v.ext[0] ? -ext_rows : 0;
         g.jend = v.ny + (v.ext[1] ? ext_rows : 0);
         const int nrows = g.jend - g.jbeg;
-        int nch = plain->slots / g.nstrips;
+        const int slots = s.yring ? k->slots - k->slots / 16 : k->slots, floorK = s.yring ? 6 : 8;
+        int nch = slots / g.nstrips;
         if (nch < 1) nch = 1;
         g.Hc = (nrows + nch - 1) / nch;
-        if (g.Hc < 8 * K) g.Hc = 8 * K;
+        if (g.Hc < floorK * K) g.Hc = floorK * K;
         if ((long)v.nx * v.ny < 2000000L) g.Hc = 6;
         if (L->fused_hc > 0) g.Hc = L->fused_hc;
         if (RST) g.Hc += g.Hc & 1;
@@ -784,6 +819,7 @@
     hipLaunchKernelGGL(k->fn, dim3(g.ntiles), dim3(NT), 0, st, v, D.fp, pin, D.phi_alt, L->ph, g);
     if (unmasked) L->relax_unmasked++;
     if (s.zbu) L->relax_zb_uniform[depth]++;
+    if (s.yring) L->relax_yring[depth]++;
     if (part != 1) { std::swap(D.fp.f[SUHMO_F_PHI], D.phi_alt); suhmo_fp_changed(); }
     return 0;
 }
@@ -1262,6 +1298,7 @@
     const bool plain = variants && !s.rst && !s.rout;
     s.frhs = (absorb & ABSORB_RHS) && plain;
     s.bcf = absorb == ABSORB_BCOEF && plain && depth == 0 && !stored && !s.masked;
+    s.yring = L->yface_ring && s.zbu && plain && !s.frhs && !s.bcf && !v.per[1];
     s.adv = ext ? plan_halo_advance(F, s.need, (absorb & ABSORB_RHS) ? F : 2 * (left - K) + tail, v.gy - s.need, s.rst) : 0;
     return s;
 }
diff --git a/suhmo_amd/csrc/suhmo_level.hip b/suhmo_amd/csrc/suhmo_level.hip
--- a/suhmo_amd/csrc/suhmo_level.hip
+++ b/suhmo_amd/csrc/suhmo_level.hip
@@ -173,6 +173,7 @@
     L->graph_max_cells = 1500000; L->gstream = nullptr; L->vgraph_replays = 0; memset(L->vgraph_seen, 0, sizeof(L->vgraph_seen));
     L->fused_min_cells = 1000000;
     L->skip_mask = 1; L->mask_known = 1; L->poll_readback = 1; L->zb_known = 1;
+    L->yface_ring = 1; memset(L->relax_yring, 0, sizeof(L->relax_yring));
     L->bottom_solver = 0; L->bottom_one_launch_max_cells = 16384;
     L->bottom_ctr = nullptr; L->bottom_host_iters = L->bottom_host_solves = 0;
     {
@@ -186,7 +187,7 @@
             {"SUHMO_TILE_RESTRICT", &suhmo_level::tile_restrict}, {"SUHMO_TILE_ORDER", &suhmo_level::tile_order}, {"SUHMO_FAS_RHS_IN_RELAX", &suhmo_level::fas_rhs_in_relax},
             {"SUHMO_TILE_S", &suhmo_level::tile_s}, {"SUHMO_GSRB_TILE", &suhmo_level::gsrb_tile}, {"SUHMO_TILE_T", &suhmo_level::tile_t},
             {"SUHMO_FUSED_RESTRICT", &suhmo_level::fused_restrict}, {"SUHMO_SKIP_MASK", &suhmo_level::skip_mask}, {"SUHMO_MASK_KNOWN", &suhmo_level::mask_known}, {"SUHMO_ZB_KNOWN", &suhmo_level::zb_known},
-            {"SUHMO_POLL_READBACK", &suhmo_level::poll_readback}, {"SUHMO_AVG_OVERLAP", &suhmo_level::avg_overlap}};
+            {"SUHMO_POLL_READBACK", &suhmo_level::poll_readback}, {"SUHMO_AVG_OVERLAP", &suhmo_level::avg_overlap}, {"SUHMO_YFACE_RING", &suhmo_level::yface_ring}};
         static const LongKnob longs[] = {
             {"SUHMO_AGG_MIN_CELLS", &suhmo_level::agg_min_cells}, {"SUHMO_TILE_MAX_CELLS", &suhmo_level::tile_max_cells},
             {"SUHMO_GRAPH_MAX_CELLS", &suhmo_level::graph_max_cells}, {"SUHMO_FUSED_MIN_CELLS", &suhmo_level::fused_min_cells},
@@ -392,7 +393,7 @@
         {"tile_strips", &suhmo_level::tile_strips}, {"overlap_halo", &suhmo_level::overlap_halo}, {"skip_mask", &suhmo_level::skip_mask}, {"mask_known", &suhmo_level::mask_known}, {"zb_known", &suhmo_level::zb_known}, {"tile_chunks",
             &suhmo_level::tile_chunks}, {"tile_order", &suhmo_level::tile_order}, {"tile_restrict", &suhmo_level::tile_restrict}, {"fas_rhs_in_relax",
             &suhmo_level::fas_rhs_in_relax}, {"resid_in_relax", &suhmo_level::resid_in_relax}, {"bcoef_in_relax", &suhmo_level::bcoef_in_relax}, {"fas_rhs_fused", &suhmo_level::fas_rhs_fused},
-        {"avg_overlap", &suhmo_level::avg_overlap}, {"tile_s", &suhmo_level::tile_s}, {"gsrb_tile", &suhmo_level::gsrb_tile}, {"tile_t", &suhmo_level::tile_t}, {"poll_readback", &suhmo_level::poll_readback}};
+        {"avg_overlap", &suhmo_level::avg_overlap}, {"yface_ring", &suhmo_level::yface_ring}, {"tile_s", &suhmo_level::tile_s}, {"gsrb_tile", &suhmo_level::gsrb_tile}, {"tile_t", &suhmo_level::tile_t}, {"poll_readback", &suhmo_level::poll_readback}};
     for (const auto &e : tab) if (!strcmp(key, e.k)) return &(L->*(e.m));
     return nullptr;
 }
@@ -451,19 +452,23 @@
     if (!strcmp(key, "relax_unmasked_launches")) { *value = L->relax_unmasked; return 0; }
     {
         if (!strcmp(key, "zb_scans")) { *value = L->zb_scans; return 0; }
-        const bool st = !strncmp(key, "zb_state", 8), nl = !strncmp(key, "relax_zb_uniform_launches", 25);
-        const char *rest = st ? key + 8 : nl ? key + 25 : nullptr;
+        const bool st = !strncmp(key, "zb_state", 8), nl = !strncmp(key, "relax_zb_uniform_launches", 25), yr = !strncmp(key, "relax_yring_launches", 20);
+        const char *rest = st ? key + 8 : nl ? key + 25 : yr ? key + 20 : nullptr;
         if (rest && !*rest) {
             *value = st ? L->d[0].zb_state : 0;
-            for (int d = 0; nl && d < L->ndepth; d++) *value += L->relax_zb_uniform[d];
+            for (int d = 0; (nl || yr) && d < L->ndepth; d++) *value += yr ? L->relax_yring[d] : L->relax_zb_uniform[d];
             return 0;
         }
         if (rest && rest[0] == '_' && rest[1] == 'd' && rest[2] >= '0' && rest[2] <= '9') {
             const int d = atoi(rest + 2);
             if (d >= L->ndepth) { suhmo_set_error("option '%s': the level has %d depths", key, L->ndepth); return -1; }
-            *value = st ? L->d[d].zb_state : L->relax_zb_uniform[d];
+            *value = st ? L->d[d].zb_state : yr ? L->relax_yring[d] : L->relax_zb_uniform[d];
             return 0;
         }
+    }
+    if (!strncmp(key, "stream_wg_per_cu_", 17)) {
+        const int rc = suhmo_gsrb_stream_wg_per_cu(key + 17, value);
+        if (rc <= 0) return rc;
     }
     if (!strcmp(key, "vcycle_graph_replays")) { *value = L->vgraph_replays; return 0; }
     if (!strcmp(key, "bottom_solver")) { *value = L->bottom_solver; return 0; }
```

Measured after the change: 561.2 V-cycles/s (median of 6 runs). 1.02x the previous value.
